# dragonlong/articulated-pose

Hardware: AMD Instinct MI355X
Metric: point-clouds/sec (N=1024, eyeglasses ANCSH infer+pose-fit) (higher is better)
Workload: dtype f32 (network) / f64 (joint LM)

## Files before the change

### articulated-pose_amd/_lib.py

```python
import ctypes
import os
import subprocess

import torch

_HERE = os.path.dirname(os.path.abspath(__file__))
LIB_PATH = os.environ.get("ANCSH_HIP_LIB") or os.path.join(_HERE, "libancsh_hip.so")

_c_int, _c_long, _c_float, _vp = ctypes.c_int, ctypes.c_long, ctypes.c_float, ctypes.c_void_p

SIGNATURES = {
    "ancsh_farthest_point_sample": [_c_int, _c_int, _c_int, _vp, _vp, _vp, _vp],
    "ancsh_farthest_point_sample_gather": [_c_int, _c_int, _c_int, _vp, _vp, _vp, _vp, _vp],
    "ancsh_prob_sample": [_c_int, _c_int, _c_int, _vp, _vp, _vp, _vp, _vp],
    "ancsh_gather_point": [_c_int, _c_int, _c_int, _vp, _vp, _vp, _vp],
    "ancsh_query_ball_point": [_c_int, _c_int, _c_int, _c_float, _c_int, _vp, _vp, _vp, _vp, _vp],
    "ancsh_query_ball_point_multi": [_c_int] + [_vp] * 10,
    "ancsh_group_point": [_c_int, _c_int, _c_int, _c_int, _c_int, _vp, _vp, _vp, _vp],
    "ancsh_group_point_multi": [_c_int] + [_vp] * 9,
    "ancsh_selection_sort": [_c_int, _c_int, _c_int, _c_int, _vp, _vp, _vp, _vp],
    "ancsh_knn_point": [_c_int, _c_int, _c_int, _c_int, _c_int, _vp, _vp, _vp, _vp, _vp],
    "ancsh_group_point_ex": [_c_int, _c_int, _c_int, _c_int, _c_int, _vp, _vp, _vp, _vp, _c_int, _c_int, _vp],
    "ancsh_three_nn": [_c_int, _c_int, _c_int, _vp, _vp, _vp, _vp, _vp],
    "ancsh_three_weights": [_c_int, _vp, _vp, _vp],
    "ancsh_three_nn_weights": [_c_int, _c_int, _c_int, _vp, _vp, _vp, _vp, _vp, _vp],
    "ancsh_three_interpolate": [_c_int, _c_int, _c_int, _c_int, _vp, _vp, _vp, _vp, _vp],
    "ancsh_three_interpolate_ex": [_c_int, _c_int, _c_int, _c_int, _vp, _vp, _vp, _vp, _c_int, _c_int, _vp],
    "ancsh_conv1x1": [_c_long, _c_int, _c_int, _vp, _c_int, _vp, _vp, _vp, _vp, _c_int, _vp, _c_int, _c_int, _vp],
    "ancsh_conv1x1_ex": [_c_long, _c_int, _c_int, _vp, _c_int, _vp, _vp, _vp, _vp, _c_int, _vp, _c_int, _c_int, _vp, _c_int, _vp],
    "ancsh_conv1x1_packed": [_c_long, _c_int, _c_int, _vp, _c_int, _vp, _vp, _vp, _vp, _c_int, _vp, _c_int, _c_int, _vp, _c_int, _vp],
    "ancsh_conv1x1_packed_grouped": [_c_int, _c_long, _c_int, _c_int, _vp, _c_int, _vp, _vp, _vp, _vp, _c_int, _vp, _c_int, _c_int, _vp, _c_int, _vp],
    "ancsh_conv1x1_grouped": [_c_int, _c_long, _c_int, _c_int, _vp, _c_int, _vp, _vp, _vp, _vp, _c_int, _vp, _c_int, _c_int, _vp],
    "ancsh_sa_module_fused_grouped": [_c_int] * 9 + [_vp] * 4 + [_vp, _vp, _vp],
    "ancsh_sa_module_fused_partial_grouped": [_c_int] * 8 + [_vp] * 7,
    "ancsh_fp_interpolate_concat_ex": [_c_int, _c_int, _c_int, _c_int, _vp, _vp, _vp, _vp, _c_int, _vp, _c_int, _c_int, _c_int, _vp],
    "ancsh_sa_pack_weights_bf16x3": [_c_int, _c_int, _vp, _vp, _vp],
    "ancsh_sa_module_fused_bf16x3": [_c_int] * 8 + [_vp] * 4 + [_vp, _vp, _vp],
    "ancsh_sa_module_fused_partial_bf16x3": [_c_int] * 7 + [_vp] * 7,
    "ancsh_sa_module_fused_bf16x3_grouped": [_c_int] * 9 + [_vp] * 4 + [_vp, _vp, _vp],
    "ancsh_sa_module_fused_partial_bf16x3_grouped": [_c_int] * 8 + [_vp] * 7,
    "ancsh_sa_pack_weights_f16x2": [_c_int, _c_int, _vp, _vp, _vp],
    "ancsh_sa_module_fused_f16x2_grouped": [_c_int] * 9 + [_vp] * 4 + [_vp, _vp, _vp],
    "ancsh_sa_module_fused_partial_f16x2_grouped": [_c_int] * 8 + [_vp] * 7,
    "ancsh_mlp_chain_grouped_fp_f16x2": [_c_int] * 5 + [_vp] * 7 + [_vp],
    "ancsh_sa3_chain_grouped_bf16x3": [_c_int] * 7 + [_vp] * 4 + [_vp],
    "ancsh_sa3_chain_grouped_f16x2": [_c_int] * 7 + [_vp] * 4 + [_vp],
    "ancsh_fp1_chain_grouped_bf16x3": [_c_int] * 6 + [_vp] * 4 + [_vp],
    "ancsh_fp1_chain_grouped_f16x2": [_c_int] * 6 + [_vp] * 4 + [_vp],
    "ancsh_fp2_chain_grouped_bf16x3": [_c_int] * 8 + [_vp] * 6 + [_vp],
    "ancsh_fp2_chain_grouped_f16x2": [_c_int] * 8 + [_vp] * 6 + [_vp],
    "ancsh_sa_module_fused_f16x2_grouped_guarded": [_c_int] * 9 + [_vp] * 4 + [_vp, _vp, _vp, _c_int, _vp],
    "ancsh_sa_module_fused_partial_f16x2_grouped_guarded": [_c_int] * 8 + [_vp] * 6 + [_vp, _c_int, _vp],
    "ancsh_mlp_chain_grouped_fp_f16x2_guarded": [_c_int] * 5 + [_vp] * 7 + [_vp, _c_int, _vp],
    "ancsh_sa3_chain_grouped_f16x2_guarded": [_c_int] * 7 + [_vp] * 4 + [_vp, _c_int, _vp],
    "ancsh_fp1_chain_grouped_f16x2_guarded": [_c_int] * 6 + [_vp] * 4 + [_vp, _c_int, _vp],
    "ancsh_fp2_chain_grouped_f16x2_guarded": [_c_int] * 8 + [_vp] * 6 + [_vp, _c_int, _vp],
    "ancsh_iou_3d": [_c_int, _c_int, _vp, _vp, _vp, _vp, _vp],
    "ancsh_joint_params": [_c_int] * 5 + [_vp] * 9 + [_vp],
    "ancsh_part_extents": [_c_int] * 4 + [_vp] * 3 + [_c_int] + [_vp] * 4 + [_vp],
    "ancsh_articulation_rec": [_c_int] * 5 + [_vp] * 10 + [_vp] * 4 + [_vp],
    "ancsh_fp_interpolate_concat": [_c_int, _c_int, _c_int, _c_int, _vp, _vp, _vp, _vp, _c_int, _vp, _c_int, _vp],
    "ancsh_query_ball_group_xyz": [_c_int, _c_int, _c_int, _c_float, _c_int, _vp, _vp, _c_int, _vp, _vp, _vp, _c_int, _vp],
    "ancsh_query_ball_group_xyz_multi": [_c_int] + [_vp] * 13,
    "ancsh_group_max": [_c_long, _c_int, _c_int, _vp, _vp, _vp],
    "ancsh_sa_module_fused": [_c_int] * 8 + [_vp] * 4 + [_vp, _vp, _vp],
    "ancsh_sa_module_fused_partial": [_c_int] * 7 + [_vp] * 7,
    "ancsh_sa_pack_weights": [_c_int, _c_int, _vp, _vp, _vp],
    "ancsh_mlp_chain": [_c_long, _c_int, _vp, _c_int, _c_int, _vp, _vp, _vp],
    "ancsh_mlp_chain_grouped": [_c_int, _c_long, _c_int, _vp, _c_int, _vp, _vp, _vp, _vp, _vp],
    "ancsh_sa3_chain_grouped": [_c_int] * 7 + [_vp] * 4 + [_vp],
    "ancsh_fp_single_source_init": [_c_int] * 5 + [_vp] * 3 + [_vp],
    "ancsh_fp1_chain_grouped": [_c_int] * 6 + [_vp] * 4 + [_vp],
    "ancsh_fp2_chain_grouped": [_c_int] * 8 + [_vp] * 6 + [_vp],
    "ancsh_mlp_chain_grouped_fp": [_c_int] * 5 + [_vp] * 8 + [_vp],
    "ancsh_mlp_chain_grouped_fp_bf16x3": [_c_int] * 5 + [_vp] * 7 + [_vp],
    "ancsh_head_activations": [_c_long, _c_int, _c_int, _vp, _c_int] + [_vp] * 10 + [_vp],
    "ancsh_pose_partition": [_c_int, _c_int, _c_int] + [_vp] * 11 + [_vp],
    "ancsh_pose_poison_records": [_c_int, _c_int, _c_int] + [_vp] * 5 + [_vp],
    "ancsh_pose_joint_direction": [_c_int, _c_int, _c_int, _vp, _vp, _vp, _vp],
    "ancsh_ransac_single": [_c_int, _vp, _vp, _vp, _c_float, _c_int, _vp, ctypes.c_ulonglong, _c_int, _vp, _vp, _vp, _vp, _vp],
    "ancsh_ransac_single_ex": [_c_int, _vp, _vp, _vp, _c_float, _c_int, _vp, ctypes.c_ulonglong, _c_int, _vp, _vp, _vp, _vp, _vp, _c_long, _vp],
    "ancsh_ransac_single_rec": [_c_int, _vp, _vp, _vp, _c_float, _c_int, _vp, ctypes.c_ulonglong, _c_int, _vp, _vp, _vp, _vp, _vp, _c_long,
                                _vp, _c_int, _vp, _c_float, _vp],
    "ancsh_ransac_joint_rec": [_c_int, _vp, _vp, _vp, _vp, _vp, ctypes.c_double, _c_int, _vp, ctypes.c_ulonglong, _c_int]
                              + [_vp] * 7 + [_c_int, _vp, _c_int, _vp, ctypes.c_double, _vp],
    "ancsh_ransac_joint": [_c_int, _vp, _vp, _vp, _vp, _vp, ctypes.c_double, _c_int, _vp, ctypes.c_ulonglong, _c_int]
                          + [_vp] * 7 + [_vp],
    "ancsh_ransac_single_rec_dseed": [_c_int, _vp, _vp, _vp, _c_float, _c_int, _vp, _vp, _c_int, _vp, _vp, _vp, _vp, _vp, _c_long,
                                      _vp, _c_int, _vp, _c_float, _vp],
    "ancsh_ransac_joint_rec_dseed": [_c_int, _vp, _vp, _vp, _vp, _vp, ctypes.c_double, _c_int, _vp, _vp, _c_int]
                                    + [_vp] * 7 + [_c_int, _vp, _c_int, _vp, ctypes.c_double, _vp],
    "ancsh_input_sample_stream": [_c_int, _c_int, _c_int, _vp, _c_long, _vp, _vp, _c_int, _vp, _vp, _vp, _vp, _vp],
    "ancsh_input_sample_stream_keyed": [_c_int, _c_int, _c_int, _vp, _c_long, _vp, _vp, _c_int, _vp, _vp, _vp, _vp, _vp],
    "ancsh_ransac_single_rec_dkey": [_c_int, _vp, _vp, _vp, _c_float, _c_int, _vp, _vp, _c_int, _vp, _vp, _vp, _vp, _vp, _c_long,
                                     _vp, _c_int, _vp, _c_float, _vp],
    "ancsh_ransac_joint_rec_dkey": [_c_int, _vp, _vp, _vp, _vp, _vp, ctypes.c_double, _c_int, _vp, _vp, _c_int]
                                   + [_vp] * 7 + [_c_int, _vp, _c_int, _vp, ctypes.c_double, _vp],
    "ancsh_raw_point_labels": [_c_int] * 5 + [_vp, _c_long] + [_vp] * 8 + [_vp],
    "ancsh_pose_joint_direction_pred": [_c_int, _c_int, _c_int, _c_int, _vp, _vp, _vp, _vp],
    "ancsh_pose_poison_records_pred": [_c_int, _c_int, _c_int] + [_vp] * 4 + [_c_int, _vp, _vp, _vp],
    "ancsh_input_sample_stream_xyz": [_c_int, _c_int, _c_int, _vp, _c_long, _vp, _vp, _vp, _vp, _vp, _vp],
    "ancsh_input_sample_stream_xyz_keyed": [_c_int, _c_int, _c_int, _vp, _c_long, _vp, _vp, _vp, _vp, _vp, _vp],
    "ancsh_ransac_joint_rec_kind": [_c_int, _vp, _vp, _vp, _vp, _vp, ctypes.c_double, _c_int, _vp, ctypes.c_ulonglong, _c_int]
                                   + [_vp] * 7 + [_c_int, _vp, _c_int, _vp, ctypes.c_double, _vp, _vp],
    "ancsh_ransac_joint_rec_dseed_kind": [_c_int, _vp, _vp, _vp, _vp, _vp, ctypes.c_double, _c_int, _vp, _vp, _c_int]
                                         + [_vp] * 7 + [_c_int, _vp, _c_int, _vp, ctypes.c_double, _vp, _vp],
    "ancsh_ransac_joint_rec_dkey_kind": [_c_int, _vp, _vp, _vp, _vp, _vp, ctypes.c_double, _c_int, _vp, _vp, _c_int]
                                        + [_vp] * 7 + [_c_int, _vp, _c_int, _vp, ctypes.c_double, _vp, _vp],
    "ancsh_depth_unproject_stream": [_c_int, _c_int, _vp, _vp, _c_long, _vp, _vp, _vp, _c_long, _vp, _vp, _vp, _vp],
    "ancsh_depth_label_images": [_c_int, _c_int, _vp, _vp, _c_long] + [_vp] * 5 + [_c_long, _vp, _vp, _vp, _c_long, _vp],
    "ancsh_joint_state_rec": [_c_int] * 3 + [_vp, _c_int] + [_vp] * 5 + [_vp],
    "ancsh_fit_quality_rec": [_c_int] * 2 + [_vp] * 4 + [ctypes.c_double] + [_vp] * 3 + [_vp],
    "ancsh_gt_error_rec": [_c_int] * 4 + [_vp, _c_int] + [_vp] * 3 + [_c_int] + [_vp] * 2 + [_vp],
    "ancsh_input_sample": [_c_int, _c_int, _c_int, _vp, _vp, _vp, _vp, _c_int, _c_int, _c_int, _vp, _vp, _vp, _vp, _vp],
    "ancsh_test_losses": [_c_int, _c_int, _c_int, _c_int, _vp, _vp, _vp],
    "ancsh_ransac_joint_ex": [_c_int, _vp, _vp, _vp, _vp, _vp, ctypes.c_double, _c_int, _vp, ctypes.c_ulonglong, _c_int]
                             + [_vp] * 7 + [_c_int, _vp],
    "ancsh_umeyama": [_c_int, _vp, _vp, _vp, _vp, _vp],
    "ancsh_estimate_similarity_transform": [_c_int, _vp, _vp, _vp, _c_int, _vp, ctypes.c_ulonglong, _vp, _vp, _vp],
}

_lib = None


def build(force=False):
    args = ["make", "-s", "-j8", "-C", os.path.join(_HERE, "csrc")]
    if force:
        subprocess.check_call(args + ["clean"])
    subprocess.check_call(args)
    return LIB_PATH


def lib():
    global _lib
    if _lib is None:
        if not os.path.exists(LIB_PATH):
            raise RuntimeError(
                f"{LIB_PATH} is missing: the HIP extension is not built (run __graft_entry__.build()); "
                "there is no CPU fallback for the product path")
        L = ctypes.CDLL(LIB_PATH)
        for name, argtypes in SIGNATURES.items():
            fn = getattr(L, name)
            fn.argtypes = argtypes
            fn.restype = _c_int
        L.ancsh_last_error.restype = ctypes.c_char_p
        L.ancsh_abi_version.restype = _c_int
        L.ancsh_last_ball_query_schedule.restype = _c_int
        L.ancsh_sa_packed_weight_floats.argtypes = [_c_int, _c_int]
        L.ancsh_sa_packed_weight_floats.restype = _c_long
        L.ancsh_sa_packed_weight_bytes_bf16x3.argtypes = [_c_int, _c_int]
        L.ancsh_sa_packed_weight_bytes_bf16x3.restype = _c_long
        L.ancsh_sa_packed_weight_bytes_f16x2.argtypes = [_c_int, _c_int]
        L.ancsh_sa_packed_weight_bytes_f16x2.restype = _c_long
        L.ancsh_ransac_single_quads_floats.argtypes = [_c_long, _c_int]
        L.ancsh_ransac_single_quads_floats.restype = _c_long
        _lib = L
    return _lib


def stream_ptr():
    return torch.cuda.current_stream().cuda_stream


def ptr(t):
    return 0 if t is None else t.data_ptr()


_prof = None
_prof_lead = (0, {})


def profile_start(lead=0, lead_for=None):
    global _prof, _prof_lead
    _prof, _prof_lead = [], (int(lead), dict(lead_for or {}))


def profile_stop():
    global _prof
    rec, _prof = _prof, None
    torch.cuda.synchronize()
    return [(n, a, e0.elapsed_time(e1)) for n, a, e0, e1 in rec]


def call(name, *args):
    L = lib()
    if _prof is not None:
        e0, e1 = torch.cuda.Event(enable_timing=True), torch.cuda.Event(enable_timing=True)
        for _ in range(_prof_lead[1].get(name, _prof_lead[0])):
            getattr(L, name)(*args, stream_ptr())
        e0.record()
        rc = getattr(L, name)(*args, stream_ptr())
        e1.record()
        _prof.append((name, args, e0, e1))
    else:
        rc = getattr(L, name)(*args, stream_ptr())
    if rc != 0:
        msg = L.ancsh_last_error().decode()
        if rc == -1:
            raise ValueError(msg)
        raise RuntimeError(f"{name}: {msg}")


def require_cuda(*tensors):
    for t in tensors:
        if t is not None and not t.is_cuda:
            raise RuntimeError("articulated-pose_amd ops run on the MI355X only: got a CPU tensor "
                               "(no CPU fallback in the product path)")
```

### articulated-pose_amd/csrc/pose.hip

```cpp
#include "common.h"
#include "pose_math.h"

namespace ancsh {
namespace pose {

constexpr int MODEL_A = 13;
constexpr int MODEL_B = 26;

__device__ __forceinline__ unsigned long long splitmix64(unsigned long long x) {
    x += 0x9E3779B97F4A7C15ull;
    x = (x ^ (x >> 30)) * 0xBF58476D1CE4E5B9ull;
    x = (x ^ (x >> 27)) * 0x94D049BB133111EBull;
    return x ^ (x >> 31);
}
__device__ __forceinline__ int device_draw(unsigned long long seed, int prob, int iter, int k, int n) {
    const unsigned long long h = splitmix64(seed ^ splitmix64(((unsigned long long)prob << 40) ^ ((unsigned long long)iter << 8) ^ (unsigned)k));
    return (int)(h % (unsigned long long)n);
}
enum { KEY_VALUE = 0, KEY_DSEED = 1, KEY_DKEY = 2 };
struct DKey {
    const ancsh_stream_key *key;
    int parts;
};
template <int KM> struct KeyArgT { typedef unsigned long long type; };
// ... 112 lines not shown
__device__ __forceinline__ int inlier2_f32(const float R[9], float sc, const float tr[3], f32x2 sx, f32x2 sy, f32x2 sz,
                                           f32x2 tx, f32x2 ty, f32x2 tz, float th_sq) {
#pragma clang fp contract(off)
    const f32x2 rx = __builtin_elementwise_fma((f32x2)R[2], sz, __builtin_elementwise_fma((f32x2)R[1], sy, R[0] * sx));
    const f32x2 ry = __builtin_elementwise_fma((f32x2)R[5], sz, __builtin_elementwise_fma((f32x2)R[4], sy, R[3] * sx));
    const f32x2 rz = __builtin_elementwise_fma((f32x2)R[8], sz, __builtin_elementwise_fma((f32x2)R[7], sy, R[6] * sx));
    const f32x2 ex = (tx - sc * rx) - tr[0], ey = (ty - sc * ry) - tr[1], ez = (tz - sc * rz) - tr[2];
    const f32x2 s = (ex * ex + ey * ey) + ez * ez;
    return (s.x < th_sq ? 1 : 0) + (s.y < th_sq ? 1 : 0);
}

#if defined(__HIP_DEVICE_COMPILE__) && !defined(__gfx950__)
#error "pose.hip: the packed-f32 clamp counting (v_pk_mul_f32 ... clamp, DX10_CLAMP semantics) is written for gfx950 only"
#endif
__device__ __forceinline__ void inlier2_count_f32(const float R[9], float sc, const float tr[3], f32x2 sx, f32x2 sy, f32x2 sz,
                                                  f32x2 tx, f32x2 ty, f32x2 tz, float th_sq, f32x2 &cnt) {
#pragma clang fp contract(off)
    const f32x2 rx = __builtin_elementwise_fma((f32x2)R[2], sz, __builtin_elementwise_fma((f32x2)R[1], sy, R[0] * sx));
    const f32x2 ry = __builtin_elementwise_fma((f32x2)R[5], sz, __builtin_elementwise_fma((f32x2)R[4], sy, R[3] * sx));
    const f32x2 rz = __builtin_elementwise_fma((f32x2)R[8], sz, __builtin_elementwise_fma((f32x2)R[7], sy, R[6] * sx));
    const f32x2 ex = (tx - sc * rx) - tr[0], ey = (ty - sc * ry) - tr[1], ez = (tz - sc * rz) - tr[2];
    const f32x2 s = (ex * ex + ey * ey) + ez * ez;
    const f32x2 nbig = {-0x1p126f, -0x1p126f};
    const f32x2 tbig = {th_sq * 0x1p126f, th_sq * 0x1p126f};
    f32x2 one;
    asm("v_pk_fma_f32 %0, %1, %2, %3 clamp" : "=v"(one) : "v"(s), "v"(nbig), "v"(tbig));
    cnt = cnt + one;
}

__device__ __forceinline__ void load_draw3(const int *draws, unsigned long long seed, int prob, int kbase, int niter, int h, int k0,
                                           int stride, int n, int idx[3]) {
#pragma unroll
    for (int k = 0; k < 3; ++k) {
        int v = draws ? draws[((size_t)prob * niter + h) * stride + k0 + k] : device_draw(seed, prob + kbase, h, k0 + k, n);
        idx[k] = v < 0 ? 0 : (v >= n ? n - 1 : v);
    }
}

#ifndef A_CHUNK_N
#define A_CHUNK_N 2048
#endif
constexpr int A_CHUNK = A_CHUNK_N;

template <int KM>
__global__ __launch_bounds__(256) void ransac_single_score_kernel(const int *__restrict__ off, const float *__restrict__ src,
                                                                  const float *__restrict__ tgt, float th, int niter,
                                                                  const int *__restrict__ draws, KeyArg<KM> seed_arg,
                                                                  int *__restrict__ scores) {
    const unsigned long long seed = kernel_seed<KM>(seed_arg, 0);
    const int kbase = key_problem_base<KM>(seed_arg);
    __shared__ __attribute__((aligned(16))) float pl[6][A_CHUNK];
    const int prob = blockIdx.y, h = blockIdx.x * 256 + threadIdx.x;
    const int r0 = off[prob], n = off[prob + 1] - r0;
    const bool live = h < niter && n > 0;
    float R[9] = {1, 0, 0, 0, 1, 0, 0, 0, 1}, sc = 0.f, tr[3] = {0, 0, 0};
    if (live) {
        int id[3];
        load_draw3(draws, seed, prob, kbase, niter, h, 0, 3, n, id);
        float s3[3][3], t3[3][3];
#pragma unroll
        for (int i = 0; i < 3; ++i)
#pragma unroll
            for (int c = 0; c < 3; ++c) {
                s3[i][c] = src[(size_t)(r0 + id[i]) * 3 + c];
                t3[i][c] = tgt[(size_t)(r0 + id[i]) * 3 + c];
            }
        estimate_single3(s3, t3, R, sc, tr);
    }
    int cnt = 0;
    for (int base = 0; base < n; base += A_CHUNK) {
        const int m = (n - base) < A_CHUNK ? (n - base) : A_CHUNK;
        const int m4 = (m + 3) & ~3;
        __syncthreads();
        for (int e = threadIdx.x; e < m4 * 3; e += 256) {
            const int i = e / 3, c = e - i * 3;
            const bool in = i < m;
            pl[c][i] = in ? src[(size_t)(r0 + base) * 3 + e] : 0.f;
            pl[3 + c][i] = in ? tgt[(size_t)(r0 + base) * 3 + e] : __builtin_inff();
        }
        __syncthreads();
        if (live) {
            const float4 *px = (const float4 *)pl[0], *py = (const float4 *)pl[1], *pz = (const float4 *)pl[2];
            const float4 *pa = (const float4 *)pl[3], *pb = (const float4 *)pl[4], *pc = (const float4 *)pl[5];
            const int nq = m4 >> 2;
            auto score4 = [&](const float4 &x, const float4 &y, const float4 &z, const float4 &a, const float4 &b, const float4 &c) {
                cnt += inlier2_f32(R, sc, tr, f32x2{x.x, x.y}, f32x2{y.x, y.y}, f32x2{z.x, z.y}, f32x2{a.x, a.y}, f32x2{b.x, b.y},
                                   f32x2{c.x, c.y}, th);
                cnt += inlier2_f32(R, sc, tr, f32x2{x.z, x.w}, f32x2{y.z, y.w}, f32x2{z.z, z.w}, f32x2{a.z, a.w}, f32x2{b.z, b.w},
                                   f32x2{c.z, c.w}, th);
            };
            float4 x0 = px[0], y0 = py[0], z0 = pz[0], a0 = pa[0], b0 = pb[0], c0 = pc[0];
            for (int q = 0; q < nq; q += 2) {
                const int q1 = q + 1 < nq ? q + 1 : q, q2 = q + 2 < nq ? q + 2 : q1;
                const float4 x1 = px[q1], y1 = py[q1], z1 = pz[q1], a1 = pa[q1], b1 = pb[q1], c1 = pc[q1];
                __builtin_amdgcn_sched_barrier(0);
                score4(x0, y0, z0, a0, b0, c0);
                __builtin_amdgcn_sched_barrier(0);
                x0 = px[q2]; y0 = py[q2]; z0 = pz[q2]; a0 = pa[q2]; b0 = pb[q2]; c0 = pc[q2];
                __builtin_amdgcn_sched_barrier(0);
                if (q + 1 < nq) score4(x1, y1, z1, a1, b1, c1);
                __builtin_amdgcn_sched_barrier(0);
            }
        }
    }
    if (h < niter) scores[(size_t)prob * niter + h] = cnt;
}

__device__ __forceinline__ int quad_start(int r0, int prob) { return 2 * ((r0 + 7) / 8 + prob); }

__global__ __launch_bounds__(256) void soa_quads_kernel(const int *__restrict__ off, const float *__restrict__ src,
                                                        const float *__restrict__ tgt, float *__restrict__ quads, int cap_quads) {
    const int prob = blockIdx.y, i = blockIdx.x * 256 + threadIdx.x;
    const int r0 = off[prob], n = off[prob + 1] - r0;
    if (i >= ((n + 7) & ~7)) return;
    if (quad_start(r0, prob) + (i >> 2) >= cap_quads) return;
    float *q = quads + ((size_t)quad_start(r0, prob) + (i >> 2)) * 24 + (i & 3);
    const bool in = i < n;
#pragma unroll
    for (int c = 0; c < 3; ++c) {
        q[c * 4] = in ? src[(size_t)(r0 + i) * 3 + c] : 0.f;
        q[12 + c * 4] = in ? tgt[(size_t)(r0 + i) * 3 + c] : __builtin_inff();
    }
}

#ifndef POSE_SCORE_WAVES
#define POSE_SCORE_WAVES 0
#endif
#if POSE_SCORE_WAVES > 0
#define POSE_SCORE_ATTR __attribute__((amdgpu_waves_per_eu(POSE_SCORE_WAVES)))
#else
#define POSE_SCORE_ATTR
#endif
template <int KM>
__global__ __launch_bounds__(256) POSE_SCORE_ATTR void ransac_single_score_sreg_kernel(const int *__restrict__ off, const float *__restrict__ src,
                                                                       const float *__restrict__ tgt, const float *__restrict__ quads,
                                                                       int cap_quads, float th, int niter, const int *__restrict__ draws,
                                                                       KeyArg<KM> seed_arg, int *__restrict__ scores) {
    const unsigned long long seed = kernel_seed<KM>(seed_arg, 0);
    const int kbase = key_problem_base<KM>(seed_arg);
    const int prob = blockIdx.y, h = blockIdx.x * 256 + threadIdx.x;
    const int r0 = off[prob], n = off[prob + 1] - r0;
    float R[9] = {1, 0, 0, 0, 1, 0, 0, 0, 1}, sc = 0.f, tr[3] = {0, 0, 0};
    if (h < niter && n > 0) {
        int id[3];
        load_draw3(draws, seed, prob, kbase, niter, h, 0, 3, n, id);
        float s3[3][3], t3[3][3];
#pragma unroll
        for (int i = 0; i < 3; ++i)
#pragma unroll
            for (int c = 0; c < 3; ++c) {
                s3[i][c] = src[(size_t)(r0 + id[i]) * 3 + c];
                t3[i][c] = tgt[(size_t)(r0 + id[i]) * 3 + c];
            }
        estimate_single3(s3, t3, R, sc, tr);
    }
    typedef float f32x8 __attribute__((ext_vector_type(8)));
    const int q0 = quad_start(r0, prob);
    const f32x8 *Q = reinterpret_cast<const f32x8 *>(quads + (size_t)q0 * 24);
    int nq = ((n + 7) >> 3) * 2;
    nq = min(nq, (cap_quads - q0) & ~1);
    f32x2 cnt2 = {0.f, 0.f};
    auto score4 = [&](const f32x8 &v0, const f32x8 &v1, const f32x8 &v2) {
        inlier2_count_f32(R, sc, tr, f32x2{v0[0], v0[1]}, f32x2{v0[4], v0[5]}, f32x2{v1[0], v1[1]}, f32x2{v1[4], v1[5]},
                          f32x2{v2[0], v2[1]}, f32x2{v2[4], v2[5]}, th, cnt2);
        inlier2_count_f32(R, sc, tr, f32x2{v0[2], v0[3]}, f32x2{v0[6], v0[7]}, f32x2{v1[2], v1[3]}, f32x2{v1[6], v1[7]},
                          f32x2{v2[2], v2[3]}, f32x2{v2[6], v2[7]}, th, cnt2);
    };
    constexpr int LGKM0 = 0xC07F;
    if (nq > 0) {
        f32x8 a0 = Q[0], a1 = Q[1], a2 = Q[2];
        __builtin_amdgcn_s_waitcnt(LGKM0);
        for (int q = 0; q < nq; q += 2) {
            const int q2 = q + 2 < nq ? q + 2 : q;
            const f32x8 b0 = Q[q * 3 + 3], b1 = Q[q * 3 + 4], b2 = Q[q * 3 + 5];
            __builtin_amdgcn_sched_barrier(0);
            score4(a0, a1, a2);
            __builtin_amdgcn_sched_barrier(0);
            __builtin_amdgcn_s_waitcnt(LGKM0);
            a0 = Q[q2 * 3]; a1 = Q[q2 * 3 + 1]; a2 = Q[q2 * 3 + 2];
            __builtin_amdgcn_sched_barrier(0);
            score4(b0, b1, b2);
            __builtin_amdgcn_sched_barrier(0);
            __builtin_amdgcn_s_waitcnt(LGKM0);
        }
    }
    if (h < niter) scores[(size_t)prob * niter + h] = n > 0 ? (int)(cnt2.x + cnt2.y) : 0;
}

template <class T>
__device__ __forceinline__ int block_argmax_first(const T *sc, int niter, T *best_out, void *lds) {
    T bv = (T)-1;
    int bi = 0x7fffffff;
    for (int h = threadIdx.x; h < niter; h += blockDim.x) {
        const T v = sc[h];
        if (v > bv) { bv = v; bi = h; }
    }
#pragma unroll
    for (int o = 32; o > 0; o >>= 1) {
        const T ov = __shfl_xor(bv, o, 64);
        const int oi = __shfl_xor(bi, o, 64);
        if (ov > bv || (ov == bv && oi < bi)) { bv = ov; bi = oi; }
    }
    T *rv = (T *)lds;
    int *ri = (int *)(rv + 8);
    const int lane = threadIdx.x & 63, wave = threadIdx.x >> 6, nw = blockDim.x >> 6;
    __syncthreads();
    if (lane == 0) { rv[wave] = bv; ri[wave] = bi; }
    __syncthreads();
    bv = rv[0]; bi = ri[0];
    for (int w = 1; w < nw; ++w)
        if (rv[w] > bv || (rv[w] == bv && ri[w] < bi)) { bv = rv[w]; bi = ri[w]; }
    __syncthreads();
    *best_out = bv;
    return bi;
}

__device__ __forceinline__ void pair_sums(const float (*cs)[3], const float (*ct)[3], int n, double (&pr)[3]) {
#pragma clang fp contract(off)
    const int lane = threadIdx.x & 63;
    const int wave = __builtin_amdgcn_readfirstlane(threadIdx.x >> 6), nw = blockDim.x >> 6;
    const int seg = (n + nw - 1) / nw;
    const int j0 = wave * seg, j1 = min(n, j0 + seg);
    constexpr int RB = 6;
    for (int ib = lane; ib < n; ib += 64 * RB) {
        float sx[RB], sy[RB], sz[RB], tx[RB], ty[RB], tz[RB], ab[RB], aa[RB], bb[RB];
#pragma unroll
        for (int r = 0; r < RB; ++r) {
            const int i = min(ib + 64 * r, n - 1);
            sx[r] = cs[i][0]; sy[r] = cs[i][1]; sz[r] = cs[i][2];
            tx[r] = ct[i][0]; ty[r] = ct[i][1]; tz[r] = ct[i][2];
            ab[r] = aa[r] = bb[r] = 0.f;
        }
        for (int j = j0; j < j1; ++j) {
            const float cx = cs[j][0], cy = cs[j][1], cz = cs[j][2], dx = ct[j][0], dy = ct[j][1], dz = ct[j][2];
#pragma unroll
            for (int r = 0; r < RB; ++r) {
                const float ux = sx[r] - cx, uy = sy[r] - cy, uz = sz[r] - cz;
                const float vx = tx[r] - dx, vy = ty[r] - dy, vz = tz[r] - dz;
                const float A = __builtin_amdgcn_sqrtf((ux * ux + uy * uy) + uz * uz);
                const float b = __builtin_amdgcn_sqrtf((vx * vx + vy * vy) + vz * vz);
                ab[r] += A * b;
                aa[r] += A * A;
                bb[r] += b * b;
            }
        }
#pragma unroll
        for (int r = 0; r < RB; ++r)
            if (ib + 64 * r < n) { pr[0] += (double)ab[r]; pr[1] += (double)aa[r]; pr[2] += (double)bb[r]; }
    }
}

__device__ __forceinline__ void refit_similarity(const float (*cs)[3], const float (*ct)[3], int n_in, double *red,
                                                 double R[9], double &scale, double tr[3]) {
    double sums[6] = {0, 0, 0, 0, 0, 0};
    for (int i = threadIdx.x; i < n_in; i += 256) {
#pragma unroll
        for (int c = 0; c < 3; ++c) { sums[c] += cs[i][c]; sums[3 + c] += ct[i][c]; }
    }
    block_sum<6>(sums, red, 4);
    double sm[3], tm[3];
#pragma unroll
    for (int c = 0; c < 3; ++c) { sm[c] = sums[c] / n_in; tm[c] = sums[3 + c] / n_in; }
    double M[9] = {0, 0, 0, 0, 0, 0, 0, 0, 0};
    for (int i = threadIdx.x; i < n_in; i += 256)
#pragma unroll
        for (int a = 0; a < 3; ++a)
#pragma unroll
            for (int b = 0; b < 3; ++b) M[a * 3 + b] += (ct[i][a] - tm[a]) * (cs[i][b] - sm[b]);
    block_sum<9>(M, red, 4);
    double q[4];
    horn_quat(M, q);
    quat_to_mat(q, R);
    double pr[3] = {0, 0, 0};
    pair_sums(cs, ct, n_in, pr);
    block_sum<3>(pr, red, 4);
    scale = pr[0] / (pr[1] + 1e-6);
    const double sf = (double)(float)scale;
#pragma unroll
    for (int a = 0; a < 3; ++a) tr[a] = tm[a] - sf * (R[a * 3 + 0] * sm[0] + R[a * 3 + 1] * sm[1] + R[a * 3 + 2] * sm[2]);
}

__device__ __forceinline__ int compact_flagged(bool flag, int i, int n, const float *src, const float *tgt, size_t row0,
                                               float (*cs)[3], float (*ct)[3], int base, int *wcnt) {
    const int lane = threadIdx.x & 63, wave = threadIdx.x >> 6;
    const unsigned long long m = __ballot(flag);
    __syncthreads();
    if (lane == 0) wcnt[wave] = __popcll(m);
    __syncthreads();
    int start = base;
    for (int w = 0; w < wave; ++w) start += wcnt[w];
    const int total = wcnt[0] + wcnt[1] + wcnt[2] + wcnt[3];
    if (flag) {
        const int pos = start + __builtin_amdgcn_mbcnt_hi((unsigned)(m >> 32), __builtin_amdgcn_mbcnt_lo((unsigned)m, 0));
#pragma unroll
        for (int c = 0; c < 3; ++c) {
            cs[pos][c] = src[(row0 + i) * 3 + c];
            ct[pos][c] = tgt[(row0 + i) * 3 + c];
        }
    }
    return base + total;
}

template <int KM>
__global__ __launch_bounds__(256) void ransac_single_finish_kernel(const int *__restrict__ off, const float *__restrict__ src,
                                                                   const float *__restrict__ tgt, float th, int niter,
                                                                   const int *__restrict__ draws, KeyArg<KM> seed_arg,
                                                                   const int *__restrict__ scores, int max_n,
                                                                   double *__restrict__ out_model,
                                                                   unsigned char *__restrict__ out_inliers,
                                                                   int *__restrict__ out_best, FitExtras E) {
    const unsigned long long seed = kernel_seed<KM>(seed_arg, 0);
    const int kbase = key_problem_base<KM>(seed_arg);
    extern __shared__ __attribute__((aligned(16))) unsigned char smem[];
    double *red = (double *)smem;
    int *wcnt = (int *)(red + 64);
    float(*cs)[3] = (float(*)[3])(wcnt + 8);
    float(*ct)[3] = cs + max_n;
    const int prob = blockIdx.x;
    const int r0 = off[prob], n = off[prob + 1] - r0;
    double *om = out_model + (size_t)prob * MODEL_A;
    if (n <= 0 || n > max_n) {
        if (threadIdx.x < MODEL_A) om[threadIdx.x] = NAN;
        if (E.record && threadIdx.x < (E.K == 1 ? 2 * MODEL_A : MODEL_A)) E.record[(size_t)prob * 26 + threadIdx.x] = NAN;
        if (E.tie && threadIdx.x < 2) E.tie[prob * 2 + threadIdx.x] = 0;
        if (threadIdx.x == 0) { out_best[prob * 2] = -1; out_best[prob * 2 + 1] = n <= 0 ? 0 : -2; }
        for (int i = threadIdx.x; i < n; i += 256) out_inliers[r0 + i] = 0;
        return;
    }
    int best_score;
    const int best = block_argmax_first<int>(scores + (size_t)prob * niter, niter, &best_score, red);
    int id[3];
    load_draw3(draws, seed, prob, kbase, niter, best, 0, 3, n, id);
    float s3[3][3], t3[3][3], R[9], sc, tr[3];
#pragma unroll
    for (int i = 0; i < 3; ++i)
#pragma unroll
        for (int c = 0; c < 3; ++c) {
            s3[i][c] = src[(size_t)(r0 + id[i]) * 3 + c];
            t3[i][c] = tgt[(size_t)(r0 + id[i]) * 3 + c];
        }
    estimate_single3(s3, t3, R, sc, tr);
    int n_in = 0, n_border = 0, n_near = 0;
    for (int base = 0; base < n; base += 256) {
        const int i = base + threadIdx.x;
        bool f = false, border = false;
        if (i < n) {
            const float *ps = src + (size_t)(r0 + i) * 3, *pt = tgt + (size_t)(r0 + i) * 3;
            const float rs = residual_sq_f32(R, sc, tr, ps[0], ps[1], ps[2], pt[0], pt[1], pt[2]);
            f = rs < th;
            border = rs >= E.lo_f && rs < E.hi_f;
            out_inliers[r0 + i] = f ? 1 : 0;
        }
        n_border += __popcll(__ballot(border));
        n_in = compact_flagged(f, i, n, src, tgt, (size_t)r0, cs, ct, n_in, wcnt);
    }
    if (E.tie) {
        const bool winner_degenerate = id[0] == id[1] || id[0] == id[2] || id[1] == id[2];
        __shared__ int s_cand[TIE_MAX_CAND];
        const int *sp = scores + (size_t)prob * niter;
        const int lane = threadIdx.x & 63, wave = threadIdx.x >> 6;
        int found = 0;
        for (int h0 = 0; h0 < niter; h0 += 256) {
            const int h = h0 + threadIdx.x;
            bool cand = false;
            if (h < niter && h != best && sp[h] >= best_score - 1) {
                int d3[3];
                load_draw3(draws, seed, prob, kbase, niter, h, 0, 3, n, d3);
                cand = d3[0] == d3[1] || d3[0] == d3[2] || d3[1] == d3[2];
            }
            const unsigned long long m = __ballot(cand);
            __syncthreads();
            if (lane == 0) wcnt[wave] = __popcll(m);
            __syncthreads();
            int start = found;
            for (int w = 0; w < wave; ++w) start += wcnt[w];
            if (cand) {
                const int slot = start + __builtin_amdgcn_mbcnt_hi((unsigned)(m >> 32), __builtin_amdgcn_mbcnt_lo((unsigned)m, 0));
                if (slot < TIE_MAX_CAND) s_cand[slot] = h;
            }
            found += wcnt[0] + wcnt[1] + wcnt[2] + wcnt[3];
        }
        __syncthreads();
        const int ncand = found < TIE_MAX_CAND ? found : TIE_MAX_CAND;
        n_near = found - ncand + (winner_degenerate ? 1 : 0);
        for (int c = 0; c < ncand; ++c) {
            const int h = s_cand[c];
            int d3[3];
            load_draw3(draws, seed, prob, kbase, niter, h, 0, 3, n, d3);
            float hs[3][3], ht[3][3], hR[9], hsc, htr[3];
#pragma unroll
            for (int i = 0; i < 3; ++i)
#pragma unroll
                for (int cc = 0; cc < 3; ++cc) {
                    hs[i][cc] = src[(size_t)(r0 + d3[i]) * 3 + cc];
                    ht[i][cc] = tgt[(size_t)(r0 + d3[i]) * 3 + cc];
                }
            estimate_single3(hs, ht, hR, hsc, htr);
            int differs = 0;
            for (int i = threadIdx.x; i < n; i += 256) {
                const float *ps = src + (size_t)(r0 + i) * 3, *pt = tgt + (size_t)(r0 + i) * 3;
                const bool f = residual_sq_f32(hR, hsc, htr, ps[0], ps[1], ps[2], pt[0], pt[1], pt[2]) < th;
                differs |= (int)(f != (out_inliers[r0 + i] != 0));
            }
            n_near += __syncthreads_or(differs) ? 1 : 0;
        }
        if ((threadIdx.x & 63) == 0) wcnt[4 + (threadIdx.x >> 6)] = n_border;
        __syncthreads();
        if (threadIdx.x == 0) {
            E.tie[prob * 2] = wcnt[4] + wcnt[5] + wcnt[6] + wcnt[7];
            E.tie[prob * 2 + 1] = winner_degenerate ? -n_near : n_near;
        }
    }
    __syncthreads();
    double Rd[9], scale, trd[3];
    if (n_in > 0) {
        refit_similarity(cs, ct, n_in, red, Rd, scale, trd);
    } else {
#pragma unroll
        for (int a = 0; a < 9; ++a) Rd[a] = NAN;
        scale = NAN; trd[0] = trd[1] = trd[2] = NAN;
    }
    if (threadIdx.x == 0) {
#pragma unroll
        for (int a = 0; a < 9; ++a) om[a] = Rd[a];
        om[9] = (double)(float)scale;
#pragma unroll
        for (int a = 0; a < 3; ++a) om[10 + a] = trd[a];
        out_best[prob * 2] = best;
        out_best[prob * 2 + 1] = best_score;
        if (E.record) {
            double *rec = E.record + (size_t)prob * 26;
#pragma unroll
            for (int a = 0; a < MODEL_A; ++a) rec[a] = om[a];
            if (E.K == 1) {
#pragma unroll
                for (int a = 0; a < MODEL_A; ++a) rec[MODEL_A + a] = om[a];
            }
        }
    }
}

struct PartFd {
    Rod b, p[3];
    double rh[3];
    double blk[6];
    double gv[3];
    double ju[3];
    double jd[3][3];

    __device__ __forceinline__ void begin_points(const double r[3]) {
        b = rod_prepare(r[0], r[1], r[2]);
#pragma unroll
        for (int q = 0; q < 3; ++q) {
            const double h = fd_step(r[q]);
            rh[q] = fast_rcp(h);
            p[q] = rod_prepare(r[0] + (q == 0 ? h : 0.0), r[1] + (q == 1 ? h : 0.0), r[2] + (q == 2 ? h : 0.0));
        }
#pragma unroll
        for (int i = 0; i < 6; ++i) blk[i] = 0.0;
        gv[0] = gv[1] = gv[2] = 0.0;
    }
    __device__ __forceinline__ void begin(const double r[3], const double J[3]) {
        begin_points(r);
        rod_apply(b, J[0], J[1], J[2], ju[0], ju[1], ju[2]);
#pragma unroll
        for (int q = 0; q < 3; ++q) {
            double qx, qy, qz;
            rod_apply(p[q], J[0], J[1], J[2], qx, qy, qz);
            jd[0][q] = qx; jd[1][q] = qy; jd[2][q] = qz;
        }
    }
    __device__ __forceinline__ void point(double px, double py, double pz, double yx, double yy, double yz) {
        double ox, oy, oz;
        rod_apply(b, px, py, pz, ox, oy, oz);
        const double f0 = yx - ox, f1 = yy - oy, f2 = yz - oz;
        double a[3][3];
#pragma unroll
        for (int q = 0; q < 3; ++q) {
            double qx, qy, qz;
            rod_apply(p[q], px, py, pz, qx, qy, qz);
            a[0][q] = ((yx - qx) - f0) * rh[q];
            a[1][q] = ((yy - qy) - f1) * rh[q];
            a[2][q] = ((yz - qz) - f2) * rh[q];
        }
#pragma unroll
        for (int q = 0; q < 3; ++q) {
#pragma unroll
            for (int r = 0; r <= q; ++r) blk[q * (q + 1) / 2 + r] += a[0][q] * a[0][r] + a[1][q] * a[1][r] + a[2][q] * a[2][r];
            gv[q] += a[0][q] * f0 + a[1][q] * f1 + a[2][q] * f2;
        }
    }
};

__device__ __forceinline__ void assemble_normal(const PartFd &p0, const double blk0[6], const double g0[3], const PartFd &p1,
                                                const double blk1[6], const double g1[3], double wj, double A[21], double g[6]) {
    double f[3], a[3][6];
#pragma unroll
    for (int c = 0; c < 3; ++c) f[c] = p0.ju[c] - p1.ju[c];
#pragma unroll
    for (int c = 0; c < 3; ++c)
#pragma unroll
        for (int q = 0; q < 3; ++q) {
            a[c][q] = (((p0.jd[c][q] - p1.ju[c]) - f[c])) * p0.rh[q];
            a[c][3 + q] = (((p0.ju[c] - p1.jd[c][q]) - f[c])) * p1.rh[q];
        }
#pragma unroll
    for (int i = 0; i < 6; ++i) {
#pragma unroll
        for (int j = 0; j <= i; ++j) {
            double v = wj * (a[0][i] * a[0][j] + a[1][i] * a[1][j] + a[2][i] * a[2][j]);
            if (i < 3) v += blk0[i * (i + 1) / 2 + j];
            else if (j >= 3) v += blk1[(i - 3) * (i - 2) / 2 + (j - 3)];
            A[i * (i + 1) / 2 + j] = v;
        }
        g[i] = wj * (a[0][i] * f[0] + a[1][i] * f[1] + a[2][i] * f[2]) + (i < 3 ? g0[i] : g1[i - 3]);
    }
}

__device__ __forceinline__ double prismatic_cost(const double x[6]) {
    const double a = x[0] - x[3], b = x[1] - x[4], c = x[2] - x[5];
    return a * a + b * b + c * c;
}
__device__ __forceinline__ void assemble_normal_prismatic(const double x[6], const double blk0[6], const double g0[3],
                                                          const double blk1[6], const double g1[3], double A[21], double g[6]) {
    double f[3], d0[3], d1[3];
#pragma unroll
    for (int c = 0; c < 3; ++c) {
        const double h0 = fd_step(x[c]), h1 = fd_step(x[3 + c]);
        f[c] = x[c] - x[3 + c];
        d0[c] = (((x[c] + h0) - x[3 + c]) - f[c]) * fast_rcp(h0);
        d1[c] = ((x[c] - (x[3 + c] + h1)) - f[c]) * fast_rcp(h1);
    }
#pragma unroll
    for (int i = 0; i < 6; ++i) {
#pragma unroll
        for (int j = 0; j <= i; ++j) {
            double v = 0.0;
            if (i < 3) v = (i == j ? d0[i] * d0[i] : 0.0) + blk0[i * (i + 1) / 2 + j];
            else if (j >= 3) v = (i == j ? d1[i - 3] * d1[i - 3] : 0.0) + blk1[(i - 3) * (i - 2) / 2 + (j - 3)];
            else if (i - 3 == j) v = d1[j] * d0[j];
            A[i * (i + 1) / 2 + j] = v;
        }
        g[i] = i < 3 ? d0[i] * f[i] + g0[i] : d1[i - 3] * f[i - 3] + g1[i - 3];
    }
}

template <bool PRISM>
struct HypProblemT {
    double x0[3][3], y0[3][3], x1[3][3], y1[3][3], J[3], wj;

    __device__ __forceinline__ double cost(const double x[6]) const {
        const Rod r0 = rod_prepare(x[0], x[1], x[2]), r1 = rod_prepare(x[3], x[4], x[5]);
        double s = 0.0, ox, oy, oz;
#pragma unroll
        for (int i = 0; i < 3; ++i) {
            rod_apply(r0, x0[i][0], x0[i][1], x0[i][2], ox, oy, oz);
            const double a = y0[i][0] - ox, b = y0[i][1] - oy, c = y0[i][2] - oz;
            s += a * a + b * b + c * c;
            rod_apply(r1, x1[i][0], x1[i][1], x1[i][2], ox, oy, oz);
            const double d = y1[i][0] - ox, e = y1[i][1] - oy, f = y1[i][2] - oz;
            s += d * d + e * e + f * f;
        }
        if constexpr (PRISM) {
            return s + prismatic_cost(x);
        } else {
            double ux, uy, uz, wx, wy, wz;
            rod_apply(r0, J[0], J[1], J[2], ux, uy, uz);
            rod_apply(r1, J[0], J[1], J[2], wx, wy, wz);
            s += wj * ((ux - wx) * (ux - wx) + (uy - wy) * (uy - wy) + (uz - wz) * (uz - wz));
            return s;
        }
    }
    __device__ __forceinline__ void normal(const double x[6], double A[21], double g[6]) const {
        PartFd p0, p1;
        if constexpr (PRISM) p0.begin_points(x); else p0.begin(x, J);
#pragma unroll
        for (int i = 0; i < 3; ++i) p0.point(x0[i][0], x0[i][1], x0[i][2], y0[i][0], y0[i][1], y0[i][2]);
        if constexpr (PRISM) p1.begin_points(x + 3); else p1.begin(x + 3, J);
#pragma unroll
        for (int i = 0; i < 3; ++i) p1.point(x1[i][0], x1[i][1], x1[i][2], y1[i][0], y1[i][1], y1[i][2]);
        if constexpr (PRISM) assemble_normal_prismatic(x, p0.blk, p0.gv, p1.blk, p1.gv, A, g);
        else assemble_normal(p0, p0.blk, p0.gv, p1, p1.blk, p1.gv, wj, A, g);
    }
};
typedef HypProblemT<false> HypProblem;

__device__ __forceinline__ void scales3(const float s[3][3], const float t[3][3], float &sc, float &sc_inv) {
    double ab = 0.0, aa = 0.0, bb = 0.0;
#pragma unroll
    for (int i = 0; i < 3; ++i)
#pragma unroll
        for (int j = i + 1; j < 3; ++j) {
            double ds = 0.0, dt = 0.0;
#pragma unroll
            for (int c = 0; c < 3; ++c) {
                const double u = (double)s[i][c] - s[j][c], v = (double)t[i][c] - t[j][c];
                ds += u * u;
                dt += v * v;
            }
            ab += 2.0 * sqrt(ds) * sqrt(dt);
            aa += 2.0 * ds;
            bb += 2.0 * dt;
        }
    sc = (float)(ab / (aa + 1e-6));
    sc_inv = (float)(ab / (bb + 1e-6));
}

__device__ __forceinline__ void center_part3(const float s[3][3], const float t[3][3], float sc_inv, double xc[3][3],
                                             double yc[3][3]) {
    float sm[3], tm[3];
#pragma unroll
    for (int c = 0; c < 3; ++c) {
        sm[c] = ((s[0][c] + s[1][c]) + s[2][c]) / 3.0f;
        tm[c] = ((sc_inv * t[0][c] + sc_inv * t[1][c]) + sc_inv * t[2][c]) / 3.0f;
    }
#pragma unroll
    for (int i = 0; i < 3; ++i) {
#pragma unroll
        for (int c = 0; c < 3; ++c) {
            xc[i][c] = (double)(s[i][c] - sm[c]);
            yc[i][c] = (double)(sc_inv * t[i][c] - tm[c]);
        }
    }
}

__device__ __forceinline__ void prep_part3(const float s[3][3], const float t[3][3], float sc_inv, double xc[3][3],
                                           double yc[3][3], double rv[3]) {
    center_part3(s, t, sc_inv, xc, yc);
    double M[9] = {0, 0, 0, 0, 0, 0, 0, 0, 0};
#pragma unroll
    for (int i = 0; i < 3; ++i)
#pragma unroll
        for (int a = 0; a < 3; ++a)
#pragma unroll
            for (int b = 0; b < 3; ++b) M[a * 3 + b] += yc[i][a] * xc[i][b];
    double q[4];
    horn_quat_fast(M, q);
    quat_to_rotvec(q, rv);
}

__device__ __forceinline__ double residual_sq_f64(const double R[9], double sc, const double tr[3], float sx, float sy, float sz,
                                                  float tx, float ty, float tz) {
    const double rx = R[0] * sx + R[1] * sy + R[2] * sz, ry = R[3] * sx + R[4] * sy + R[5] * sz,
                 rz = R[6] * sx + R[7] * sy + R[8] * sz;
    const double ex = ((double)tx - sc * rx) - tr[0], ey = ((double)ty - sc * ry) - tr[1], ez = ((double)tz - sc * rz) - tr[2];
    return ex * ex + ey * ey + ez * ez;
}
__device__ __forceinline__ bool inlier_f64(const double R[9], double sc, const double tr[3], float sx, float sy, float sz,
                                           float tx, float ty, float tz, double th) {
    return residual_sq_f64(R, sc, tr, sx, sy, sz, tx, ty, tz) < th;
}

struct HypSamples {
    float s0[3][3], t0[3][3], s1[3][3], t1[3][3];
};
__device__ __forceinline__ void load_hyp_samples(const float *__restrict__ src, const float *__restrict__ tgt, const int *draws,
                                                 unsigned long long seed, int prob, int kbase, int niter, int h, int a0, int n0, int a1,
                                                 int n1, HypSamples &q) {
    int i0[3], i1[3];
    load_draw3(draws, seed, prob, kbase, niter, h, 0, 6, n0, i0);
    load_draw3(draws, seed, prob, kbase, niter, h, 3, 6, n1, i1);
#pragma unroll
    for (int i = 0; i < 3; ++i)
#pragma unroll
        for (int c = 0; c < 3; ++c) {
            q.s0[i][c] = src[(size_t)(a0 + i0[i]) * 3 + c];
            q.t0[i][c] = tgt[(size_t)(a0 + i0[i]) * 3 + c];
            q.s1[i][c] = src[(size_t)(a1 + i1[i]) * 3 + c];
            q.t1[i][c] = tgt[(size_t)(a1 + i1[i]) * 3 + c];
        }
}

template <int KM>
__global__ __launch_bounds__(64) void ransac_joint_init_kernel(const int *__restrict__ rng0, const int *__restrict__ rng1,
                                                               const float *__restrict__ src, const float *__restrict__ tgt,
                                                               int niter, const int *__restrict__ draws, KeyArg<KM> seed_arg,
                                                               double *__restrict__ scores, double *__restrict__ models) {
    const unsigned long long seed = kernel_seed<KM>(seed_arg, 1);
    const int kbase = key_problem_base<KM>(seed_arg);
    const int prob = blockIdx.y, h = blockIdx.x * 64 + threadIdx.x;
    const int a0 = rng0[prob * 2], n0 = rng0[prob * 2 + 1] - a0;
    const int a1 = rng1[prob * 2], n1 = rng1[prob * 2 + 1] - a1;
    if (h >= niter) return;
    double *mo = models + ((size_t)prob * niter + h) * MODEL_B;
    if (n0 <= 0 || n1 <= 0) {
        scores[(size_t)prob * niter + h] = -1.0;
        for (int i = 0; i < MODEL_B; ++i) mo[i] = NAN;
        return;
    }
    HypSamples q;
    load_hyp_samples(src, tgt, draws, seed, prob, kbase, niter, h, a0, n0, a1, n1, q);
    float sc0, sc0i, sc1, sc1i;
    scales3(q.s0, q.t0, sc0, sc0i);
    scales3(q.s1, q.t1, sc1, sc1i);
    double xc[3][3], yc[3][3], x[6];
    prep_part3(q.s0, q.t0, sc0i, xc, yc, x);
    prep_part3(q.s1, q.t1, sc1i, xc, yc, x + 3);
#pragma unroll
    for (int i = 0; i < 6; ++i) mo[i] = x[i];
    mo[6] = sc0i; mo[7] = sc1i; mo[8] = sc0; mo[9] = sc1;
}

constexpr int HYP_CHUNK = 256;
constexpr int HYP_CHUNK_SMALL = 64;
constexpr long HYP_SMALL_LAUNCH = 8192;
constexpr int HYP_REFILL = 16;

template <int KM, bool PRISM>
__device__ __forceinline__ void ransac_joint_lm_run(const int *__restrict__ rng0, const int *__restrict__ rng1,
                                                    const float *__restrict__ src, const float *__restrict__ tgt,
                                                    const float *__restrict__ joint_dir, int niter,
                                                    const int *__restrict__ draws, KeyArg<KM> seed_arg,
                                                    double *__restrict__ models, int *__restrict__ lm_stat, int chunk) {
    const unsigned long long seed = kernel_seed<KM>(seed_arg, 1);
    const int kbase = key_problem_base<KM>(seed_arg);
    const int prob = blockIdx.y;
    const int a0 = rng0[prob * 2], n0 = rng0[prob * 2 + 1] - a0;
    const int a1 = rng1[prob * 2], n1 = rng1[prob * 2 + 1] - a1;
    if (n0 <= 0 || n1 <= 0) return;
    const int c1 = min(niter, (int)(blockIdx.x + 1) * chunk);
    int next = blockIdx.x * chunk;
    HypProblemT<PRISM> P;
    if constexpr (!PRISM) {
        P.J[0] = joint_dir[prob * 3]; P.J[1] = joint_dir[prob * 3 + 1]; P.J[2] = joint_dir[prob * 3 + 2];
        P.wj = 3.0;
    }
    Lm6 S;
    bool active = false;
    int h = 0;
    for (;;) {
        const unsigned long long idle = __ballot(!active);
        const int n_idle = __popcll(idle);
        if (next < c1 && (n_idle >= HYP_REFILL || n_idle >= c1 - next || n_idle == 64)) {
            if (!active) {
                const int mine = next + __builtin_amdgcn_mbcnt_hi((unsigned)(idle >> 32), __builtin_amdgcn_mbcnt_lo((unsigned)idle, 0));
                if (mine < c1) {
                    h = mine;
                    const double *mo = models + ((size_t)prob * niter + h) * MODEL_B;
                    HypSamples q;
                    load_hyp_samples(src, tgt, draws, seed, prob, kbase, niter, h, a0, n0, a1, n1, q);
                    center_part3(q.s0, q.t0, (float)mo[6], P.x0, P.y0);
                    center_part3(q.s1, q.t1, (float)mo[7], P.x1, P.y1);
#pragma unroll
                    for (int i = 0; i < 6; ++i) S.x[i] = mo[i];
                    lm6_begin(P, S);
                    active = true;
                }
            }
            next += n_idle;
        } else if (n_idle == 64) {
            break;
        }
        if (active && lm6_trip(P, S, 1e-4, 1e-8, 1e-8, 4200)) {
            double *mo = models + ((size_t)prob * niter + h) * MODEL_B;
#pragma unroll
            for (int i = 0; i < 6; ++i) mo[i] = S.x[i];
#ifdef LM_COUNT
            if (lm_stat) { lm_stat[((size_t)prob * niter + h) * 2] = S.info | (S.trips << 4) | (S.nchol << 17); lm_stat[((size_t)prob * niter + h) * 2 + 1] = S.nfev; }
#else
            if (lm_stat) { lm_stat[((size_t)prob * niter + h) * 2] = S.info; lm_stat[((size_t)prob * niter + h) * 2 + 1] = S.nfev; }
#endif
            active = false;
        }
    }
}

template <int KM>
__global__ __launch_bounds__(64) void ransac_joint_lm_kernel(const int *__restrict__ rng0, const int *__restrict__ rng1,
                                                             const float *__restrict__ src, const float *__restrict__ tgt,
                                                             const float *__restrict__ joint_dir, int niter,
                                                             const int *__restrict__ draws, KeyArg<KM> seed_arg,
                                                             double *__restrict__ models, int *__restrict__ lm_stat, int chunk) {
    ransac_joint_lm_run<KM, false>(rng0, rng1, src, tgt, joint_dir, niter, draws, seed_arg, models, lm_stat, chunk);
}

template <int KM>
__global__ __launch_bounds__(64) void ransac_joint_lm_kind_kernel(const int *__restrict__ rng0, const int *__restrict__ rng1,
                                                                  const float *__restrict__ src, const float *__restrict__ tgt,
                                                                  const float *__restrict__ joint_dir, int niter,
                                                                  const int *__restrict__ draws, KeyArg<KM> seed_arg,
                                                                  double *__restrict__ models, int *__restrict__ lm_stat, int chunk,
                                                                  const int *__restrict__ joint_kind) {
    if (joint_kind[blockIdx.y] != 0) ransac_joint_lm_run<KM, true>(rng0, rng1, src, tgt, joint_dir, niter, draws, seed_arg, models, lm_stat, chunk);
    else ransac_joint_lm_run<KM, false>(rng0, rng1, src, tgt, joint_dir, niter, draws, seed_arg, models, lm_stat, chunk);
}

constexpr int COOP_G = 8;
constexpr int COOP_XCH = 112;
constexpr int COOP_HYP_PER_WAVE = 32;

__device__ __forceinline__ void group_lds_fence() {
    __builtin_amdgcn_fence(__ATOMIC_RELEASE, "wavefront");
    __builtin_amdgcn_wave_barrier();
    __builtin_amdgcn_fence(__ATOMIC_ACQUIRE, "wavefront");
}

template <bool PRISM>
struct HypProblemCoopT {
    double x0[3][3], y0[3][3], x1[3][3], y1[3][3], J[3], wj;
    double *xch;
    int role;

    __device__ __forceinline__ double cost(const double x[6]) const {
        const bool joint = role >= 6;
        const bool p1 = role >= 3 && role < 6;
        const int i = joint ? 0 : (p1 ? role - 3 : role);
        double partial;
        if (!joint) {
            const Rod r = p1 ? rod_prepare(x[3], x[4], x[5]) : rod_prepare(x[0], x[1], x[2]);
            const double px = p1 ? (i == 0 ? x1[0][0] : i == 1 ? x1[1][0] : x1[2][0]) : (i == 0 ? x0[0][0] : i == 1 ? x0[1][0] : x0[2][0]);
            const double py = p1 ? (i == 0 ? x1[0][1] : i == 1 ? x1[1][1] : x1[2][1]) : (i == 0 ? x0[0][1] : i == 1 ? x0[1][1] : x0[2][1]);
            const double pz = p1 ? (i == 0 ? x1[0][2] : i == 1 ? x1[1][2] : x1[2][2]) : (i == 0 ? x0[0][2] : i == 1 ? x0[1][2] : x0[2][2]);
            const double tx = p1 ? (i == 0 ? y1[0][0] : i == 1 ? y1[1][0] : y1[2][0]) : (i == 0 ? y0[0][0] : i == 1 ? y0[1][0] : y0[2][0]);
            const double ty = p1 ? (i == 0 ? y1[0][1] : i == 1 ? y1[1][1] : y1[2][1]) : (i == 0 ? y0[0][1] : i == 1 ? y0[1][1] : y0[2][1]);
            const double tz = p1 ? (i == 0 ? y1[0][2] : i == 1 ? y1[1][2] : y1[2][2]) : (i == 0 ? y0[0][2] : i == 1 ? y0[1][2] : y0[2][2]);
            double ox, oy, oz;
            rod_apply(r, px, py, pz, ox, oy, oz);
            const double a = tx - ox, b = ty - oy, c = tz - oz;
            partial = a * a + b * b + c * c;
        } else if constexpr (PRISM) {
            partial = prismatic_cost(x);
        } else {
            const Rod r0 = rod_prepare(x[0], x[1], x[2]), r1 = rod_prepare(x[3], x[4], x[5]);
            double ux, uy, uz, wx, wy, wz;
            rod_apply(r0, J[0], J[1], J[2], ux, uy, uz);
            rod_apply(r1, J[0], J[1], J[2], wx, wy, wz);
            partial = (ux - wx) * (ux - wx) + (uy - wy) * (uy - wy) + (uz - wz) * (uz - wz);
        }
        double *cs = xch + 102;
        if (role < 7) cs[role] = partial;
        group_lds_fence();
        double s = 0.0;
#pragma unroll
        for (int k = 0; k < 3; ++k) { s += cs[k]; s += cs[3 + k]; }
        if constexpr (PRISM) s += cs[6]; else s += wj * cs[6];
        group_lds_fence();
        return s;
    }

    __device__ __forceinline__ void normal(const double x[6], double A[21], double g[6]) const {
        double *col = xch, *jdx = xch + 54, *rhx = xch + 72, *fx = xch + 78, *jux = xch + 96;
        {
            const int cr = role < 6 ? role : role - 6;
            const bool p1 = cr >= 3;
            const int q = p1 ? cr - 3 : cr;
            const double r0 = p1 ? x[3] : x[0], r1 = p1 ? x[4] : x[1], r2 = p1 ? x[5] : x[2];
            const Rod b = rod_prepare(r0, r1, r2);
            const double h = fd_step(q == 0 ? r0 : q == 1 ? r1 : r2);
            const double rh = fast_rcp(h);
            const Rod pr = rod_prepare(r0 + (q == 0 ? h : 0.0), r1 + (q == 1 ? h : 0.0), r2 + (q == 2 ? h : 0.0));
            const bool wr = role < 6;
#pragma unroll
            for (int i = 0; i < 3; ++i) {
                const double px = p1 ? x1[i][0] : x0[i][0], py = p1 ? x1[i][1] : x0[i][1], pz = p1 ? x1[i][2] : x0[i][2];
                const double yx = p1 ? y1[i][0] : y0[i][0], yy = p1 ? y1[i][1] : y0[i][1], yz = p1 ? y1[i][2] : y0[i][2];
                double ox, oy, oz, qx, qy, qz;
                rod_apply(b, px, py, pz, ox, oy, oz);
                const double f0 = yx - ox, f1 = yy - oy, f2 = yz - oz;
                rod_apply(pr, px, py, pz, qx, qy, qz);
                if (wr) {
                    col[cr * 9 + i * 3 + 0] = ((yx - qx) - f0) * rh;
                    col[cr * 9 + i * 3 + 1] = ((yy - qy) - f1) * rh;
                    col[cr * 9 + i * 3 + 2] = ((yz - qz) - f2) * rh;
                    if (q == 0) { fx[(p1 ? 9 : 0) + i * 3] = f0; fx[(p1 ? 9 : 0) + i * 3 + 1] = f1; fx[(p1 ? 9 : 0) + i * 3 + 2] = f2; }
                }
            }
            if constexpr (!PRISM) {
                double ux, uy, uz, vx, vy, vz;
                rod_apply(b, J[0], J[1], J[2], ux, uy, uz);
                rod_apply(pr, J[0], J[1], J[2], vx, vy, vz);
                if (wr) {
                    jdx[cr * 3] = vx; jdx[cr * 3 + 1] = vy; jdx[cr * 3 + 2] = vz;
                    rhx[cr] = rh;
                    if (q == 0) { jux[(p1 ? 3 : 0)] = ux; jux[(p1 ? 3 : 0) + 1] = uy; jux[(p1 ? 3 : 0) + 2] = uz; }
                }
            }
        }
        group_lds_fence();
        double blk[2][6], gv[2][3];
#pragma unroll
        for (int p = 0; p < 2; ++p) {
#pragma unroll
            for (int e = 0; e < 6; ++e) blk[p][e] = 0.0;
            gv[p][0] = gv[p][1] = gv[p][2] = 0.0;
#pragma unroll
            for (int i = 0; i < 3; ++i) {
                double a[3][3];
#pragma unroll
                for (int q = 0; q < 3; ++q)
#pragma unroll
                    for (int c = 0; c < 3; ++c) a[c][q] = col[(p * 3 + q) * 9 + i * 3 + c];
                const double f0 = fx[p * 9 + i * 3], f1 = fx[p * 9 + i * 3 + 1], f2 = fx[p * 9 + i * 3 + 2];
#pragma unroll
                for (int q = 0; q < 3; ++q) {
#pragma unroll
                    for (int r = 0; r <= q; ++r) blk[p][q * (q + 1) / 2 + r] += a[0][q] * a[0][r] + a[1][q] * a[1][r] + a[2][q] * a[2][r];
                    gv[p][q] += a[0][q] * f0 + a[1][q] * f1 + a[2][q] * f2;
                }
            }
        }
        if constexpr (PRISM) {
            assemble_normal_prismatic(x, blk[0], gv[0], blk[1], gv[1], A, g);
        } else {
        double f[3], a[3][6];
#pragma unroll
        for (int c = 0; c < 3; ++c) f[c] = jux[c] - jux[3 + c];
#pragma unroll
        for (int c = 0; c < 3; ++c)
#pragma unroll
            for (int q = 0; q < 3; ++q) {
                a[c][q] = ((jdx[q * 3 + c] - jux[3 + c]) - f[c]) * rhx[q];
                a[c][3 + q] = ((jux[c] - jdx[(3 + q) * 3 + c]) - f[c]) * rhx[3 + q];
            }
#pragma unroll
        for (int i = 0; i < 6; ++i) {
#pragma unroll
            for (int j = 0; j <= i; ++j) {
                double v = wj * (a[0][i] * a[0][j] + a[1][i] * a[1][j] + a[2][i] * a[2][j]);
                if (i < 3) v += blk[0][i * (i + 1) / 2 + j];
                else if (j >= 3) v += blk[1][(i - 3) * (i - 2) / 2 + (j - 3)];
                A[i * (i + 1) / 2 + j] = v;
            }
            g[i] = wj * (a[0][i] * f[0] + a[1][i] * f[1] + a[2][i] * f[2]) + (i < 3 ? gv[0][i] : gv[1][i - 3]);
        }
        }
        group_lds_fence();
    }
};
typedef HypProblemCoopT<false> HypProblemCoop;

template <int KM, bool PRISM>
__device__ __forceinline__ void ransac_joint_lm_coop_run(const int *__restrict__ rng0, const int *__restrict__ rng1,
                                                         const float *__restrict__ src, const float *__restrict__ tgt,
                                                         const float *__restrict__ joint_dir, int niter,
                                                         const int *__restrict__ draws, KeyArg<KM> seed_arg,
                                                         double *__restrict__ models, int *__restrict__ lm_stat,
                                                         double (*xch)[COOP_XCH]) {
    const unsigned long long seed = kernel_seed<KM>(seed_arg, 1);
    const int kbase = key_problem_base<KM>(seed_arg);
    const int prob = blockIdx.y, lane = threadIdx.x;
    const int a0 = rng0[prob * 2], n0 = rng0[prob * 2 + 1] - a0;
    const int a1 = rng1[prob * 2], n1 = rng1[prob * 2 + 1] - a1;
    if (n0 <= 0 || n1 <= 0) return;
    const int c1 = min(niter, (int)(blockIdx.x + 1) * COOP_HYP_PER_WAVE);
    int next = blockIdx.x * COOP_HYP_PER_WAVE;
    const int grp = lane / COOP_G;
    const unsigned long long leaders = 0x0101010101010101ull;
    HypProblemCoopT<PRISM> P;
    if constexpr (!PRISM) {
        P.J[0] = joint_dir[prob * 3]; P.J[1] = joint_dir[prob * 3 + 1]; P.J[2] = joint_dir[prob * 3 + 2];
        P.wj = 3.0;
    }
    P.xch = xch[grp];
    P.role = lane & (COOP_G - 1);
    Lm6 S;
    bool active = false;
    int h = 0;
    for (;;) {
        const unsigned long long idle = __ballot(!active) & leaders;
        const int n_idle = __popcll(idle);
        if (next < c1 && n_idle > 0) {
            if (!active) {
                const int mine = next + __popcll(idle & ((1ull << (grp * COOP_G)) - 1ull));
                if (mine < c1) {
                    h = mine;
                    const double *mo = models + ((size_t)prob * niter + h) * MODEL_B;
                    HypSamples q;
                    load_hyp_samples(src, tgt, draws, seed, prob, kbase, niter, h, a0, n0, a1, n1, q);
                    center_part3(q.s0, q.t0, (float)mo[6], P.x0, P.y0);
                    center_part3(q.s1, q.t1, (float)mo[7], P.x1, P.y1);
#pragma unroll
                    for (int i = 0; i < 6; ++i) S.x[i] = mo[i];
                    lm6_begin(P, S);
                    active = true;
                }
            }
            next += n_idle;
        } else if (n_idle == 64 / COOP_G) {
            break;
        }
        if (active && lm6_trip(P, S, 1e-4, 1e-8, 1e-8, 4200)) {
            if (P.role == 0) {
                double *mo = models + ((size_t)prob * niter + h) * MODEL_B;
#pragma unroll
                for (int i = 0; i < 6; ++i) mo[i] = S.x[i];
                if (lm_stat) { lm_stat[((size_t)prob * niter + h) * 2] = S.info; lm_stat[((size_t)prob * niter + h) * 2 + 1] = S.nfev; }
            }
            active = false;
        }
    }
}

template <int KM>
__global__ __launch_bounds__(64) void ransac_joint_lm_coop_kernel(const int *__restrict__ rng0, const int *__restrict__ rng1,
                                                                  const float *__restrict__ src, const float *__restrict__ tgt,
                                                                  const float *__restrict__ joint_dir, int niter,
                                                                  const int *__restrict__ draws, KeyArg<KM> seed_arg,
                                                                  double *__restrict__ models, int *__restrict__ lm_stat) {
    __shared__ double xch[64 / COOP_G][COOP_XCH];
    ransac_joint_lm_coop_run<KM, false>(rng0, rng1, src, tgt, joint_dir, niter, draws, seed_arg, models, lm_stat, xch);
}

template <int KM>
__global__ __launch_bounds__(64) void ransac_joint_lm_coop_kind_kernel(const int *__restrict__ rng0, const int *__restrict__ rng1,
                                                                       const float *__restrict__ src, const float *__restrict__ tgt,
                                                                       const float *__restrict__ joint_dir, int niter,
                                                                       const int *__restrict__ draws, KeyArg<KM> seed_arg,
                                                                       double *__restrict__ models, int *__restrict__ lm_stat,
                                                                       const int *__restrict__ joint_kind) {
    __shared__ double xch[64 / COOP_G][COOP_XCH];
    if (joint_kind[blockIdx.y] != 0) ransac_joint_lm_coop_run<KM, true>(rng0, rng1, src, tgt, joint_dir, niter, draws, seed_arg, models, lm_stat, xch);
    else ransac_joint_lm_coop_run<KM, false>(rng0, rng1, src, tgt, joint_dir, niter, draws, seed_arg, models, lm_stat, xch);
}

template <int KM>
__global__ __launch_bounds__(64) void ransac_joint_model_kernel(const int *__restrict__ rng0, const int *__restrict__ rng1,
                                                                const float *__restrict__ src, const float *__restrict__ tgt,
                                                                int niter, const int *__restrict__ draws, KeyArg<KM> seed_arg,
                                                                double *__restrict__ models) {
    const unsigned long long seed = kernel_seed<KM>(seed_arg, 1);
    const int kbase = key_problem_base<KM>(seed_arg);
    const int prob = blockIdx.y, h = blockIdx.x * 64 + threadIdx.x;
    const int a0 = rng0[prob * 2], n0 = rng0[prob * 2 + 1] - a0;
    const int a1 = rng1[prob * 2], n1 = rng1[prob * 2 + 1] - a1;
    if (h >= niter || n0 <= 0 || n1 <= 0) return;
    double *mo = models + ((size_t)prob * niter + h) * MODEL_B;
    HypSamples q;
    load_hyp_samples(src, tgt, draws, seed, prob, kbase, niter, h, a0, n0, a1, n1, q);
    double x[6];
#pragma unroll
    for (int i = 0; i < 6; ++i) x[i] = mo[i];
    const float sc0 = (float)mo[8], sc1 = (float)mo[9];
    double R0[9], R1[9], tr0[3], tr1[3];
    rotvec_to_mat(x, R0);
    rotvec_to_mat(x + 3, R1);
#pragma unroll
    for (int a = 0; a < 3; ++a) {
        double u = 0.0, v = 0.0;
#pragma unroll
        for (int i = 0; i < 3; ++i) {
            u += (double)q.t0[i][a] - (double)sc0 * (R0[a * 3] * q.s0[i][0] + R0[a * 3 + 1] * q.s0[i][1] + R0[a * 3 + 2] * q.s0[i][2]);
            v += (double)q.t1[i][a] - (double)sc1 * (R1[a * 3] * q.s1[i][0] + R1[a * 3 + 1] * q.s1[i][1] + R1[a * 3 + 2] * q.s1[i][2]);
        }
        tr0[a] = u / 3.0;
        tr1[a] = v / 3.0;
    }
#pragma unroll
    for (int a = 0; a < 9; ++a) { mo[a] = R0[a]; mo[13 + a] = R1[a]; }
    mo[9] = sc0; mo[22] = sc1;
#pragma unroll
    for (int a = 0; a < 3; ++a) { mo[10 + a] = tr0[a]; mo[23 + a] = tr1[a]; }
}

__global__ __launch_bounds__(256) void ransac_joint_verify_kernel(const int *__restrict__ rng0, const int *__restrict__ rng1,
                                                                 const float *__restrict__ src, const float *__restrict__ tgt,
                                                                 double th, int niter, const double *__restrict__ models,
                                                                 double *__restrict__ scores) {
    const int prob = blockIdx.y, lane = threadIdx.x & 63;
    const int h = blockIdx.x * 4 + (threadIdx.x >> 6);
    if (h >= niter) return;
    const int a0 = rng0[prob * 2], n0 = rng0[prob * 2 + 1] - a0;
    const int a1 = rng1[prob * 2], n1 = rng1[prob * 2 + 1] - a1;
    if (n0 <= 0 || n1 <= 0) return;
    const double *mo = models + ((size_t)prob * niter + h) * MODEL_B;
    double R0[9], R1[9], tr0[3], tr1[3];
#pragma unroll
    for (int a = 0; a < 9; ++a) { R0[a] = mo[a]; R1[a] = mo[13 + a]; }
    const double sc0 = mo[9], sc1 = mo[22];
#pragma unroll
    for (int a = 0; a < 3; ++a) { tr0[a] = mo[10 + a]; tr1[a] = mo[23 + a]; }
    int c0 = 0, c1 = 0;
    for (int i = lane; i < n0; i += 64) {
        const float *ps = src + (size_t)(a0 + i) * 3, *pt = tgt + (size_t)(a0 + i) * 3;
        c0 += inlier_f64(R0, sc0, tr0, ps[0], ps[1], ps[2], pt[0], pt[1], pt[2], th) ? 1 : 0;
    }
    for (int i = lane; i < n1; i += 64) {
        const float *ps = src + (size_t)(a1 + i) * 3, *pt = tgt + (size_t)(a1 + i) * 3;
        c1 += inlier_f64(R1, sc1, tr1, ps[0], ps[1], ps[2], pt[0], pt[1], pt[2], th) ? 1 : 0;
    }
#pragma unroll
    for (int o = 32; o > 0; o >>= 1) { c0 += __shfl_xor(c0, o, 64); c1 += __shfl_xor(c1, o, 64); }
    if (lane == 0) scores[(size_t)prob * niter + h] = ((double)c0 / 3.0 + (double)c1 / 3.0) / 2.0;
}

template <bool PRISM>
struct BlockProblemT {
    const float (*x0)[3];
// ... 474 lines not shown
    }
#pragma unroll
    for (int a = 0; a < 3; ++a) {
#pragma unroll
        for (int b = 0; b < 3; ++b) o[15 + a * 4 + b] = s * R[a * 3 + b];
        o[15 + a * 4 + 3] = T[a];
    }
    o[27] = 0; o[28] = 0; o[29] = 0; o[30] = 1; o[31] = 0;
}


__device__ __forceinline__ void umeyama_small(const double (*s)[3], const double (*t)[3], int n, double T[12]) {
    double sm[3] = {0, 0, 0}, tm[3] = {0, 0, 0};
    for (int i = 0; i < n; ++i)
#pragma unroll
        for (int c = 0; c < 3; ++c) { sm[c] += s[i][c]; tm[c] += t[i][c]; }
#pragma unroll
    for (int c = 0; c < 3; ++c) { sm[c] /= n; tm[c] /= n; }
    double M[9] = {0, 0, 0, 0, 0, 0, 0, 0, 0}, var = 0.0;
    for (int i = 0; i < n; ++i) {
#pragma unroll
        for (int a = 0; a < 3; ++a) {
#pragma unroll
            for (int b = 0; b < 3; ++b) M[a * 3 + b] += (t[i][a] - tm[a]) * (s[i][b] - sm[b]);
            var += (s[i][a] - sm[a]) * (s[i][a] - sm[a]);
        }
    }
#pragma unroll
    for (int a = 0; a < 9; ++a) M[a] /= n;
    var /= n;
    double q[4], R[9];
    horn_quat(M, q);
    quat_to_mat(q, R);
    double tr = 0.0;
#pragma unroll
    for (int a = 0; a < 9; ++a) tr += R[a] * M[a];
    const double sc = tr / var;
#pragma unroll
    for (int a = 0; a < 3; ++a) {
#pragma unroll
        for (int b = 0; b < 3; ++b) T[a * 4 + b] = sc * R[a * 3 + b];
        T[a * 4 + 3] = tm[a] - sc * (R[a * 3] * sm[0] + R[a * 3 + 1] * sm[1] + R[a * 3 + 2] * sm[2]);
    }
}

__global__ __launch_bounds__(128) void ransac_umeyama5_kernel(const int *__restrict__ off, const float *__restrict__ src,
                                                              const float *__restrict__ tgt, int niter,
                                                              const int *__restrict__ draws, unsigned long long seed,
                                                              double *__restrict__ out, int *__restrict__ status) {
    __shared__ double red[64];
    __shared__ double h_res[128], h_ratio[128];
    __shared__ double Tsel[12];
    __shared__ double thr[2];
    __shared__ int sel;
    const int prob = blockIdx.x, r0 = off[prob], n = off[prob + 1] - r0, h = threadIdx.x;
    double *o = out + (size_t)prob * 32;
    if (n <= 0 || niter > 128) {
        if (h < 32) o[h] = NAN;
        if (h == 0) status[prob] = -1;
        return;
    }
    double nm[2] = {0, 0};
    for (int i = h; i < n; i += 128) {
        const float *ps = src + (size_t)(r0 + i) * 3, *pt = tgt + (size_t)(r0 + i) * 3;
        nm[0] += sqrt((double)ps[0] * ps[0] + (double)ps[1] * ps[1] + (double)ps[2] * ps[2]);
        nm[1] += sqrt((double)pt[0] * pt[0] + (double)pt[1] * pt[1] + (double)pt[2] * pt[2]);
    }
    block_sum<2>(nm, red, 2);
    if (h == 0) {
        const double ts = (nm[1] / n) / (nm[0] / n), st = (nm[0] / n) / (nm[1] / n);
        thr[0] = st > ts ? st : ts;
        thr[1] = thr[0] / 100.0;
    }
    __syncthreads();
    const double passT = thr[0], stopT = thr[1];
    double T[12];
    if (h < niter) {
        double s5[5][3], t5[5][3];
#pragma unroll
        for (int k = 0; k < 5; ++k) {
            int v = draws ? draws[((size_t)prob * niter + h) * 5 + k] : device_draw(seed, prob, h, k, n);
            v = v < 0 ? 0 : (v >= n ? n - 1 : v);
#pragma unroll
            for (int c = 0; c < 3; ++c) { s5[k][c] = src[(size_t)(r0 + v) * 3 + c]; t5[k][c] = tgt[(size_t)(r0 + v) * 3 + c]; }
        }
        umeyama_small(s5, t5, 5, T);
        double rs = 0.0;
        int cnt = 0;
        for (int i = 0; i < n; ++i) {
            const float *ps = src + (size_t)(r0 + i) * 3, *pt = tgt + (size_t)(r0 + i) * 3;
            double e2 = 0.0;
#pragma unroll
            for (int a = 0; a < 3; ++a) {
                const double e = (double)pt[a] - (T[a * 4] * ps[0] + T[a * 4 + 1] * ps[1] + T[a * 4 + 2] * ps[2] + T[a * 4 + 3]);
                e2 += e * e;
            }
            rs += e2;
            if (sqrt(e2) < passT && i != 0) ++cnt;
        }
        h_res[h] = sqrt(rs);
        h_ratio[h] = (double)cnt / (double)n;
    }
    __syncthreads();
    if (h == 0) {
        double bestRes = 1e10, bestRatio = 0.0;
        int best = -1;
        for (int i = 0; i < niter; ++i) {
            if (h_ratio[i] > bestRatio) { bestRes = h_res[i]; bestRatio = h_ratio[i]; best = i; }
            if (bestRes < stopT) break;
        }
        sel = best;
        thr[0] = bestRatio;
    }
    __syncthreads();
    const int best = sel;
    const double bestRatio = thr[0];
    if (best >= 0 && h == best)
#pragma unroll
        for (int a = 0; a < 12; ++a) Tsel[a] = T[a];
    __syncthreads();
    if (bestRatio < 0.1) {
        if (h < 32) o[h] = NAN;
        if (h == 0) status[prob] = 1;
        return;
    }
    double sums[7] = {0, 0, 0, 0, 0, 0, 0};
    auto is_in = [&](int i) {
        if (best < 0) return true;
        const float *ps = src + (size_t)(r0 + i) * 3, *pt = tgt + (size_t)(r0 + i) * 3;
        double e2 = 0.0;
#pragma unroll
        for (int a = 0; a < 3; ++a) {
            const double e = (double)pt[a] - (Tsel[a * 4] * ps[0] + Tsel[a * 4 + 1] * ps[1] + Tsel[a * 4 + 2] * ps[2] + Tsel[a * 4 + 3]);
            e2 += e * e;
        }
        return sqrt(e2) < passT;
    };
    for (int i = h; i < n; i += 128)
        if (is_in(i)) {
#pragma unroll
            for (int c = 0; c < 3; ++c) { sums[c] += src[(size_t)(r0 + i) * 3 + c]; sums[3 + c] += tgt[(size_t)(r0 + i) * 3 + c]; }
            sums[6] += 1.0;
        }
    block_sum<7>(sums, red, 2);
    const double m = sums[6];
    double sm[3], tm[3];
#pragma unroll
    for (int c = 0; c < 3; ++c) { sm[c] = sums[c] / m; tm[c] = sums[3 + c] / m; }
    double acc[10] = {0, 0, 0, 0, 0, 0, 0, 0, 0, 0};
    for (int i = h; i < n; i += 128)
        if (is_in(i)) {
            double sc[3], tc[3];
#pragma unroll
            for (int c = 0; c < 3; ++c) { sc[c] = src[(size_t)(r0 + i) * 3 + c] - sm[c]; tc[c] = tgt[(size_t)(r0 + i) * 3 + c] - tm[c]; }
#pragma unroll
            for (int a = 0; a < 3; ++a)
#pragma unroll
                for (int b = 0; b < 3; ++b) acc[a * 3 + b] += tc[a] * sc[b];
            acc[9] += sc[0] * sc[0] + sc[1] * sc[1] + sc[2] * sc[2];
        }
    block_sum<10>(acc, red, 2);
    if (h != 0) return;
    double M[9], q[4], R[9];
#pragma unroll
    for (int a = 0; a < 9; ++a) M[a] = acc[a] / m;
    horn_quat(M, q);
    quat_to_mat(q, R);
    double trace = 0.0;
#pragma unroll
    for (int a = 0; a < 9; ++a) trace += R[a] * M[a];
    const double s = trace / (acc[9] / m);
    o[0] = o[1] = o[2] = s;
#pragma unroll
    for (int a = 0; a < 3; ++a)
#pragma unroll
        for (int b = 0; b < 3; ++b) o[3 + a * 3 + b] = R[b * 3 + a];
#pragma unroll
    for (int a = 0; a < 3; ++a) {
        const double Tv = tm[a] - s * (R[a * 3] * sm[0] + R[a * 3 + 1] * sm[1] + R[a * 3 + 2] * sm[2]);
        o[12 + a] = Tv;
#pragma unroll
        for (int b = 0; b < 3; ++b) o[15 + a * 4 + b] = s * R[a * 3 + b];
        o[15 + a * 4 + 3] = Tv;
    }
    o[27] = 0; o[28] = 0; o[29] = 0; o[30] = 1; o[31] = bestRatio;
    status[prob] = 0;
}

}
}

using namespace ancsh;
using namespace ancsh::pose;

static float sq_threshold_f32(float th) {
    float t = th * th;
    while (sqrtf(t) >= th && t > 0.f) t = nextafterf(t, 0.f);
    while (sqrtf(t) < th) t = nextafterf(t, INFINITY);
    return t;
}
static double sq_threshold_f64(double th) {
    double t = th * th;
    while (sqrt(t) >= th && t > 0.0) t = nextafter(t, 0.0);
    while (sqrt(t) < th) t = nextafter(t, INFINITY);
    return t;
}

extern "C" int ancsh_pose_partition(int b, int n, int K, const float *W, const float *P, const float *nocs, int *labels,
                                    int *part_index, int *off, float *src, float *tgt, int *counts, int *rng0, int *rng1,
                                    void *stream) {
    ANCSH_REQUIRE(b >= 0 && n > 0 && K >= 1 && K <= 16, "pose_partition: bad shape b=%d n=%d K=%d", b, n, K);
    if (b == 0) return ANCSH_OK;
    ANCSH_REQUIRE(W && P && nocs && part_index && off && src && tgt, "pose_partition: null pointer");
    ANCSH_REQUIRE((rng0 == nullptr) == (rng1 == nullptr), "pose_partition: rng0 and rng1 go together");
    hipLaunchKernelGGL(partition_kernel, dim3(b), dim3(256), 0, (hipStream_t)stream, n, K, W, P, nocs, labels, part_index, off,
                       src, tgt, counts, rng0, rng1);
    return check_launch("pose_partition");
}

extern "C" int ancsh_pose_poison_records(int b, int n, int K, const float *P, const float *nocs, const float *W, const float *joint_axis,
                                         double *record, void *stream) {
    ANCSH_REQUIRE(b >= 0 && n > 0 && K >= 1 && K <= 16, "pose_poison_records: bad shape b=%d n=%d K=%d", b, n, K);
    if (b == 0) return ANCSH_OK;
    ANCSH_REQUIRE(P && nocs && W && record, "pose_poison_records: null pointer");
    hipLaunchKernelGGL(poison_records_kernel<false>, dim3(b), dim3(1024), 0, (hipStream_t)stream, n, K, P, nocs, W, joint_axis, record, 0,
                       nullptr);
    return check_launch("pose_poison_records");
}

extern "C" int ancsh_pose_poison_records_pred(int b, int n, int K, const float *P, const float *nocs, const float *W,
                                              const float *joint_axis, int joint_channels, const float *joint_index, double *record,
                                              void *stream) {
    ANCSH_REQUIRE(b >= 0 && n > 0 && K >= 1 && K <= 16, "pose_poison_records_pred: bad shape b=%d n=%d K=%d", b, n, K);
    ANCSH_REQUIRE(joint_channels >= 1 && joint_channels <= 64, "pose_poison_records_pred: joint_channels=%d must be in [1,64]",
                  joint_channels);
    ANCSH_REQUIRE(P && nocs && W && joint_index && record, "pose_poison_records_pred: null pointer");
    if (b == 0) return ANCSH_OK;
    hipLaunchKernelGGL(poison_records_kernel<true>, dim3(b), dim3(1024), 0, (hipStream_t)stream, n, K, P, nocs, W, joint_axis, record,
                       joint_channels, joint_index);
    return check_launch("pose_poison_records_pred");
}

extern "C" int ancsh_pose_joint_direction(int b, int n, int K, const float *joint_axis, const int *joint_cls, float *out,
                                          void *stream) {
    ANCSH_REQUIRE(b >= 0 && n > 0 && K >= 1, "pose_joint_direction: bad shape");
    ANCSH_REQUIRE(n <= 8192, "pose_joint_direction: n %d > 8192", n);
    if (b == 0 || K == 1) return ANCSH_OK;
    ANCSH_REQUIRE(joint_axis && joint_cls && out, "pose_joint_direction: null pointer");
    int npow2 = 1;
    while (npow2 < n) npow2 <<= 1;
    const size_t lds = (size_t)3 * npow2 * sizeof(float);
    if (lds > 48 * 1024) (void)hipFuncSetAttribute((const void *)joint_direction_kernel, hipFuncAttributeMaxDynamicSharedMemorySize, (int)lds);
    hipLaunchKernelGGL(joint_direction_kernel, dim3(b, K - 1), dim3(256), lds, (hipStream_t)stream, n, K, joint_axis, joint_cls, out);
    return check_launch("pose_joint_direction");
}

extern "C" int ancsh_pose_joint_direction_pred(int b, int n, int K, int joint_channels, const float *joint_axis, const float *joint_index,
                                               float *out, void *stream) {
    ANCSH_REQUIRE(b >= 0 && n > 0 && K >= 2 && K <= 16, "pose_joint_direction_pred: bad shape b=%d n=%d K=%d (K >= 2: a joint)", b, n, K);
    ANCSH_REQUIRE(n <= 8192, "pose_joint_direction_pred: n %d > 8192", n);
    ANCSH_REQUIRE(joint_channels >= 1 && joint_channels <= 64, "pose_joint_direction_pred: joint_channels=%d must be in [1,64]",
                  joint_channels);
    ANCSH_REQUIRE(joint_axis && joint_index && out, "pose_joint_direction_pred: null pointer");
    if (b == 0) return ANCSH_OK;
    int npow2 = 1;
    while (npow2 < n) npow2 <<= 1;
    const size_t lds = (size_t)3 * npow2 * sizeof(float);
    if (lds > 48 * 1024)
        (void)hipFuncSetAttribute((const void *)joint_direction_pred_kernel, hipFuncAttributeMaxDynamicSharedMemorySize, (int)lds);
    hipLaunchKernelGGL(joint_direction_pred_kernel, dim3(b, K - 1), dim3(256), lds, (hipStream_t)stream, n, K, joint_channels, joint_axis,
                       joint_index, out);
    return check_launch("pose_joint_direction_pred");
}

static FitExtras no_extras() {
    FitExtras E;
    E.record = nullptr; E.K = 0; E.tie = nullptr;
    E.lo_f = E.hi_f = 0.f; E.lo_d = E.hi_d = 0.0;
    E.draws = nullptr; E.seed = 0;
    return E;
}

static int make_extras(const char *who, int nprob, double *record, int K, int min_K, int *tie, double th, double window, FitExtras &E) {
    E.record = record; E.K = K; E.tie = tie;
    if (record) {
        ANCSH_REQUIRE(K >= min_K && nprob % (K - (min_K - 1)) == 0, "%s: record needs K >= %d and nprob (%d) a multiple of %s (K = %d)", who, min_K, nprob,
                      min_K == 1 ? "K" : "K - 1", K);
    }
    if (tie) {
        ANCSH_REQUIRE(window >= 0.0 && window < th, "%s: tie_window %g must be in [0, inlier_th)", who, window);
        const double lo = (th - window) * (th - window), hi = (th + window) * (th + window);
        E.lo_f = (float)lo; E.hi_f = (float)hi; E.lo_d = lo; E.hi_d = hi;
    }
    return ANCSH_OK;
}

static long single_quads_needed(long rows, int nprob) { return 2 * ((rows + 7) / 8 + nprob) + 2; }

extern "C" long ancsh_ransac_single_quads_floats(long rows, int nprob) {
    if (rows < 0 || nprob < 0) return -1;
    return 24 * single_quads_needed(rows, nprob);
}

template <int KM>
static int ransac_single_impl(int nprob, const int *off, const float *src, const float *tgt, float inlier_th, int niter,
                              const int *draws, KeyArg<KM> seed, int max_n, double *out_model,
                              unsigned char *out_inliers, int *out_best, int *scratch_scores, float *scratch_quads, long rows,
                              FitExtras E, void *stream) {
    ANCSH_REQUIRE(nprob >= 0 && niter > 0 && max_n > 0, "ransac_single: bad sizes nprob=%d niter=%d max_n=%d", nprob, niter, max_n);
    ANCSH_REQUIRE(max_n <= 6144, "ransac_single: max_n %d > 6144 (refit keeps the inliers in LDS)", max_n);
    if (nprob == 0) return ANCSH_OK;
    ANCSH_REQUIRE(off && src && tgt && out_model && out_inliers && out_best && scratch_scores, "ransac_single: null pointer");
    hipStream_t st = (hipStream_t)stream;
    ANCSH_REQUIRE(inlier_th > 0.f, "ransac_single: inlier_th must be positive");
    inlier_th = sq_threshold_f32(inlier_th);
    if (scratch_quads && inlier_th >= 0x1p-100f && inlier_th < 4.0f) {
        ANCSH_REQUIRE(rows >= 0 && rows < (1L << 30), "ransac_single_ex: rows=%ld out of range", rows);
        ANCSH_REQUIRE((((uintptr_t)scratch_quads) & 31) == 0, "ransac_single_ex: scratch_quads must be 32-byte aligned");
        const int cap = (int)single_quads_needed(rows, nprob);
        hipLaunchKernelGGL(soa_quads_kernel, dim3((max_n + 7 + 255) / 256, nprob), dim3(256), 0, st, off, src, tgt, scratch_quads, cap);
        hipLaunchKernelGGL(ransac_single_score_sreg_kernel<KM>, dim3((niter + 255) / 256, nprob), dim3(256), 0, st, off, src, tgt,
                           (const float *)scratch_quads, cap, inlier_th, niter, draws, seed, scratch_scores);
    } else {
        hipLaunchKernelGGL(ransac_single_score_kernel<KM>, dim3((niter + 255) / 256, nprob), dim3(256), 0, st, off, src, tgt, inlier_th,
                           niter, draws, seed, scratch_scores);
    }
    const size_t lds = 64 * sizeof(double) + 8 * sizeof(int) + (size_t)2 * max_n * 3 * sizeof(float);
    if (lds > 48 * 1024) (void)hipFuncSetAttribute((const void *)ransac_single_finish_kernel<KM>, hipFuncAttributeMaxDynamicSharedMemorySize, (int)lds);
    hipLaunchKernelGGL(ransac_single_finish_kernel<KM>, dim3(nprob), dim3(256), lds, st, off, src, tgt, inlier_th, niter, draws, seed,
                       scratch_scores, max_n, out_model, out_inliers, out_best, E);
    return check_launch("ransac_single");
}

extern "C" int ancsh_ransac_single(int nprob, const int *off, const float *src, const float *tgt, float inlier_th, int niter,
                                   const int *draws, unsigned long long seed, int max_n, double *out_model,
                                   unsigned char *out_inliers, int *out_best, int *scratch_scores, void *stream) {
    return ransac_single_impl<KEY_VALUE>(nprob, off, src, tgt, inlier_th, niter, draws, seed, max_n, out_model, out_inliers, out_best,
                                     scratch_scores, nullptr, 0, no_extras(), stream);
}

extern "C" int ancsh_ransac_single_ex(int nprob, const int *off, const float *src, const float *tgt, float inlier_th, int niter,
                                      const int *draws, unsigned long long seed, int max_n, double *out_model,
                                      unsigned char *out_inliers, int *out_best, int *scratch_scores, float *scratch_quads,
                                      long rows, void *stream) {
    ANCSH_REQUIRE(scratch_quads, "ransac_single_ex: scratch_quads is NULL (ancsh_ransac_single is the call without it)");
    return ransac_single_impl<KEY_VALUE>(nprob, off, src, tgt, inlier_th, niter, draws, seed, max_n, out_model, out_inliers, out_best,
                                     scratch_scores, scratch_quads, rows, no_extras(), stream);
}

extern "C" int ancsh_ransac_single_rec(int nprob, const int *off, const float *src, const float *tgt, float inlier_th, int niter,
                                       const int *draws, unsigned long long seed, int max_n, double *out_model,
                                       unsigned char *out_inliers, int *out_best, int *scratch_scores, float *scratch_quads,
                                       long rows, double *record, int K, int *tie_stats, float tie_window, void *stream) {
    FitExtras E = no_extras();
    if (int rc = make_extras("ransac_single_rec", nprob, record, K, 1, tie_stats, (double)inlier_th, (double)tie_window, E)) return rc;
    return ransac_single_impl<KEY_VALUE>(nprob, off, src, tgt, inlier_th, niter, draws, seed, max_n, out_model, out_inliers, out_best,
                                     scratch_scores, scratch_quads, rows, E, stream);
}

template <int KM>
static int ransac_joint_impl(int nprob, const int *rng0, const int *rng1, const float *src, const float *tgt,
                             const float *joint_dir, double inlier_th, int niter, const int *draws,
                             KeyArg<KM> seed, int max_n, double *out_model, unsigned char *out_inliers,
                             int *out_best, double *out_score, double *scratch_scores, double *scratch_models,
                             int *lm_stat, int lm_schedule, FitExtras E, void *stream, const int *joint_kind = nullptr) {
    ANCSH_REQUIRE(lm_schedule >= ANCSH_LM_AUTO && lm_schedule <= ANCSH_LM_LATENCY, "ransac_joint: unknown lm_schedule %d", lm_schedule);
    ANCSH_REQUIRE(nprob >= 0 && niter > 0 && max_n > 0, "ransac_joint: bad sizes");
    ANCSH_REQUIRE(max_n <= 3072, "ransac_joint: max_n %d > 3072 (refit keeps both parts' inliers in LDS)", max_n);
    if (nprob == 0) return ANCSH_OK;
    ANCSH_REQUIRE(rng0 && rng1 && src && tgt && joint_dir && out_model && out_inliers && out_best && out_score &&
                      scratch_scores && scratch_models, "ransac_joint: null pointer");
    hipStream_t st = (hipStream_t)stream;
    ANCSH_REQUIRE(inlier_th > 0.0, "ransac_joint: inlier_th must be positive");
    inlier_th = sq_threshold_f64(inlier_th);
    const dim3 per_hyp((niter + 63) / 64, nprob);
    hipLaunchKernelGGL(ransac_joint_init_kernel<KM>, per_hyp, dim3(64), 0, st, rng0, rng1, src, tgt, niter, draws, seed, scratch_scores,
                       scratch_models);
    if (lm_schedule == ANCSH_LM_LATENCY) {
        const dim3 grid((niter + COOP_HYP_PER_WAVE - 1) / COOP_HYP_PER_WAVE, nprob);
        if (joint_kind)
            hipLaunchKernelGGL(ransac_joint_lm_coop_kind_kernel<KM>, grid, dim3(64), 0, st, rng0, rng1, src, tgt, joint_dir, niter, draws, seed,
                               scratch_models, lm_stat, joint_kind);
        else
            hipLaunchKernelGGL(ransac_joint_lm_coop_kernel<KM>, grid, dim3(64), 0, st,
                               rng0, rng1, src, tgt, joint_dir, niter, draws, seed, scratch_models, lm_stat);
    } else {
        const int chunk = (long)nprob * niter <= HYP_SMALL_LAUNCH ? HYP_CHUNK_SMALL : HYP_CHUNK;
        if (joint_kind)
            hipLaunchKernelGGL(ransac_joint_lm_kind_kernel<KM>, dim3((niter + chunk - 1) / chunk, nprob), dim3(64), 0, st, rng0, rng1, src, tgt,
                               joint_dir, niter, draws, seed, scratch_models, lm_stat, chunk, joint_kind);
        else
            hipLaunchKernelGGL(ransac_joint_lm_kernel<KM>, dim3((niter + chunk - 1) / chunk, nprob), dim3(64), 0, st, rng0, rng1, src, tgt,
                               joint_dir, niter, draws, seed, scratch_models, lm_stat, chunk);
    }
    hipLaunchKernelGGL(ransac_joint_model_kernel<KM>, per_hyp, dim3(64), 0, st, rng0, rng1, src, tgt, niter, draws, seed, scratch_models);
    hipLaunchKernelGGL(ransac_joint_verify_kernel, dim3((niter + 3) / 4, nprob), dim3(256), 0, st, rng0, rng1, src, tgt, inlier_th,
                       niter, scratch_models, scratch_scores);
    const size_t lds = 128 * sizeof(double) + 8 * sizeof(int) + (size_t)4 * max_n * 3 * sizeof(float);
    if (joint_kind) {
        if (lds > 48 * 1024) (void)hipFuncSetAttribute((const void *)ransac_joint_finish_kind_kernel<KM>, hipFuncAttributeMaxDynamicSharedMemorySize, (int)lds);
        hipLaunchKernelGGL(ransac_joint_finish_kind_kernel<KM>, dim3(nprob), dim3(256), lds, st, rng0, rng1, src, tgt, joint_dir, inlier_th,
                           niter, scratch_scores, scratch_models, max_n, out_model, out_inliers, out_best, out_score, E, joint_kind);
        return check_launch("ransac_joint");
    }
    if (lds > 48 * 1024) (void)hipFuncSetAttribute((const void *)ransac_joint_finish_kernel<KM>, hipFuncAttributeMaxDynamicSharedMemorySize, (int)lds);
    hipLaunchKernelGGL(ransac_joint_finish_kernel<KM>, dim3(nprob), dim3(256), lds, st, rng0, rng1, src, tgt, joint_dir, inlier_th,
                       niter, scratch_scores, scratch_models, max_n, out_model, out_inliers, out_best, out_score, E);
    return check_launch("ransac_joint");
}

static int check_joint_kind(const char *who, int nprob, const int *joint_kind) {
    if (!joint_kind || nprob <= 0) return ANCSH_OK;
    hipPointerAttribute_t at;
    if (hipPointerGetAttributes(&at, joint_kind) != hipSuccess) { (void)hipGetLastError(); return ANCSH_OK; }
    if (at.type != hipMemoryTypeHost) return ANCSH_OK;
    for (int p = 0; p < nprob; ++p)
        ANCSH_REQUIRE(joint_kind[p] == 0 || joint_kind[p] == 1, "%s: joint_kind[%d] = %d (0 revolute, 1 prismatic)", who, p, joint_kind[p]);
    return ANCSH_OK;
}

extern "C" int ancsh_ransac_joint(int nprob, const int *rng0, const int *rng1, const float *src, const float *tgt,
                                  const float *joint_dir, double inlier_th, int niter, const int *draws,
                                  unsigned long long seed, int max_n, double *out_model, unsigned char *out_inliers,
                                  int *out_best, double *out_score, double *scratch_scores, double *scratch_models,
                                  int *lm_stat, void *stream) {
    return ransac_joint_impl<KEY_VALUE>(nprob, rng0, rng1, src, tgt, joint_dir, inlier_th, niter, draws, seed, max_n, out_model, out_inliers,
                                    out_best, out_score, scratch_scores, scratch_models, lm_stat, ANCSH_LM_AUTO, no_extras(), stream);
}

extern "C" int ancsh_ransac_joint_ex(int nprob, const int *rng0, const int *rng1, const float *src, const float *tgt,
                                     const float *joint_dir, double inlier_th, int niter, const int *draws,
                                     unsigned long long seed, int max_n, double *out_model, unsigned char *out_inliers,
                                     int *out_best, double *out_score, double *scratch_scores, double *scratch_models,
                                     int *lm_stat, int lm_schedule, void *stream) {
    return ransac_joint_impl<KEY_VALUE>(nprob, rng0, rng1, src, tgt, joint_dir, inlier_th, niter, draws, seed, max_n, out_model, out_inliers,
                                    out_best, out_score, scratch_scores, scratch_models, lm_stat, lm_schedule, no_extras(), stream);
}

extern "C" int ancsh_ransac_joint_rec(int nprob, const int *rng0, const int *rng1, const float *src, const float *tgt,
                                      const float *joint_dir, double inlier_th, int niter, const int *draws,
                                      unsigned long long seed, int max_n, double *out_model, unsigned char *out_inliers,
                                      int *out_best, double *out_score, double *scratch_scores, double *scratch_models,
                                      int *lm_stat, int lm_schedule, double *record, int K, int *tie_stats, double tie_window,
                                      void *stream) {
    FitExtras E = no_extras();
    if (int rc = make_extras("ransac_joint_rec", nprob, record, K, 2, tie_stats, inlier_th, tie_window, E)) return rc;
    E.draws = draws; E.seed = seed;
    return ransac_joint_impl<KEY_VALUE>(nprob, rng0, rng1, src, tgt, joint_dir, inlier_th, niter, draws, seed, max_n, out_model, out_inliers,
                                    out_best, out_score, scratch_scores, scratch_models, lm_stat, lm_schedule, E, stream);
}

extern "C" int ancsh_ransac_single_rec_dseed(int nprob, const int *off, const float *src, const float *tgt, float inlier_th, int niter,
                                             const int *draws, const unsigned long long *seed, int max_n, double *out_model,
                                             unsigned char *out_inliers, int *out_best, int *scratch_scores, float *scratch_quads,
                                             long rows, double *record, int K, int *tie_stats, float tie_window, void *stream) {
    ANCSH_REQUIRE(seed, "ransac_single_rec_dseed: null seed pointer");
    FitExtras E = no_extras();
    if (int rc = make_extras("ransac_single_rec_dseed", nprob, record, K, 1, tie_stats, (double)inlier_th, (double)tie_window, E)) return rc;
    return ransac_single_impl<KEY_DSEED>(nprob, off, src, tgt, inlier_th, niter, draws, (unsigned long long)(uintptr_t)seed, max_n, out_model,
                                    out_inliers, out_best, scratch_scores, scratch_quads, rows, E, stream);
}

extern "C" int ancsh_ransac_joint_rec_dseed(int nprob, const int *rng0, const int *rng1, const float *src, const float *tgt,
                                            const float *joint_dir, double inlier_th, int niter, const int *draws,
                                            const unsigned long long *seed, int max_n, double *out_model, unsigned char *out_inliers,
                                            int *out_best, double *out_score, double *scratch_scores, double *scratch_models,
                                            int *lm_stat, int lm_schedule, double *record, int K, int *tie_stats, double tie_window,
                                            void *stream) {
    ANCSH_REQUIRE(seed, "ransac_joint_rec_dseed: null seed pointer");
    FitExtras E = no_extras();
    if (int rc = make_extras("ransac_joint_rec_dseed", nprob, record, K, 2, tie_stats, inlier_th, tie_window, E)) return rc;
    E.draws = draws; E.seed = (unsigned long long)(uintptr_t)seed;
    return ransac_joint_impl<KEY_DSEED>(nprob, rng0, rng1, src, tgt, joint_dir, inlier_th, niter, draws, E.seed, max_n, out_model,
                                   out_inliers, out_best, out_score, scratch_scores, scratch_models, lm_stat, lm_schedule, E, stream);
}

extern "C" int ancsh_ransac_single_rec_dkey(int nprob, const int *off, const float *src, const float *tgt, float inlier_th, int niter,
                                            const int *draws, const ancsh_stream_key *key, int max_n, double *out_model,
                                            unsigned char *out_inliers, int *out_best, int *scratch_scores, float *scratch_quads,
                                            long rows, double *record, int K, int *tie_stats, float tie_window, void *stream) {
    ANCSH_REQUIRE(key, "ransac_single_rec_dkey: null key pointer");
    ANCSH_REQUIRE(K >= 1 && nprob >= 0 && nprob % K == 0 && nprob < (1 << 20),
                  "ransac_single_rec_dkey: nprob (%d) must be a multiple of K (%d) below 2^20", nprob, K);
    FitExtras E = no_extras();
    if (int rc = make_extras("ransac_single_rec_dkey", nprob, record, K, 1, tie_stats, (double)inlier_th, (double)tie_window, E)) return rc;
    return ransac_single_impl<KEY_DKEY>(nprob, off, src, tgt, inlier_th, niter, draws, DKey{key, K}, max_n, out_model, out_inliers,
                                        out_best, scratch_scores, scratch_quads, rows, E, stream);
}

extern "C" int ancsh_ransac_joint_rec_dkey(int nprob, const int *rng0, const int *rng1, const float *src, const float *tgt,
                                           const float *joint_dir, double inlier_th, int niter, const int *draws,
                                           const ancsh_stream_key *key, int max_n, double *out_model, unsigned char *out_inliers,
                                           int *out_best, double *out_score, double *scratch_scores, double *scratch_models,
                                           int *lm_stat, int lm_schedule, double *record, int K, int *tie_stats, double tie_window,
                                           void *stream) {
    ANCSH_REQUIRE(key, "ransac_joint_rec_dkey: null key pointer");
    ANCSH_REQUIRE(K >= 2 && nprob >= 0 && nprob % (K - 1) == 0 && nprob < (1 << 20),
                  "ransac_joint_rec_dkey: nprob (%d) must be a multiple of K - 1 (K = %d >= 2) below 2^20", nprob, K);
    FitExtras E = no_extras();
    if (int rc = make_extras("ransac_joint_rec_dkey", nprob, record, K, 2, tie_stats, inlier_th, tie_window, E)) return rc;
    E.draws = draws; E.seed = (unsigned long long)(uintptr_t)key;
    return ransac_joint_impl<KEY_DKEY>(nprob, rng0, rng1, src, tgt, joint_dir, inlier_th, niter, draws, DKey{key, K - 1}, max_n,
                                       out_model, out_inliers, out_best, out_score, scratch_scores, scratch_models, lm_stat, lm_schedule,
                                       E, stream);
}

extern "C" int ancsh_ransac_joint_rec_kind(int nprob, const int *rng0, const int *rng1, const float *src, const float *tgt,
                                           const float *joint_dir, double inlier_th, int niter, const int *draws,
                                           unsigned long long seed, int max_n, double *out_model, unsigned char *out_inliers,
                                           int *out_best, double *out_score, double *scratch_scores, double *scratch_models,
                                           int *lm_stat, int lm_schedule, double *record, int K, int *tie_stats, double tie_window,
                                           const int *joint_kind, void *stream) {
    if (int rc = check_joint_kind("ransac_joint_rec_kind", nprob, joint_kind)) return rc;
    FitExtras E = no_extras();
    if (int rc = make_extras("ransac_joint_rec_kind", nprob, record, K, 2, tie_stats, inlier_th, tie_window, E)) return rc;
    E.draws = draws; E.seed = seed;
    return ransac_joint_impl<KEY_VALUE>(nprob, rng0, rng1, src, tgt, joint_dir, inlier_th, niter, draws, seed, max_n, out_model, out_inliers,
                                        out_best, out_score, scratch_scores, scratch_models, lm_stat, lm_schedule, E, stream, joint_kind);
}

extern "C" int ancsh_ransac_joint_rec_dseed_kind(int nprob, const int *rng0, const int *rng1, const float *src, const float *tgt,
                                                 const float *joint_dir, double inlier_th, int niter, const int *draws,
                                                 const unsigned long long *seed, int max_n, double *out_model,
                                                 unsigned char *out_inliers, int *out_best, double *out_score, double *scratch_scores,
                                                 double *scratch_models, int *lm_stat, int lm_schedule, double *record, int K,
                                                 int *tie_stats, double tie_window, const int *joint_kind, void *stream) {
    ANCSH_REQUIRE(seed, "ransac_joint_rec_dseed_kind: null seed pointer");
    if (int rc = check_joint_kind("ransac_joint_rec_dseed_kind", nprob, joint_kind)) return rc;
    FitExtras E = no_extras();
    if (int rc = make_extras("ransac_joint_rec_dseed_kind", nprob, record, K, 2, tie_stats, inlier_th, tie_window, E)) return rc;
    E.draws = draws; E.seed = (unsigned long long)(uintptr_t)seed;
    return ransac_joint_impl<KEY_DSEED>(nprob, rng0, rng1, src, tgt, joint_dir, inlier_th, niter, draws, E.seed, max_n, out_model,
                                        out_inliers, out_best, out_score, scratch_scores, scratch_models, lm_stat, lm_schedule, E, stream,
                                        joint_kind);
}

extern "C" int ancsh_ransac_joint_rec_dkey_kind(int nprob, const int *rng0, const int *rng1, const float *src, const float *tgt,
                                                const float *joint_dir, double inlier_th, int niter, const int *draws,
                                                const ancsh_stream_key *key, int max_n, double *out_model, unsigned char *out_inliers,
                                                int *out_best, double *out_score, double *scratch_scores, double *scratch_models,
                                                int *lm_stat, int lm_schedule, double *record, int K, int *tie_stats,
                                                double tie_window, const int *joint_kind, void *stream) {
    ANCSH_REQUIRE(key, "ransac_joint_rec_dkey_kind: null key pointer");
    ANCSH_REQUIRE(K >= 2 && nprob >= 0 && nprob % (K - 1) == 0 && nprob < (1 << 20),
                  "ransac_joint_rec_dkey_kind: nprob (%d) must be a multiple of K - 1 (K = %d >= 2) below 2^20", nprob, K);
    if (int rc = check_joint_kind("ransac_joint_rec_dkey_kind", nprob, joint_kind)) return rc;
    FitExtras E = no_extras();
    if (int rc = make_extras("ransac_joint_rec_dkey_kind", nprob, record, K, 2, tie_stats, inlier_th, tie_window, E)) return rc;
    E.draws = draws; E.seed = (unsigned long long)(uintptr_t)key;
    return ransac_joint_impl<KEY_DKEY>(nprob, rng0, rng1, src, tgt, joint_dir, inlier_th, niter, draws, DKey{key, K - 1}, max_n,
                                       out_model, out_inliers, out_best, out_score, scratch_scores, scratch_models, lm_stat, lm_schedule,
                                       E, stream, joint_kind);
}

extern "C" int ancsh_umeyama(int nprob, const int *off, const float *src, const float *tgt, double *out, void *stream) {
    ANCSH_REQUIRE(nprob >= 0, "umeyama: negative nprob");
    if (nprob == 0) return ANCSH_OK;
    ANCSH_REQUIRE(off && src && tgt && out, "umeyama: null pointer");
    hipLaunchKernelGGL(umeyama_kernel, dim3(nprob), dim3(256), 0, (hipStream_t)stream, off, src, tgt, out);
    return check_launch("umeyama");
}

extern "C" int ancsh_estimate_similarity_transform(int nprob, const int *off, const float *src, const float *tgt, int niter,
                                                   const int *draws, unsigned long long seed, double *out, int *status,
                                                   void *stream) {
    ANCSH_REQUIRE(nprob >= 0 && niter > 0 && niter <= 128, "estimate_similarity_transform: niter %d outside 1..128", niter);
    if (nprob == 0) return ANCSH_OK;
    ANCSH_REQUIRE(off && src && tgt && out && status, "estimate_similarity_transform: null pointer");
    hipLaunchKernelGGL(ransac_umeyama5_kernel, dim3(nprob), dim3(128), 0, (hipStream_t)stream, off, src, tgt, niter, draws, seed,
                       out, status);
    return check_launch("estimate_similarity_transform");
}
```

### articulated-pose_amd/pose/parallel_ancsh_pose.py

```python
import os
import pickle

import numpy as np
import torch

from .. import _lib
from .d3_utils import rot_diff_degree


def _i32(t, dev):
    if torch.is_tensor(t):
        return t.to(dev, torch.int32).contiguous()
    return torch.from_numpy(np.ascontiguousarray(t, np.int32)).to(dev)


def _f32(t, dev):
    if torch.is_tensor(t):
        return t.to(dev, torch.float32).contiguous()
    return torch.from_numpy(np.ascontiguousarray(t, np.float32)).to(dev)


TIE_WINDOW = 32 * 2.0 ** -27


def ransac_single_batch(off, src, tgt, inlier_th, niter, draws=None, seed=0, max_n=None, scalar_points=True, record=None, K=0,
                        tie_window=None, seed_dev=None, key_dev=None):
    dev = src.device
    nprob = off.numel() - 1
    rows = src.shape[0]
    max_n = int(max_n or rows)
    model = torch.empty((nprob, 13), dtype=torch.float64, device=dev)
    inl = torch.empty((rows,), dtype=torch.uint8, device=dev)
    best = torch.empty((nprob, 2), dtype=torch.int32, device=dev)
    scores = torch.empty((nprob * niter,), dtype=torch.int32, device=dev)
    d = None if draws is None else _i32(draws, dev)
    if d is not None and d.numel() != nprob * niter * 3:
        raise ValueError("draws must have shape (nprob, niter, 3)")
    quads, tie = None, None
    if scalar_points:
        quads = torch.empty((_lib.lib().ancsh_ransac_single_quads_floats(rows, nprob),), dtype=torch.float32, device=dev)
    if key_dev is not None or seed_dev is not None:
        tie = torch.empty((nprob, 2), dtype=torch.int32, device=dev) if tie_window is not None else None
        _lib.call("ancsh_ransac_single_rec_dkey" if key_dev is not None else "ancsh_ransac_single_rec_dseed", nprob, _lib.ptr(off),
                  _lib.ptr(src), _lib.ptr(tgt), float(inlier_th), int(niter), _lib.ptr(d), _lib.ptr(key_dev if key_dev is not None else seed_dev),
                  max_n, _lib.ptr(model), _lib.ptr(inl), _lib.ptr(best), _lib.ptr(scores), _lib.ptr(quads),
                  rows, _lib.ptr(record), int(K), _lib.ptr(tie), float(tie_window or 0.0))
    elif record is not None or tie_window is not None:
        tie = torch.empty((nprob, 2), dtype=torch.int32, device=dev) if tie_window is not None else None
        _lib.call("ancsh_ransac_single_rec", nprob, _lib.ptr(off), _lib.ptr(src), _lib.ptr(tgt), float(inlier_th), int(niter),
                  _lib.ptr(d), int(seed), max_n, _lib.ptr(model), _lib.ptr(inl), _lib.ptr(best), _lib.ptr(scores), _lib.ptr(quads), rows,
                  _lib.ptr(record), int(K), _lib.ptr(tie), float(tie_window or 0.0))
    elif scalar_points:
        _lib.call("ancsh_ransac_single_ex", nprob, _lib.ptr(off), _lib.ptr(src), _lib.ptr(tgt), float(inlier_th), int(niter),
                  _lib.ptr(d), int(seed), max_n, _lib.ptr(model), _lib.ptr(inl), _lib.ptr(best), _lib.ptr(scores), _lib.ptr(quads), rows)
    else:
        _lib.call("ancsh_ransac_single", nprob, _lib.ptr(off), _lib.ptr(src), _lib.ptr(tgt), float(inlier_th), int(niter),
                  _lib.ptr(d), int(seed), max_n, _lib.ptr(model), _lib.ptr(inl), _lib.ptr(best), _lib.ptr(scores))
    return dict(model=model, inliers=inl, best=best, scores=scores.view(nprob, niter), tie=tie, _keep=(d, scores, quads))


LM_SCHEDULES = {"auto": 0, "throughput": 1, "latency": 2}
JOINT_KINDS = {"revolute": 0, "prismatic": 1}


def check_joint_types(joint_types, num_parts):
    if joint_types is None:
        return None
    nj = max(int(num_parts) - 1, 0)
    if isinstance(joint_types, str):
        if joint_types not in JOINT_KINDS:
            raise ValueError("joint_types must be one of %s, got %r" % (tuple(JOINT_KINDS), joint_types))
        return (JOINT_KINDS[joint_types],) * nj
    if not isinstance(joint_types, (list, tuple)):
        raise ValueError("joint_types must be None, one of %s, or a sequence of %d of them (one per joint), got %r"
                         % (tuple(JOINT_KINDS), nj, joint_types))
    if len(joint_types) != nj:
        raise ValueError("joint_types must name the %d joints of a %d-part object, got %d entries: %r"
                         % (nj, num_parts, len(joint_types), list(joint_types)))
    for j, t in enumerate(joint_types):
        if not isinstance(t, str) or t not in JOINT_KINDS:
            raise ValueError("joint_types[%d] (joint %d) must be one of %s, got %r" % (j, j + 1, tuple(JOINT_KINDS), t))
    return tuple(JOINT_KINDS[t] for t in joint_types)


def joint_kind_tensor(kinds, B, device):
    if kinds is None:
        return None
    return torch.tensor(list(kinds) * int(B), dtype=torch.int32).to(device)


def ransac_joint_batch(rng0, rng1, src, tgt, joint_dir, inlier_th, niter, draws=None, seed=0, max_n=None, want_lm_stat=False,
                       lm_schedule="auto", record=None, K=0, tie_window=None, seed_dev=None, key_dev=None, joint_kind=None):
    dev = src.device
    nprob = rng0.shape[0]
    max_n = int(max_n or src.shape[0])
    model = torch.empty((nprob, 26), dtype=torch.float64, device=dev)
    inl = torch.empty((nprob, 2, max_n), dtype=torch.uint8, device=dev)
    best = torch.empty((nprob,), dtype=torch.int32, device=dev)
    score = torch.empty((nprob,), dtype=torch.float64, device=dev)
    sc = torch.empty((nprob * niter,), dtype=torch.float64, device=dev)
    mo = torch.empty((nprob * niter, 26), dtype=torch.float64, device=dev)
    stat = torch.empty((nprob, niter, 2), dtype=torch.int32, device=dev) if want_lm_stat else None
    d = None if draws is None else _i32(draws, dev)
    if d is not None and d.numel() != nprob * niter * 6:
        raise ValueError("draws must have shape (nprob, niter, 6)")
    tie = None
    if joint_kind is not None:
        if joint_kind.dtype != torch.int32 or joint_kind.numel() != nprob or not joint_kind.is_contiguous():
            raise ValueError("joint_kind must be a contiguous int32 tensor of %d entries (one per problem)" % nprob)
        tie = torch.empty((nprob, 2), dtype=torch.int32, device=dev) if tie_window is not None else None
        name, key = (("ancsh_ransac_joint_rec_dkey_kind", _lib.ptr(key_dev)) if key_dev is not None else
                     ("ancsh_ransac_joint_rec_dseed_kind", _lib.ptr(seed_dev)) if seed_dev is not None else
                     ("ancsh_ransac_joint_rec_kind", int(seed)))
        _lib.call(name, nprob, _lib.ptr(rng0), _lib.ptr(rng1), _lib.ptr(src), _lib.ptr(tgt), _lib.ptr(joint_dir), float(inlier_th),
                  int(niter), _lib.ptr(d), key, max_n, _lib.ptr(model), _lib.ptr(inl), _lib.ptr(best), _lib.ptr(score), _lib.ptr(sc),
                  _lib.ptr(mo), _lib.ptr(stat), LM_SCHEDULES[lm_schedule], _lib.ptr(record), int(K), _lib.ptr(tie),
                  float(tie_window or 0.0), _lib.ptr(joint_kind))
    elif key_dev is not None or seed_dev is not None:
        tie = torch.empty((nprob, 2), dtype=torch.int32, device=dev) if tie_window is not None else None
        _lib.call("ancsh_ransac_joint_rec_dkey" if key_dev is not None else "ancsh_ransac_joint_rec_dseed", nprob, _lib.ptr(rng0),
                  _lib.ptr(rng1), _lib.ptr(src), _lib.ptr(tgt), _lib.ptr(joint_dir), float(inlier_th), int(niter), _lib.ptr(d),
                  _lib.ptr(key_dev if key_dev is not None else seed_dev), max_n, _lib.ptr(model), _lib.ptr(inl), _lib.ptr(best),
                  _lib.ptr(score), _lib.ptr(sc), _lib.ptr(mo), _lib.ptr(stat), LM_SCHEDULES[lm_schedule], _lib.ptr(record), int(K),
                  _lib.ptr(tie), float(tie_window or 0.0))
    elif record is not None or tie_window is not None:
        tie = torch.empty((nprob, 2), dtype=torch.int32, device=dev) if tie_window is not None else None
        _lib.call("ancsh_ransac_joint_rec", nprob, _lib.ptr(rng0), _lib.ptr(rng1), _lib.ptr(src), _lib.ptr(tgt), _lib.ptr(joint_dir),
                  float(inlier_th), int(niter), _lib.ptr(d), int(seed), max_n, _lib.ptr(model), _lib.ptr(inl), _lib.ptr(best),
                  _lib.ptr(score), _lib.ptr(sc), _lib.ptr(mo), _lib.ptr(stat), LM_SCHEDULES[lm_schedule], _lib.ptr(record), int(K),
                  _lib.ptr(tie), float(tie_window or 0.0))
    else:
        _lib.call("ancsh_ransac_joint_ex", nprob, _lib.ptr(rng0), _lib.ptr(rng1), _lib.ptr(src), _lib.ptr(tgt), _lib.ptr(joint_dir),
                  float(inlier_th), int(niter), _lib.ptr(d), int(seed), max_n, _lib.ptr(model), _lib.ptr(inl), _lib.ptr(best),
                  _lib.ptr(score), _lib.ptr(sc), _lib.ptr(mo), _lib.ptr(stat), LM_SCHEDULES[lm_schedule])
    return dict(model=model, inliers=inl, best=best, score=score, lm_stat=stat, hyp_models=mo, hyp_scores=sc, tie=tie, _keep=(d, joint_kind))


def draws_from_seed(seed, counts, niter_a, niter_b):
    rs = np.random.RandomState(seed)
    K = len(counts)
    da = np.zeros((K, niter_a, 3), np.int32)
    for j in range(K):
        for i in range(niter_a):
            da[j, i] = rs.randint(counts[j], size=3)
    db = np.zeros((max(K - 1, 0), niter_b, 6), np.int32)
    for j in range(1, K):
        for i in range(niter_b):
            db[j - 1, i, :3] = rs.randint(counts[0], size=3)
            db[j - 1, i, 3:] = rs.randint(counts[j], size=3)
    return da, db


class PoseSolver(object):

    def __init__(self, num_parts, inlier_th=0.1, niter_a=10000, niter_b=200, device="cuda:0", want_lm_stat=False,
                 max_part_points=None, lm_schedule="auto", tie_window=TIE_WINDOW, joint_types=None):
        kinds = check_joint_types(joint_types, num_parts)
        self.joint_kinds = kinds if kinds is not None and any(kinds) else None
        self._kind_dev = {}
        self.K, self.th, self.niter_a, self.niter_b = num_parts, inlier_th, niter_a, niter_b
        self.tie_window = tie_window
        self.device = torch.device(device)
        self.max_part_points = max_part_points
        if lm_schedule not in LM_SCHEDULES:
            raise ValueError("lm_schedule must be one of %s" % sorted(LM_SCHEDULES))
        self.lm_schedule = lm_schedule
        self.want_lm_stat = want_lm_stat

    def prepare(self, B):
        if self.joint_kinds is None or self.K < 2:
            return None
        if B not in self._kind_dev:
            self._kind_dev[B] = joint_kind_tensor(self.joint_kinds, B, self.device)
        return self._kind_dev[B]

    def solve(self, P, nocs_pred, mask_pred, joint_axis_per_point, joint_cls=None, draws_a=None, draws_b=None, seed=0, seed_dev=None,
              key_dev=None, joint_index=None, fit_quality=False, ground_truth=None):
        _one_association(joint_cls, joint_index)
        if fit_quality:
            from .quality import check_fit_quality
            check_fit_quality(True, self.th)
        out = self._partition(P, nocs_pred, mask_pred)
        self._stage_b_fits(out, joint_axis_per_point, joint_cls, draws_b, seed, seed_dev, key_dev, joint_index)
        out = self._poison(self._stage_a_fits(out, draws_a, seed, seed_dev, key_dev))
        if fit_quality:
            from .quality import fit_quality_batch
            out["record_wide"] = fit_quality_batch(out, self.th)
        if ground_truth is not None:
            from .gt_errors import gt_error_batch
            P32, nocs32, mask32 = out["_inputs"]
            out["record_gt"] = gt_error_batch(P32, nocs32, mask32, out["record_wide"] if fit_quality else out["record"], ground_truth)
        return out

    def solve_stage_a(self, P, nocs_pred, mask_pred, draws_a=None, seed=0):
        out = self._partition(P, nocs_pred, mask_pred)
        if self.K > 1:
            out["record"][:, :, 13:] = float("nan")
        return self._poison(self._stage_a_fits(out, draws_a, seed))

    def _poison(self, out):
        B, N = out["_shape"]
        P, nocs, W = out["_inputs"]
        axis = out.get("_axis")
        index = out.get("_index")
        if index is not None:
            _lib.call("ancsh_pose_poison_records_pred", B, N, self.K, _lib.ptr(P), _lib.ptr(nocs), _lib.ptr(W), _lib.ptr(axis),
                      int(index.shape[2]), _lib.ptr(index), _lib.ptr(out["record"]))
        else:
            _lib.call("ancsh_pose_poison_records", B, N, self.K, _lib.ptr(P), _lib.ptr(nocs), _lib.ptr(W), _lib.ptr(axis),
                      _lib.ptr(out["record"]))
        return out

    def _partition(self, P, nocs_pred, mask_pred):
        dev, K = self.device, self.K
        P, nocs, W = _f32(P, dev), _f32(nocs_pred, dev), _f32(mask_pred, dev)
        B, N, _ = P.shape
        if nocs.shape != (B, N, 3 * K) or W.shape != (B, N, K):
            raise ValueError("nocs_pred must be (B,N,3K) and mask_pred (B,N,K)")
        max_n = min(N, self.max_part_points or N)
        labels = torch.empty((B, N), dtype=torch.int32, device=dev)
        pidx = torch.empty((B, N), dtype=torch.int32, device=dev)
        off = torch.empty((B * K + 1,), dtype=torch.int32, device=dev)
        src = torch.empty((B * N, 3), dtype=torch.float32, device=dev)
        tgt = torch.empty((B * N, 3), dtype=torch.float32, device=dev)
        counts = torch.empty((B, K), dtype=torch.int32, device=dev)
        rng0 = torch.empty((B * max(K - 1, 1), 2), dtype=torch.int32, device=dev) if K > 1 else None
        rng1 = torch.empty((B * max(K - 1, 1), 2), dtype=torch.int32, device=dev) if K > 1 else None
        _lib.call("ancsh_pose_partition", B, N, K, _lib.ptr(W), _lib.ptr(P), _lib.ptr(nocs), _lib.ptr(labels), _lib.ptr(pidx),
                  _lib.ptr(off), _lib.ptr(src), _lib.ptr(tgt), _lib.ptr(counts), _lib.ptr(rng0), _lib.ptr(rng1))
        record = torch.empty((B, K, 26), dtype=torch.float64, device=dev)
        return dict(labels=labels, part_index=pidx, off=off, counts=counts, record=record, _src=src, _tgt=tgt, _max_n=max_n, _shape=(B, N),
                    _rng=(rng0, rng1), _inputs=(P, nocs, W))

    def _stage_a_fits(self, out, draws_a=None, seed=0, seed_dev=None, key_dev=None):
        dev, K = self.device, self.K
        B, N = out["_shape"]
        a = ransac_single_batch(out["off"], out["_src"], out["_tgt"], self.th, self.niter_a,
                                None if draws_a is None else _i32(draws_a, dev).reshape(B * K, self.niter_a, 3), seed, out["_max_n"],
                                record=out["record"], K=K, tie_window=self.tie_window, seed_dev=seed_dev, key_dev=key_dev)
        out.update(baseline=out["record"][:, :, :13], best_a=a["best"].view(B, K, 2), inliers_a=a["inliers"].view(B, N))
        if a["tie"] is not None:
            out["tie_a"] = a["tie"].view(B, K, 2)
        if K == 1:
            out["nonlinear"] = out["record"][:, :, 13:]
        return out

    def solve_stage_b(self, out, joint_axis_per_point, joint_cls=None, draws_b=None, seed=0, seed_dev=None, key_dev=None,
                      joint_index=None):
        _one_association(joint_cls, joint_index)
        return self._poison(self._stage_b_fits(out, joint_axis_per_point, joint_cls, draws_b, seed, seed_dev, key_dev, joint_index))

    def _stage_b_fits(self, out, joint_axis_per_point, joint_cls, draws_b=None, seed=0, seed_dev=None, key_dev=None, joint_index=None):
        dev, K = self.device, self.K
        B, N = out["_shape"]
        src, tgt, max_n = out["_src"], out["_tgt"], out["_max_n"]
        rng0, rng1 = out["_rng"]
        if K > 1:
            axis = _f32(joint_axis_per_point, dev)
            out["_axis"] = axis
            jdir = torch.empty((B, K - 1, 3), dtype=torch.float32, device=dev)
            if joint_index is not None:
                index = _f32(joint_index, dev)
                if index.dim() != 3 or tuple(index.shape[:2]) != (B, N):
                    raise ValueError("joint_index must be (B, N, C) for %d clouds of %d points, got %s" % (B, N, tuple(index.shape)))
                out["_index"] = index
                _lib.call("ancsh_pose_joint_direction_pred", B, N, K, int(index.shape[2]), _lib.ptr(axis), _lib.ptr(index), _lib.ptr(jdir))
            else:
                jcls = _i32(joint_cls, dev)
                _lib.call("ancsh_pose_joint_direction", B, N, K, _lib.ptr(axis), _lib.ptr(jcls), _lib.ptr(jdir))
            b = ransac_joint_batch(rng0, rng1, src, tgt, jdir.view(-1, 3), self.th, self.niter_b,
                                   None if draws_b is None else _i32(draws_b, dev).reshape(B * (K - 1), self.niter_b, 6),
                                   seed + 1, max_n, want_lm_stat=self.want_lm_stat, lm_schedule=self.lm_schedule,
                                   record=out["record"], K=K, tie_window=self.tie_window, seed_dev=seed_dev, key_dev=key_dev,
                                   joint_kind=self.prepare(B))
            if self.want_lm_stat:
                out["lm_stat"] = b["lm_stat"].view(B, K - 1, self.niter_b, 2)
            out["nonlinear"] = out["record"][:, :, 13:]
            if b["tie"] is not None:
                out["tie_b"] = b["tie"].view(B, K - 1, 2)
            out["best_b"] = b["best"].view(B, K - 1)
            out["score_b"] = b["score"].view(B, K - 1)
            out["joint_direction"] = jdir
            out["inliers_b"] = b["inliers"].view(B, K - 1, 2, max_n)
        else:
            out["nonlinear"] = out["record"][:, :, 13:]
        return out


def _one_association(joint_cls, joint_index):
    if (joint_cls is None) == (joint_index is None):
        raise ValueError("give exactly one of joint_cls (a label per point) and joint_index (the index_per_point head), got %s"
                         % ("both" if joint_cls is not None else "neither"))


def _model_to_rst(m):
    return m[:9].reshape(3, 3), m[9], m[10:13]


def records_from_solution(sol, rts_list=None):
    base = sol["baseline"].cpu().numpy()
    nonl = sol["nonlinear"].cpu().numpy()
    B, K, _ = base.shape
    recs = []
    for b in range(B):
        scale_dict = {'gt': [], 'baseline': [], 'nonlinear': []}
        r_dict = {'gt': [], 'baseline': [], 'nonlinear': []}
        t_dict = {'gt': [], 'baseline': [], 'nonlinear': []}
        xyz_err = {'baseline': [], 'nonlinear': []}
        rpy_err = {'baseline': [], 'nonlinear': []}
        scale_err = {'baseline': [], 'nonlinear': []}
        for j in range(K):
            for kind, arr in (('baseline', base), ('nonlinear', nonl)):
                R, s, t = _model_to_rst(arr[b, j])
                scale_dict[kind].append(s)
                r_dict[kind].append(R)
                t_dict[kind].append(t)
                if rts_list is not None:
                    rt_gt, s_gt = rts_list[b]['rt']['gt'][j], rts_list[b]['scale']['gt'][j]
                    rpy_err[kind].append(rot_diff_degree(R, rt_gt[:3, :3]))
                    xyz_err[kind].append(np.linalg.norm(t - rt_gt[:3, 3]))
                    scale_err[kind].append(np.linalg.norm(s - s_gt[0]))
            if rts_list is not None:
                scale_dict['gt'].append(rts_list[b]['scale']['gt'][j][0])
                r_dict['gt'].append(rts_list[b]['rt']['gt'][j][:3, :3])
                t_dict['gt'].append(rts_list[b]['rt']['gt'][j][:3, 3])
        recs.append({'scale': scale_dict, 'rotation': r_dict, 'translation': t_dict, 'xyz_err': xyz_err,
                     'rpy_err': rpy_err, 'scale_err': scale_err})
    return recs


JOINT_SOURCES = ("gt", "predicted")


def solver_ransac_nonlinear(s_ind, e_ind, test_exp, baseline_exp, choose_threshold, num_parts, test_group, problem_ins,
                            rts_all, file_name, base_path=None, batch_size=32, seed=0, device="cuda:0", joint_source="gt",
                            joint_types=None):
    if joint_source not in JOINT_SOURCES:
        raise ValueError("joint_source must be one of %s, got %r" % (JOINT_SOURCES, joint_source))
    check_joint_types(joint_types, num_parts)
    from .. import prediction_io
    base_path = base_path or os.environ.get("ANCSH_BASE_PATH", ".")
    solver = PoseSolver(num_parts, choose_threshold, device=device, joint_types=joint_types)
    names = [test_group[i].split('.')[0] for i in range(s_ind, e_ind) if test_group[i].split('_')[0] not in problem_ins]
    all_rts = {}
    for c0 in range(0, len(names), batch_size):
        chunk = names[c0:c0 + batch_size]
        f = [prediction_io.load_record(os.path.join(base_path, 'results/test_pred', str(test_exp)), n) for n in chunk]
        fb = [prediction_io.load_record(os.path.join(base_path, 'results/test_pred', str(baseline_exp)), n) for n in chunk]
        sol = solver.solve(np.stack([r['P'][:, :3] for r in f]), np.stack([r['nocs_per_point'] for r in fb]),
                           np.stack([r['instance_per_point'] for r in fb]), np.stack([r['joint_axis_per_point'] for r in f]),
                           **({"joint_index": np.stack([r['index_per_point'] for r in f])} if joint_source == "predicted" else
                              {"joint_cls": np.stack([r['joint_cls_gt'] for r in f])}), seed=seed + c0)
        gts = [rts_all[n] for n in chunk] if rts_all is not None else None
        for n, rec in zip(chunk, records_from_solution(sol, gts)):
            all_rts[n] = rec
    with open(file_name, 'wb') as fh:
        pickle.dump(all_rts, fh)
    return all_rts
```

### include/ancsh_hip.h

```cpp
#ifndef ANCSH_HIP_H
#define ANCSH_HIP_H

#ifdef __cplusplus
extern "C" {
#endif

#define ANCSH_OK 0
#define ANCSH_EINVAL (-1)
#define ANCSH_EHIP (-2)

#define ANCSH_ACT_NONE 0
#define ANCSH_ACT_RELU 1
#define ANCSH_MAX_GROUPS 4
#define ANCSH_ACT_RAW 2

int ancsh_abi_version(void);
const char *ancsh_last_error(void);


int ancsh_farthest_point_sample(int b, int n, int m, const float *inp, float *temp, int *out, void *stream);

int ancsh_farthest_point_sample_gather(int b, int n, int m, const float *inp, float *temp, int *out_idx, float *out_xyz,
                                       void *stream);

int ancsh_prob_sample(int b, int n, int m, const float *inp_p, const float *inp_r, float *temp, int *out, void *stream);

int ancsh_gather_point(int b, int n, int m, const float *inp, const int *idx, float *out, void *stream);

int ancsh_query_ball_point(int b, int n, int m, float radius, int nsample, const float *xyz1, const float *xyz2,
                           int *idx, int *pts_cnt, void *stream);

int ancsh_query_ball_point_multi(int nprob, const int *b, const int *n, const int *m, const float *radius, const int *nsample,
                                 const float *const *xyz1, const float *const *xyz2, int *const *idx, int *const *pts_cnt,
                                 void *stream);

int ancsh_query_ball_group_xyz(int b, int n, int m, float radius, int nsample, const float *xyz1, const float *xyz2, int center,
                               int *idx, int *pts_cnt, float *grouped_xyz, int out_ld, void *stream);
int ancsh_query_ball_group_xyz_multi(int nprob, const int *b, const int *n, const int *m, const float *radius, const int *nsample,
                                     const float *const *xyz1, const float *const *xyz2, const int *center, int *const *idx,
                                     int *const *pts_cnt, float *const *grouped_xyz, const int *out_ld, void *stream);

int ancsh_group_point(int b, int n, int c, int m, int nsample, const float *points, const int *idx, float *out,
                      void *stream);

int ancsh_group_point_multi(int nprob, const int *b, const int *n, const int *c, const int *m, const int *nsample,
                            const float *const *points, const int *const *idx, float *const *out, void *stream);

int ancsh_selection_sort(int b, int n, int m, int k, const float *dist, int *outi, float *out, void *stream);

int ancsh_knn_point(int b, int n, int m, int c, int k, const float *xyz1, const float *xyz2, float *val, int *idx, void *stream);

int ancsh_group_point_ex(int b, int n, int c, int m, int nsample, const float *points, const int *idx,
                         const float *center, float *out, int out_ld, int out_off, void *stream);

int ancsh_three_nn(int b, int n, int m, const float *xyz1, const float *xyz2, float *dist, int *idx, void *stream);

int ancsh_three_weights(int rows, const float *dist, float *weight, void *stream);

int ancsh_three_nn_weights(int b, int n, int m, const float *xyz1, const float *xyz2, float *dist, int *idx, float *weight,
                           void *stream);

int ancsh_three_interpolate(int b, int m, int c, int n, const float *points, const int *idx, const float *weight,
                            float *out, void *stream);

int ancsh_three_interpolate_ex(int b, int m, int c, int n, const float *points, const int *idx,
                               const float *weight, float *out, int out_ld, int out_off, void *stream);

int ancsh_fp_interpolate_concat(int b, int m, int c2, int n, const float *points2, const int *idx, const float *weight,
                                const float *points1, int c1, float *out, int out_ld, void *stream);

int ancsh_fp_interpolate_concat_ex(int b, int m, int c2, int n, const float *points2, const int *idx, const float *weight,
                                   const float *points1, int c1, float *out, int out_ld, int geo_batch, int points1_batch,
                                   void *stream);


int ancsh_conv1x1(long rows, int cin, int cout, const float *x, int ldx, const float *w, const float *bias,
                  const float *scale, const float *shift, int act, float *y, int ldy, int pool, void *stream);

int ancsh_conv1x1_ex(long rows, int cin, int cout, const float *x, int ldx, const float *w, const float *bias,
                     const float *scale, const float *shift, int act, float *y, int ldy, int pool, const float *acc_init,
                     int init_rows, void *stream);

int ancsh_conv1x1_packed(long rows, int cin, int cout, const float *x, int ldx, const float *w_packed, const float *bias,
                         const float *scale, const float *shift, int act, float *y, int ldy, int pool,
                         const float *acc_init, int init_rows, void *stream);

int ancsh_conv1x1_packed_grouped(int ngroups, long rows, int cin, int cout, const float *x, int ldx,
                                 const float *const *w_packed, const float *const *bias, const float *const *scale,
                                 const float *const *shift, int act, float *y, int ldy, int pool, const float *acc_init,
                                 int init_rows, void *stream);
int ancsh_conv1x1_grouped(int ngroups, long rows, int cin, int cout, const float *x, int ldx, const float *const *w,
                          const float *const *bias, const float *const *scale, const float *const *shift, int act, float *y,
                          int ldy, int pool, void *stream);

int ancsh_sa_module_fused(int b, int n, int m, int nsample, int cfeat, int c1, int c2, int c3, const float *xyz,
                          const float *feats, const float *new_xyz, const int *idx, const float *const *params, float *out,
                          void *stream);
int ancsh_sa_module_fused_partial(int b, int n, int m, int nsample, int c1, int c2, int c3, const float *xyz,
                                  const float *partial, const float *new_xyz, const int *idx, const float *const *params,
                                  float *out, void *stream);

int ancsh_sa_module_fused_grouped(int ngroups, int b, int n, int m, int nsample, int cfeat, int c1, int c2, int c3,
                                  const float *xyz, const float *feats, const float *new_xyz, const int *idx,
                                  const float *const *params, float *out, void *stream);
int ancsh_sa_module_fused_partial_grouped(int ngroups, int b, int n, int m, int nsample, int c1, int c2, int c3,
                                          const float *xyz, const float *partial, const float *new_xyz, const int *idx,
                                          const float *const *params, float *out, void *stream);

long ancsh_sa_packed_weight_bytes_bf16x3(int k, int n);
int ancsh_sa_pack_weights_bf16x3(int k, int n, const float *w, void *packed, void *stream);
int ancsh_sa_module_fused_bf16x3(int b, int n, int m, int nsample, int cfeat, int c1, int c2, int c3, const float *xyz,
                                 const float *feats, const float *new_xyz, const int *idx, const float *const *params, float *out,
                                 void *stream);
int ancsh_sa_module_fused_partial_bf16x3(int b, int n, int m, int nsample, int c1, int c2, int c3, const float *xyz,
                                         const float *partial, const float *new_xyz, const int *idx, const float *const *params,
                                         float *out, void *stream);
int ancsh_sa_module_fused_bf16x3_grouped(int ngroups, int b, int n, int m, int nsample, int cfeat, int c1, int c2, int c3,
                                         const float *xyz, const float *feats, const float *new_xyz, const int *idx,
                                         const float *const *params, float *out, void *stream);
int ancsh_sa_module_fused_partial_bf16x3_grouped(int ngroups, int b, int n, int m, int nsample, int c1, int c2, int c3,
                                                 const float *xyz, const float *partial, const float *new_xyz, const int *idx,
                                                 const float *const *params, float *out, void *stream);
long ancsh_sa_packed_weight_bytes_f16x2(int k, int n);
int ancsh_sa_pack_weights_f16x2(int k, int n, const float *w, void *packed, void *stream);
int ancsh_sa_module_fused_f16x2_grouped(int ngroups, int b, int n, int m, int nsample, int cfeat, int c1, int c2, int c3,
                                        const float *xyz, const float *feats, const float *new_xyz, const int *idx,
                                        const float *const *params, float *out, void *stream);
int ancsh_sa_module_fused_partial_f16x2_grouped(int ngroups, int b, int n, int m, int nsample, int c1, int c2, int c3,
                                                const float *xyz, const float *partial, const float *new_xyz, const int *idx,
                                                const float *const *params, float *out, void *stream);
int ancsh_sa_module_fused_f16x2_grouped_guarded(int ngroups, int b, int n, int m, int nsample, int cfeat, int c1, int c2, int c3,
                                                const float *xyz, const float *feats, const float *new_xyz, const int *idx,
                                                const float *const *params, float *out, unsigned *range_flags, int flag_bit0, void *stream);
int ancsh_sa_module_fused_partial_f16x2_grouped_guarded(int ngroups, int b, int n, int m, int nsample, int c1, int c2, int c3,
                                                        const float *xyz, const float *partial, const float *new_xyz, const int *idx,
                                                        const float *const *params, float *out, unsigned *range_flags, int flag_bit0,
                                                        void *stream);

long ancsh_sa_packed_weight_floats(int k, int n);
int ancsh_sa_pack_weights(int k, int n, const float *w, float *packed, void *stream);

int ancsh_mlp_chain(long rows, int cin, const float *x, int ldx, int nops, const int *ops, const void *const *ptrs,
                    void *stream);

int ancsh_mlp_chain_grouped(int ngroups, long rows, int cin, const float *x, int ldx, const int *nops, const int *const *ops,
                            const void *const *const *ptrs, float *scratch, void *stream);

int ancsh_sa3_chain_grouped(int ngroups, int b, int npts, int cfeat, int c1, int c2, int c3, const float *xyz, const float *feats,
                            const float *const *params, float *out, void *stream);
int ancsh_fp_single_source_init(int ngroups, int b, int cin, int cout, int nparts, const float *x, const float *const *w, float *y,
                                void *stream);
int ancsh_fp1_chain_grouped(int ngroups, int b, int npts, int cskip, int c1, int c2, const float *skip, const float *init,
                            const float *const *params, float *out, void *stream);
int ancsh_fp2_chain_grouped(int ngroups, int b, int m, int n, int c2, int c1, int n1, int n2, const float *points2, const int *idx,
                            const float *weight, const float *points1, const float *const *params, float *out, void *stream);

int ancsh_last_ball_query_schedule(void);

int ancsh_mlp_chain_grouped_fp(int ngroups, int b, int n, int m, int c2, const float *points2, const int *idx, const float *weight,
                               const float *xyz, const int *nops, const int *const *ops, const void *const *const *ptrs, float *scratch,
                               void *stream);

int ancsh_mlp_chain_grouped_fp_bf16x3(int ngroups, int b, int n, int m, int c2, const float *points2, const int *idx, const float *weight,
                                      const float *xyz, const int *nops, const int *const *ops, const void *const *const *ptrs,
                                      void *stream);
int ancsh_mlp_chain_grouped_fp_f16x2(int ngroups, int b, int n, int m, int c2, const float *points2, const int *idx, const float *weight,
                                     const float *xyz, const int *nops, const int *const *ops, const void *const *const *ptrs,
                                     void *stream);
int ancsh_mlp_chain_grouped_fp_f16x2_guarded(int ngroups, int b, int n, int m, int c2, const float *points2, const int *idx, const float *weight,
                                             const float *xyz, const int *nops, const int *const *ops, const void *const *const *ptrs,
                                             unsigned *range_flags, int flag_bit0, void *stream);

int ancsh_sa3_chain_grouped_bf16x3(int ngroups, int b, int npts, int cfeat, int c1, int c2, int c3, const float *xyz, const float *feats,
                                   const float *const *params, float *out, void *stream);
int ancsh_sa3_chain_grouped_f16x2(int ngroups, int b, int npts, int cfeat, int c1, int c2, int c3, const float *xyz, const float *feats,
                                  const float *const *params, float *out, void *stream);
int ancsh_fp1_chain_grouped_bf16x3(int ngroups, int b, int npts, int cskip, int c1, int c2, const float *skip, const float *init,
                                   const float *const *params, float *out, void *stream);
int ancsh_fp1_chain_grouped_f16x2(int ngroups, int b, int npts, int cskip, int c1, int c2, const float *skip, const float *init,
                                  const float *const *params, float *out, void *stream);
int ancsh_fp2_chain_grouped_bf16x3(int ngroups, int b, int m, int n, int c2, int c1, int n1, int n2, const float *points2, const int *idx,
                                   const float *weight, const float *points1, const float *const *params, float *out, void *stream);
int ancsh_fp2_chain_grouped_f16x2(int ngroups, int b, int m, int n, int c2, int c1, int n1, int n2, const float *points2, const int *idx,
                                  const float *weight, const float *points1, const float *const *params, float *out, void *stream);
int ancsh_sa3_chain_grouped_f16x2_guarded(int ngroups, int b, int npts, int cfeat, int c1, int c2, int c3, const float *xyz, const float *feats,
                                          const float *const *params, float *out, unsigned *range_flags, int flag_bit0, void *stream);
int ancsh_fp1_chain_grouped_f16x2_guarded(int ngroups, int b, int npts, int cskip, int c1, int c2, const float *skip, const float *init,
                                          const float *const *params, float *out, unsigned *range_flags, int flag_bit0, void *stream);
int ancsh_fp2_chain_grouped_f16x2_guarded(int ngroups, int b, int m, int n, int c2, int c1, int n1, int n2, const float *points2, const int *idx,
                                          const float *weight, const float *points1, const float *const *params, float *out,
                                          unsigned *range_flags, int flag_bit0, void *stream);

int ancsh_group_max(long groups, int nsample, int c, const float *x, float *y, void *stream);

int ancsh_head_activations(long rows, int K, int mixed_pred, const float *logits, int ld, float *W, float *nocs,
                           float *confi, float *heatmap, float *unitvec, float *axis, float *joint_cls,
                           float *gocs, float *scale, float *trans, void *stream);


int ancsh_pose_partition(int b, int n, int K, const float *W, const float *P, const float *nocs, int *labels,
                         int *part_index, int *off, float *src, float *tgt, int *counts, int *rng0, int *rng1, void *stream);

int ancsh_pose_poison_records(int b, int n, int K, const float *P, const float *nocs, const float *W, const float *joint_axis,
                              double *record, void *stream);

int ancsh_pose_poison_records_pred(int b, int n, int K, const float *P, const float *nocs, const float *W, const float *joint_axis,
                                   int joint_channels, const float *joint_index, double *record, void *stream);

int ancsh_pose_joint_direction(int b, int n, int K, const float *joint_axis, const int *joint_cls, float *out,
                               void *stream);

int ancsh_pose_joint_direction_pred(int b, int n, int K, int joint_channels, const float *joint_axis, const float *joint_index,
                                    float *out, void *stream);

int ancsh_ransac_single(int nprob, const int *off, const float *src, const float *tgt, float inlier_th, int niter,
                        const int *draws, unsigned long long seed, int max_n, double *out_model,
                        unsigned char *out_inliers, int *out_best, int *scratch_scores, void *stream);

long ancsh_ransac_single_quads_floats(long rows, int nprob);
int ancsh_ransac_single_ex(int nprob, const int *off, const float *src, const float *tgt, float inlier_th, int niter,
                           const int *draws, unsigned long long seed, int max_n, double *out_model,
                           unsigned char *out_inliers, int *out_best, int *scratch_scores, float *scratch_quads, long rows,
                           void *stream);

int ancsh_ransac_single_rec(int nprob, const int *off, const float *src, const float *tgt, float inlier_th, int niter,
                            const int *draws, unsigned long long seed, int max_n, double *out_model, unsigned char *out_inliers,
                            int *out_best, int *scratch_scores, float *scratch_quads, long rows, double *record, int K,
                            int *tie_stats, float tie_window, void *stream);

int ancsh_ransac_joint(int nprob, const int *rng0, const int *rng1, const float *src, const float *tgt,
                       const float *joint_dir, double inlier_th, int niter, const int *draws,
                       unsigned long long seed, int max_n, double *out_model, unsigned char *out_inliers,
                       int *out_best, double *out_score, double *scratch_scores, double *scratch_models,
                       int *lm_stat, void *stream);

#define ANCSH_LM_AUTO 0
#define ANCSH_LM_THROUGHPUT 1
#define ANCSH_LM_LATENCY 2
int ancsh_ransac_joint_ex(int nprob, const int *rng0, const int *rng1, const float *src, const float *tgt,
                          const float *joint_dir, double inlier_th, int niter, const int *draws,
                          unsigned long long seed, int max_n, double *out_model, unsigned char *out_inliers,
                          int *out_best, double *out_score, double *scratch_scores, double *scratch_models,
                          int *lm_stat, int lm_schedule, void *stream);

int ancsh_ransac_joint_rec(int nprob, const int *rng0, const int *rng1, const float *src, const float *tgt,
                           const float *joint_dir, double inlier_th, int niter, const int *draws, unsigned long long seed,
                           int max_n, double *out_model, unsigned char *out_inliers, int *out_best, double *out_score,
                           double *scratch_scores, double *scratch_models, int *lm_stat, int lm_schedule, double *record, int K,
                           int *tie_stats, double tie_window, void *stream);

int ancsh_ransac_single_rec_dseed(int nprob, const int *off, const float *src, const float *tgt, float inlier_th, int niter,
                                  const int *draws, const unsigned long long *seed, int max_n, double *out_model,
                                  unsigned char *out_inliers, int *out_best, int *scratch_scores, float *scratch_quads, long rows,
                                  double *record, int K, int *tie_stats, float tie_window, void *stream);
int ancsh_ransac_joint_rec_dseed(int nprob, const int *rng0, const int *rng1, const float *src, const float *tgt,
                                 const float *joint_dir, double inlier_th, int niter, const int *draws, const unsigned long long *seed,
                                 int max_n, double *out_model, unsigned char *out_inliers, int *out_best, double *out_score,
                                 double *scratch_scores, double *scratch_models, int *lm_stat, int lm_schedule, double *record, int K,
                                 int *tie_stats, double tie_window, void *stream);

typedef struct {
    unsigned long long seed;
    int cloud_base;
    int reserved;
} ancsh_stream_key;

int ancsh_ransac_single_rec_dkey(int nprob, const int *off, const float *src, const float *tgt, float inlier_th, int niter,
                                 const int *draws, const ancsh_stream_key *key, int max_n, double *out_model,
                                 unsigned char *out_inliers, int *out_best, int *scratch_scores, float *scratch_quads, long rows,
                                 double *record, int K, int *tie_stats, float tie_window, void *stream);
int ancsh_ransac_joint_rec_dkey(int nprob, const int *rng0, const int *rng1, const float *src, const float *tgt,
                                const float *joint_dir, double inlier_th, int niter, const int *draws, const ancsh_stream_key *key,
                                int max_n, double *out_model, unsigned char *out_inliers, int *out_best, double *out_score,
                                double *scratch_scores, double *scratch_models, int *lm_stat, int lm_schedule, double *record, int K,
                                int *tie_stats, double tie_window, void *stream);

#define ANCSH_JOINT_REVOLUTE 0
#define ANCSH_JOINT_PRISMATIC 1
int ancsh_ransac_joint_rec_kind(int nprob, const int *rng0, const int *rng1, const float *src, const float *tgt,
                                const float *joint_dir, double inlier_th, int niter, const int *draws, unsigned long long seed,
                                int max_n, double *out_model, unsigned char *out_inliers, int *out_best, double *out_score,
                                double *scratch_scores, double *scratch_models, int *lm_stat, int lm_schedule, double *record, int K,
                                int *tie_stats, double tie_window, const int *joint_kind, void *stream);
int ancsh_ransac_joint_rec_dseed_kind(int nprob, const int *rng0, const int *rng1, const float *src, const float *tgt,
                                      const float *joint_dir, double inlier_th, int niter, const int *draws,
                                      const unsigned long long *seed, int max_n, double *out_model, unsigned char *out_inliers,
                                      int *out_best, double *out_score, double *scratch_scores, double *scratch_models, int *lm_stat,
                                      int lm_schedule, double *record, int K, int *tie_stats, double tie_window, const int *joint_kind,
                                      void *stream);
int ancsh_ransac_joint_rec_dkey_kind(int nprob, const int *rng0, const int *rng1, const float *src, const float *tgt,
                                     const float *joint_dir, double inlier_th, int niter, const int *draws, const ancsh_stream_key *key,
                                     int max_n, double *out_model, unsigned char *out_inliers, int *out_best, double *out_score,
                                     double *scratch_scores, double *scratch_models, int *lm_stat, int lm_schedule, double *record, int K,
                                     int *tie_stats, double tie_window, const int *joint_kind, void *stream);

int ancsh_umeyama(int nprob, const int *off, const float *src, const float *tgt, double *out, void *stream);

int ancsh_estimate_similarity_transform(int nprob, const int *off, const float *src, const float *tgt, int niter,
                                        const int *draws, unsigned long long seed, double *out, int *status, void *stream);

int ancsh_iou_3d(int npairs, int nres, const double *bbox1, const double *bbox2, double *iou, long *counts, void *stream);

int ancsh_joint_params(int b, int n, int K, int gocs_channels, int axis_mean, const float *gocs, const float *nocs,
                       const float *mask, const float *heatmap, const float *unitvec, const float *joint_axis,
                       const int *joint_cls, double *st, double *joint, void *stream);

int ancsh_part_extents(int b, int n, int K, int nocs_channels, const float *nocs, const float *mask, const float *P, int ldp,
                       const double *pose0, float *scale_pred, double *dynam, int *count, void *stream);

#define ANCSH_ARTICULATION_MAX_N 4096
int ancsh_articulation_rec(int b, int n, int K, int gocs_channels, int joint_channels, const float *gocs, const float *nocs,
                           const float *mask, const float *heatmap, const float *unitvec, const float *joint_axis,
                           const float *joint_index, const float *npcs_nocs, const float *npcs_mask, const double *record,
                           double *art, double *joint_nocs, double *st0, float *extent, void *stream);

int ancsh_joint_state_rec(int b, int n, int K, const float *P, int ldp, const float *npcs_nocs, const float *npcs_mask,
                          const double *record, const double *art, double *wide, void *stream);

#define ANCSH_FIT_QUALITY_MAX_N 8192
int ancsh_fit_quality_rec(int b, int K, const int *off, const float *src, const float *tgt, const double *record, double inlier_th,
                          const int *best_a, const double *score_b, double *wide, void *stream);

int ancsh_gt_error_rec(int b, int n, int K, int nres, const float *P, int ldp, const float *npcs_nocs, const float *npcs_mask,
                       const double *record, int ld, const double *gt, double *wide, void *stream);


int ancsh_input_sample(int nclouds, int num_points, int nchan, const float *rows, const int *offsets, const int *perm,
                       const float *norm_factor, int cls_col, int jcls_col, int n_parts, float *P, float *chan_out,
                       float *mask_array, float *joint_cls_mask, void *stream);

int ancsh_input_sample_stream(int nclouds, int num_points, int nchan, const float *rows, long capacity, const int *offsets,
                              const float *norm_factor, int jcls_col, const unsigned long long *seed, float *P, int *joint_cls,
                              int *perm_out, void *stream);

int ancsh_input_sample_stream_keyed(int nclouds, int num_points, int nchan, const float *rows, long capacity, const int *offsets,
                                    const float *norm_factor, int jcls_col, const ancsh_stream_key *key, float *P, int *joint_cls,
                                    int *perm_out, void *stream);

int ancsh_input_sample_stream_xyz(int nclouds, int num_points, int nchan, const float *rows, long capacity, const int *offsets,
                                  const float *norm_factor, const unsigned long long *seed, float *P, int *perm_out, void *stream);
int ancsh_input_sample_stream_xyz_keyed(int nclouds, int num_points, int nchan, const float *rows, long capacity, const int *offsets,
                                        const float *norm_factor, const ancsh_stream_key *key, float *P, int *perm_out, void *stream);

#define ANCSH_DEPTH_U16 0
#define ANCSH_DEPTH_F32 1
#define ANCSH_DEPTH_MAX_CHUNKS 64
int ancsh_depth_unproject_stream(int nclouds, int depth_type, const void *depth, const unsigned char *mask, long pixel_capacity,
                                 const int *geom, const float *cam, float *rows, long capacity, int *offsets, int *counts, int *scratch,
                                 void *stream);

#define ANCSH_LABEL_NAN_BITS 0x7fc00000u
int ancsh_depth_label_images(int nclouds, int depth_type, const void *depth, const unsigned char *mask, long pixel_capacity,
                             const int *geom, const int *offsets, const int *scratch, const int *labels, const float *values,
                             long capacity, const int *dest, int *img_labels, float *img_values, long image_capacity, void *stream);

int ancsh_raw_point_labels(int nclouds, int num_points, int K, int gocs_channels, int nchan, const float *rows, long capacity,
                           const int *offsets, const float *norm_factor, const float *P, const float *W, const float *nocs,
                           const float *gocs, int *labels, float *values, void *stream);


int ancsh_test_losses(int b, int n, int K, int type_l, const void *const *ptrs, float *out, void *stream);

#ifdef __cplusplus
}
#endif
#endif
```

Before: 17720.

## Fuse joint LM refinement and single-part RANSAC finish into one pose-fit launch

Adds a combined pose_fit_rec entry point that launches the joint-RANSAC LM hypothesis kernel and the single-part RANSAC finish kernel as one grid. Leading blocks run four LM chunks each, one per wave; trailing blocks each run a single-part finish problem. The goal is to cut kernel launches and let the two independent stages fill the GPU together instead of running back to back. The risk is higher LDS and register use from mixing heterogeneous block work in one kernel. The Python path is rerouted to use the fused call.

```diff
diff --git a/articulated-pose_amd/_lib.py b/articulated-pose_amd/_lib.py
--- a/articulated-pose_amd/_lib.py
+++ b/articulated-pose_amd/_lib.py
@@ -112,6 +112,11 @@
     "ancsh_joint_state_rec": [_c_int] * 3 + [_vp, _c_int] + [_vp] * 5 + [_vp],
     "ancsh_fit_quality_rec": [_c_int] * 2 + [_vp] * 4 + [ctypes.c_double] + [_vp] * 3 + [_vp],
     "ancsh_gt_error_rec": [_c_int] * 4 + [_vp, _c_int] + [_vp] * 3 + [_c_int] + [_vp] * 2 + [_vp],
+    **{"ancsh_pose_fit_rec" + sfx: [_c_int, _vp, _vp, _vp, _c_float, _c_int, _vp, key, _c_int, _vp, _vp, _vp, _vp, _vp, _c_long, _vp, _c_float,
+                                    _c_int, _vp, _vp, _vp, ctypes.c_double, _c_int, _vp, key] + [_vp] * 7 + [_c_int, _vp, ctypes.c_double,
+                                    _vp, _c_int] + kind + [_vp]
+       for sfx, key, kind in (("", ctypes.c_ulonglong, []), ("_dseed", _vp, []), ("_dkey", _vp, []),
+                              ("_kind", ctypes.c_ulonglong, [_vp]), ("_dseed_kind", _vp, [_vp]), ("_dkey_kind", _vp, [_vp]))},
     "ancsh_input_sample": [_c_int, _c_int, _c_int, _vp, _vp, _vp, _vp, _c_int, _c_int, _c_int, _vp, _vp, _vp, _vp, _vp],
     "ancsh_test_losses": [_c_int, _c_int, _c_int, _c_int, _vp, _vp, _vp],
     "ancsh_ransac_joint_ex": [_c_int, _vp, _vp, _vp, _vp, _vp, ctypes.c_double, _c_int, _vp, ctypes.c_ulonglong, _c_int]
diff --git a/articulated-pose_amd/csrc/pose.hip b/articulated-pose_amd/csrc/pose.hip
--- a/articulated-pose_amd/csrc/pose.hip
+++ b/articulated-pose_amd/csrc/pose.hip
@@ -438,21 +438,18 @@
 }
 
 template <int KM>
-__global__ __launch_bounds__(256) void ransac_single_finish_kernel(const int *__restrict__ off, const float *__restrict__ src,
-                                                                   const float *__restrict__ tgt, float th, int niter,
-                                                                   const int *__restrict__ draws, KeyArg<KM> seed_arg,
-                                                                   const int *__restrict__ scores, int max_n,
-                                                                   double *__restrict__ out_model,
-                                                                   unsigned char *__restrict__ out_inliers,
-                                                                   int *__restrict__ out_best, FitExtras E) {
+__device__ __forceinline__ void ransac_single_finish_run(int prob, unsigned char *smem, const int *__restrict__ off,
+                                                         const float *__restrict__ src, const float *__restrict__ tgt, float th, int niter,
+                                                         const int *__restrict__ draws, KeyArg<KM> seed_arg,
+                                                         const int *__restrict__ scores, int max_n, double *__restrict__ out_model,
+                                                         unsigned char *__restrict__ out_inliers, int *__restrict__ out_best,
+                                                         const FitExtras &E) {
     const unsigned long long seed = kernel_seed<KM>(seed_arg, 0);
     const int kbase = key_problem_base<KM>(seed_arg);
-    extern __shared__ __attribute__((aligned(16))) unsigned char smem[];
     double *red = (double *)smem;
     int *wcnt = (int *)(red + 64);
     float(*cs)[3] = (float(*)[3])(wcnt + 8);
     float(*ct)[3] = cs + max_n;
-    const int prob = blockIdx.x;
     const int r0 = off[prob], n = off[prob + 1] - r0;
     double *om = out_model + (size_t)prob * MODEL_A;
     if (n <= 0 || n > max_n) {
@@ -576,6 +573,18 @@
     }
 }
 
+template <int KM>
+__global__ __launch_bounds__(256) void ransac_single_finish_kernel(const int *__restrict__ off, const float *__restrict__ src,
+                                                                   const float *__restrict__ tgt, float th, int niter,
+                                                                   const int *__restrict__ draws, KeyArg<KM> seed_arg,
+                                                                   const int *__restrict__ scores, int max_n,
+                                                                   double *__restrict__ out_model,
+                                                                   unsigned char *__restrict__ out_inliers,
+                                                                   int *__restrict__ out_best, FitExtras E) {
+    extern __shared__ __attribute__((aligned(16))) unsigned char smem[];
+    ransac_single_finish_run<KM>(blockIdx.x, smem, off, src, tgt, th, niter, draws, seed_arg, scores, max_n, out_model, out_inliers, out_best, E);
+}
+
 struct PartFd {
     Rod b, p[3];
     double rh[3];
@@ -847,15 +856,15 @@
                                                     const float *__restrict__ src, const float *__restrict__ tgt,
                                                     const float *__restrict__ joint_dir, int niter,
                                                     const int *__restrict__ draws, KeyArg<KM> seed_arg,
-                                                    double *__restrict__ models, int *__restrict__ lm_stat, int chunk) {
+                                                    double *__restrict__ models, int *__restrict__ lm_stat, int chunk, int prob,
+                                                    int chunk_idx) {
     const unsigned long long seed = kernel_seed<KM>(seed_arg, 1);
     const int kbase = key_problem_base<KM>(seed_arg);
-    const int prob = blockIdx.y;
     const int a0 = rng0[prob * 2], n0 = rng0[prob * 2 + 1] - a0;
     const int a1 = rng1[prob * 2], n1 = rng1[prob * 2 + 1] - a1;
     if (n0 <= 0 || n1 <= 0) return;
-    const int c1 = min(niter, (int)(blockIdx.x + 1) * chunk);
-    int next = blockIdx.x * chunk;
+    const int c1 = min(niter, (chunk_idx + 1) * chunk);
+    int next = chunk_idx * chunk;
     HypProblemT<PRISM> P;
     if constexpr (!PRISM) {
         P.J[0] = joint_dir[prob * 3]; P.J[1] = joint_dir[prob * 3 + 1]; P.J[2] = joint_dir[prob * 3 + 2];
@@ -907,7 +916,7 @@
                                                              const float *__restrict__ joint_dir, int niter,
                                                              const int *__restrict__ draws, KeyArg<KM> seed_arg,
                                                              double *__restrict__ models, int *__restrict__ lm_stat, int chunk) {
-    ransac_joint_lm_run<KM, false>(rng0, rng1, src, tgt, joint_dir, niter, draws, seed_arg, models, lm_stat, chunk);
+    ransac_joint_lm_run<KM, false>(rng0, rng1, src, tgt, joint_dir, niter, draws, seed_arg, models, lm_stat, chunk, blockIdx.y, blockIdx.x);
 }
 
 template <int KM>
@@ -917,8 +926,64 @@
                                                                   const int *__restrict__ draws, KeyArg<KM> seed_arg,
                                                                   double *__restrict__ models, int *__restrict__ lm_stat, int chunk,
                                                                   const int *__restrict__ joint_kind) {
-    if (joint_kind[blockIdx.y] != 0) ransac_joint_lm_run<KM, true>(rng0, rng1, src, tgt, joint_dir, niter, draws, seed_arg, models, lm_stat, chunk);
-    else ransac_joint_lm_run<KM, false>(rng0, rng1, src, tgt, joint_dir, niter, draws, seed_arg, models, lm_stat, chunk);
+    if (joint_kind[blockIdx.y] != 0) ransac_joint_lm_run<KM, true>(rng0, rng1, src, tgt, joint_dir, niter, draws, seed_arg, models, lm_stat, chunk, blockIdx.y, blockIdx.x);
+    else ransac_joint_lm_run<KM, false>(rng0, rng1, src, tgt, joint_dir, niter, draws, seed_arg, models, lm_stat, chunk, blockIdx.y, blockIdx.x);
+}
+
+struct LmArgs {
+    const int *rng0, *rng1;
+    const float *joint_dir;
+    int niter;
+    const int *draws;
+    double *models;
+    int *lm_stat;
+    int chunk, chunks_per_prob, n_chunks, n_lm;
+};
+struct FinishAArgs {
+    const int *off;
+    float th;
+    int niter;
+    const int *draws, *scores;
+    int max_n;
+    double *out_model;
+    unsigned char *out_inliers;
+    int *out_best;
+};
+
+template <int KM, bool KIND>
+__device__ __forceinline__ void pose_lm_finish_a_run(unsigned char *smem, const float *__restrict__ src, const float *__restrict__ tgt,
+                                                     const LmArgs &L, KeyArg<KM> seed_b, const int *__restrict__ joint_kind,
+                                                     const FinishAArgs &A, KeyArg<KM> seed_a, const FitExtras &EA) {
+    if ((int)blockIdx.x >= L.n_lm) {
+        ransac_single_finish_run<KM>((int)blockIdx.x - L.n_lm, smem, A.off, src, tgt, A.th, A.niter, A.draws, seed_a, A.scores, A.max_n,
+                                     A.out_model, A.out_inliers, A.out_best, EA);
+        return;
+    }
+    const int chunk_id = (int)blockIdx.x * 4 + __builtin_amdgcn_readfirstlane((int)(threadIdx.x >> 6));
+    if (chunk_id >= L.n_chunks) return;
+    const int prob = chunk_id / L.chunks_per_prob, chunk_idx = chunk_id - prob * L.chunks_per_prob;
+    if constexpr (KIND) {
+        if (joint_kind[prob] != 0) {
+            ransac_joint_lm_run<KM, true>(L.rng0, L.rng1, src, tgt, L.joint_dir, L.niter, L.draws, seed_b, L.models, L.lm_stat, L.chunk, prob, chunk_idx);
+            return;
+        }
+    }
+    ransac_joint_lm_run<KM, false>(L.rng0, L.rng1, src, tgt, L.joint_dir, L.niter, L.draws, seed_b, L.models, L.lm_stat, L.chunk, prob, chunk_idx);
+}
+
+template <int KM>
+__global__ __launch_bounds__(256) void pose_lm_finish_a_kernel(const float *__restrict__ src, const float *__restrict__ tgt, LmArgs L,
+                                                               KeyArg<KM> seed_b, FinishAArgs A, KeyArg<KM> seed_a, FitExtras EA) {
+    extern __shared__ __attribute__((aligned(16))) unsigned char smem[];
+    pose_lm_finish_a_run<KM, false>(smem, src, tgt, L, seed_b, nullptr, A, seed_a, EA);
+}
+
+template <int KM>
+__global__ __launch_bounds__(256) void pose_lm_finish_a_kind_kernel(const float *__restrict__ src, const float *__restrict__ tgt, LmArgs L,
+                                                                    KeyArg<KM> seed_b, const int *__restrict__ joint_kind, FinishAArgs A,
+                                                                    KeyArg<KM> seed_a, FitExtras EA) {
+    extern __shared__ __attribute__((aligned(16))) unsigned char smem[];
+    pose_lm_finish_a_run<KM, true>(smem, src, tgt, L, seed_b, joint_kind, A, seed_a, EA);
 }
 
 constexpr int COOP_G = 8;
@@ -1999,30 +2064,51 @@
     return 24 * single_quads_needed(rows, nprob);
 }
 
+static int ransac_single_check(int nprob, const int *off, const float *src, const float *tgt, float inlier_th, int niter, int max_n,
+                               double *out_model, unsigned char *out_inliers, int *out_best, int *scratch_scores, float *scratch_quads,
+                               long rows) {
+    ANCSH_REQUIRE(nprob >= 0 && niter > 0 && max_n > 0, "ransac_single: bad sizes nprob=%d niter=%d max_n=%d", nprob, niter, max_n);
+    ANCSH_REQUIRE(max_n <= 6144, "ransac_single: max_n %d > 6144 (refit keeps the inliers in LDS)", max_n);
+    if (nprob == 0) return ANCSH_OK;
+    ANCSH_REQUIRE(off && src && tgt && out_model && out_inliers && out_best && scratch_scores, "ransac_single: null pointer");
+    ANCSH_REQUIRE(inlier_th > 0.f, "ransac_single: inlier_th must be positive");
+    const float th_sq = sq_threshold_f32(inlier_th);
+    if (scratch_quads && th_sq >= 0x1p-100f && th_sq < 4.0f) {
+        ANCSH_REQUIRE(rows >= 0 && rows < (1L << 30), "ransac_single_ex: rows=%ld out of range", rows);
+        ANCSH_REQUIRE((((uintptr_t)scratch_quads) & 31) == 0, "ransac_single_ex: scratch_quads must be 32-byte aligned");
+    }
+    return ANCSH_OK;
+}
+
+template <int KM>
+static void ransac_single_launch_score(int nprob, const int *off, const float *src, const float *tgt, float th_sq, int niter,
+                                       const int *draws, KeyArg<KM> seed, int max_n, int *scratch_scores, float *scratch_quads, long rows,
+                                       hipStream_t st) {
+    if (scratch_quads && th_sq >= 0x1p-100f && th_sq < 4.0f) {
+        const int cap = (int)single_quads_needed(rows, nprob);
+        hipLaunchKernelGGL(soa_quads_kernel, dim3((max_n + 7 + 255) / 256, nprob), dim3(256), 0, st, off, src, tgt, scratch_quads, cap);
+        hipLaunchKernelGGL(ransac_single_score_sreg_kernel<KM>, dim3((niter + 255) / 256, nprob), dim3(256), 0, st, off, src, tgt,
+                           (const float *)scratch_quads, cap, th_sq, niter, draws, seed, scratch_scores);
+    } else {
+        hipLaunchKernelGGL(ransac_single_score_kernel<KM>, dim3((niter + 255) / 256, nprob), dim3(256), 0, st, off, src, tgt, th_sq,
+                           niter, draws, seed, scratch_scores);
+    }
+}
+
+static size_t single_finish_lds(int max_n) { return 64 * sizeof(double) + 8 * sizeof(int) + (size_t)2 * max_n * 3 * sizeof(float); }
+
 template <int KM>
 static int ransac_single_impl(int nprob, const int *off, const float *src, const float *tgt, float inlier_th, int niter,
                               const int *draws, KeyArg<KM> seed, int max_n, double *out_model,
                               unsigned char *out_inliers, int *out_best, int *scratch_scores, float *scratch_quads, long rows,
                               FitExtras E, void *stream) {
-    ANCSH_REQUIRE(nprob >= 0 && niter > 0 && max_n > 0, "ransac_single: bad sizes nprob=%d niter=%d max_n=%d", nprob, niter, max_n);
-    ANCSH_REQUIRE(max_n <= 6144, "ransac_single: max_n %d > 6144 (refit keeps the inliers in LDS)", max_n);
+    if (int rc = ransac_single_check(nprob, off, src, tgt, inlier_th, niter, max_n, out_model, out_inliers, out_best, scratch_scores,
+                                     scratch_quads, rows)) return rc;
     if (nprob == 0) return ANCSH_OK;
-    ANCSH_REQUIRE(off && src && tgt && out_model && out_inliers && out_best && scratch_scores, "ransac_single: null pointer");
     hipStream_t st = (hipStream_t)stream;
-    ANCSH_REQUIRE(inlier_th > 0.f, "ransac_single: inlier_th must be positive");
     inlier_th = sq_threshold_f32(inlier_th);
-    if (scratch_quads && inlier_th >= 0x1p-100f && inlier_th < 4.0f) {
-        ANCSH_REQUIRE(rows >= 0 && rows < (1L << 30), "ransac_single_ex: rows=%ld out of range", rows);
-        ANCSH_REQUIRE((((uintptr_t)scratch_quads) & 31) == 0, "ransac_single_ex: scratch_quads must be 32-byte aligned");
-        const int cap = (int)single_quads_needed(rows, nprob);
-        hipLaunchKernelGGL(soa_quads_kernel, dim3((max_n + 7 + 255) / 256, nprob), dim3(256), 0, st, off, src, tgt, scratch_quads, cap);
-        hipLaunchKernelGGL(ransac_single_score_sreg_kernel<KM>, dim3((niter + 255) / 256, nprob), dim3(256), 0, st, off, src, tgt,
-                           (const float *)scratch_quads, cap, inlier_th, niter, draws, seed, scratch_scores);
-    } else {
-        hipLaunchKernelGGL(ransac_single_score_kernel<KM>, dim3((niter + 255) / 256, nprob), dim3(256), 0, st, off, src, tgt, inlier_th,
-                           niter, draws, seed, scratch_scores);
-    }
-    const size_t lds = 64 * sizeof(double) + 8 * sizeof(int) + (size_t)2 * max_n * 3 * sizeof(float);
+    ransac_single_launch_score<KM>(nprob, off, src, tgt, inlier_th, niter, draws, seed, max_n, scratch_scores, scratch_quads, rows, st);
+    const size_t lds = single_finish_lds(max_n);
     if (lds > 48 * 1024) (void)hipFuncSetAttribute((const void *)ransac_single_finish_kernel<KM>, hipFuncAttributeMaxDynamicSharedMemorySize, (int)lds);
     hipLaunchKernelGGL(ransac_single_finish_kernel<KM>, dim3(nprob), dim3(256), lds, st, off, src, tgt, inlier_th, niter, draws, seed,
                        scratch_scores, max_n, out_model, out_inliers, out_best, E);
@@ -2055,20 +2141,53 @@
                                      scratch_scores, scratch_quads, rows, E, stream);
 }
 
+static int ransac_joint_check(int nprob, const int *rng0, const int *rng1, const float *src, const float *tgt, const float *joint_dir,
+                              double inlier_th, int niter, int max_n, double *out_model, unsigned char *out_inliers, int *out_best,
+                              double *out_score, double *scratch_scores, double *scratch_models, int lm_schedule) {
+    ANCSH_REQUIRE(lm_schedule >= ANCSH_LM_AUTO && lm_schedule <= ANCSH_LM_LATENCY, "ransac_joint: unknown lm_schedule %d", lm_schedule);
+    ANCSH_REQUIRE(nprob >= 0 && niter > 0 && max_n > 0, "ransac_joint: bad sizes");
+    ANCSH_REQUIRE(max_n <= 3072, "ransac_joint: max_n %d > 3072 (refit keeps both parts' inliers in LDS)", max_n);
+    if (nprob == 0) return ANCSH_OK;
+    ANCSH_REQUIRE(rng0 && rng1 && src && tgt && joint_dir && out_model && out_inliers && out_best && out_score &&
+                      scratch_scores && scratch_models, "ransac_joint: null pointer");
+    ANCSH_REQUIRE(inlier_th > 0.0, "ransac_joint: inlier_th must be positive");
+    return ANCSH_OK;
+}
+
+static int lm_chunk(int nprob, int niter) { return (long)nprob * niter <= HYP_SMALL_LAUNCH ? HYP_CHUNK_SMALL : HYP_CHUNK; }
+
+template <int KM>
+static void ransac_joint_launch_tail(int nprob, const int *rng0, const int *rng1, const float *src, const float *tgt,
+                                     const float *joint_dir, double th_sq, int niter, const int *draws, KeyArg<KM> seed, int max_n,
+                                     double *out_model, unsigned char *out_inliers, int *out_best, double *out_score,
+                                     double *scratch_scores, double *scratch_models, const FitExtras &E, hipStream_t st,
+                                     const int *joint_kind) {
+    hipLaunchKernelGGL(ransac_joint_model_kernel<KM>, dim3((niter + 63) / 64, nprob), dim3(64), 0, st, rng0, rng1, src, tgt, niter, draws, seed,
+                       scratch_models);
+    hipLaunchKernelGGL(ransac_joint_verify_kernel, dim3((niter + 3) / 4, nprob), dim3(256), 0, st, rng0, rng1, src, tgt, th_sq,
+                       niter, scratch_models, scratch_scores);
+    const size_t lds = 128 * sizeof(double) + 8 * sizeof(int) + (size_t)4 * max_n * 3 * sizeof(float);
+    if (joint_kind) {
+        if (lds > 48 * 1024) (void)hipFuncSetAttribute((const void *)ransac_joint_finish_kind_kernel<KM>, hipFuncAttributeMaxDynamicSharedMemorySize, (int)lds);
+        hipLaunchKernelGGL(ransac_joint_finish_kind_kernel<KM>, dim3(nprob), dim3(256), lds, st, rng0, rng1, src, tgt, joint_dir, th_sq,
+                           niter, scratch_scores, scratch_models, max_n, out_model, out_inliers, out_best, out_score, E, joint_kind);
+        return;
+    }
+    if (lds > 48 * 1024) (void)hipFuncSetAttribute((const void *)ransac_joint_finish_kernel<KM>, hipFuncAttributeMaxDynamicSharedMemorySize, (int)lds);
+    hipLaunchKernelGGL(ransac_joint_finish_kernel<KM>, dim3(nprob), dim3(256), lds, st, rng0, rng1, src, tgt, joint_dir, th_sq,
+                       niter, scratch_scores, scratch_models, max_n, out_model, out_inliers, out_best, out_score, E);
+}
+
 template <int KM>
 static int ransac_joint_impl(int nprob, const int *rng0, const int *rng1, const float *src, const float *tgt,
                              const float *joint_dir, double inlier_th, int niter, const int *draws,
                              KeyArg<KM> seed, int max_n, double *out_model, unsigned char *out_inliers,
                              int *out_best, double *out_score, double *scratch_scores, double *scratch_models,
                              int *lm_stat, int lm_schedule, FitExtras E, void *stream, const int *joint_kind = nullptr) {
-    ANCSH_REQUIRE(lm_schedule >= ANCSH_LM_AUTO && lm_schedule <= ANCSH_LM_LATENCY, "ransac_joint: unknown lm_schedule %d", lm_schedule);
-    ANCSH_REQUIRE(nprob >= 0 && niter > 0 && max_n > 0, "ransac_joint: bad sizes");
-    ANCSH_REQUIRE(max_n <= 3072, "ransac_joint: max_n %d > 3072 (refit keeps both parts' inliers in LDS)", max_n);
+    if (int rc = ransac_joint_check(nprob, rng0, rng1, src, tgt, joint_dir, inlier_th, niter, max_n, out_model, out_inliers, out_best,
+                                    out_score, scratch_scores, scratch_models, lm_schedule)) return rc;
     if (nprob == 0) return ANCSH_OK;
-    ANCSH_REQUIRE(rng0 && rng1 && src && tgt && joint_dir && out_model && out_inliers && out_best && out_score &&
-                      scratch_scores && scratch_models, "ransac_joint: null pointer");
     hipStream_t st = (hipStream_t)stream;
-    ANCSH_REQUIRE(inlier_th > 0.0, "ransac_joint: inlier_th must be positive");
     inlier_th = sq_threshold_f64(inlier_th);
     const dim3 per_hyp((niter + 63) / 64, nprob);
     hipLaunchKernelGGL(ransac_joint_init_kernel<KM>, per_hyp, dim3(64), 0, st, rng0, rng1, src, tgt, niter, draws, seed, scratch_scores,
@@ -2082,7 +2201,7 @@
             hipLaunchKernelGGL(ransac_joint_lm_coop_kernel<KM>, grid, dim3(64), 0, st,
                                rng0, rng1, src, tgt, joint_dir, niter, draws, seed, scratch_models, lm_stat);
     } else {
-        const int chunk = (long)nprob * niter <= HYP_SMALL_LAUNCH ? HYP_CHUNK_SMALL : HYP_CHUNK;
+        const int chunk = lm_chunk(nprob, niter);
         if (joint_kind)
             hipLaunchKernelGGL(ransac_joint_lm_kind_kernel<KM>, dim3((niter + chunk - 1) / chunk, nprob), dim3(64), 0, st, rng0, rng1, src, tgt,
                                joint_dir, niter, draws, seed, scratch_models, lm_stat, chunk, joint_kind);
@@ -2090,19 +2209,8 @@
             hipLaunchKernelGGL(ransac_joint_lm_kernel<KM>, dim3((niter + chunk - 1) / chunk, nprob), dim3(64), 0, st, rng0, rng1, src, tgt,
                                joint_dir, niter, draws, seed, scratch_models, lm_stat, chunk);
     }
-    hipLaunchKernelGGL(ransac_joint_model_kernel<KM>, per_hyp, dim3(64), 0, st, rng0, rng1, src, tgt, niter, draws, seed, scratch_models);
-    hipLaunchKernelGGL(ransac_joint_verify_kernel, dim3((niter + 3) / 4, nprob), dim3(256), 0, st, rng0, rng1, src, tgt, inlier_th,
-                       niter, scratch_models, scratch_scores);
-    const size_t lds = 128 * sizeof(double) + 8 * sizeof(int) + (size_t)4 * max_n * 3 * sizeof(float);
-    if (joint_kind) {
-        if (lds > 48 * 1024) (void)hipFuncSetAttribute((const void *)ransac_joint_finish_kind_kernel<KM>, hipFuncAttributeMaxDynamicSharedMemorySize, (int)lds);
-        hipLaunchKernelGGL(ransac_joint_finish_kind_kernel<KM>, dim3(nprob), dim3(256), lds, st, rng0, rng1, src, tgt, joint_dir, inlier_th,
-                           niter, scratch_scores, scratch_models, max_n, out_model, out_inliers, out_best, out_score, E, joint_kind);
-        return check_launch("ransac_joint");
-    }
-    if (lds > 48 * 1024) (void)hipFuncSetAttribute((const void *)ransac_joint_finish_kernel<KM>, hipFuncAttributeMaxDynamicSharedMemorySize, (int)lds);
-    hipLaunchKernelGGL(ransac_joint_finish_kernel<KM>, dim3(nprob), dim3(256), lds, st, rng0, rng1, src, tgt, joint_dir, inlier_th,
-                       niter, scratch_scores, scratch_models, max_n, out_model, out_inliers, out_best, out_score, E);
+    ransac_joint_launch_tail<KM>(nprob, rng0, rng1, src, tgt, joint_dir, inlier_th, niter, draws, seed, max_n, out_model, out_inliers, out_best,
+                                 out_score, scratch_scores, scratch_models, E, st, joint_kind);
     return check_launch("ransac_joint");
 }
 
@@ -2250,6 +2358,139 @@
                                        E, stream, joint_kind);
 }
 
+template <int KM>
+static int pose_fit_impl(int nprob_a, const int *off, const float *src, const float *tgt, float inlier_th_a, int niter_a,
+                         const int *draws_a, KeyArg<KM> seed_a, int max_n, double *out_model_a, unsigned char *out_inliers_a,
+                         int *out_best_a, int *scratch_scores_a, float *scratch_quads, long rows, const FitExtras &EA, int nprob_b,
+                         const int *rng0, const int *rng1, const float *joint_dir, double inlier_th_b, int niter_b, const int *draws_b,
+                         KeyArg<KM> seed_b, double *out_model_b, unsigned char *out_inliers_b, int *out_best_b, double *out_score_b,
+                         double *scratch_scores_b, double *scratch_models_b, int *lm_stat, int lm_schedule, const FitExtras &EB,
+                         const int *joint_kind, void *stream) {
+    if (int rc = ransac_single_check(nprob_a, off, src, tgt, inlier_th_a, niter_a, max_n, out_model_a, out_inliers_a, out_best_a,
+                                     scratch_scores_a, scratch_quads, rows)) return rc;
+    if (int rc = ransac_joint_check(nprob_b, rng0, rng1, src, tgt, joint_dir, inlier_th_b, niter_b, max_n, out_model_b, out_inliers_b,
+                                    out_best_b, out_score_b, scratch_scores_b, scratch_models_b, lm_schedule)) return rc;
+    if (nprob_a == 0 && nprob_b == 0) return ANCSH_OK;
+    if (nprob_a == 0 || nprob_b == 0 || lm_schedule == ANCSH_LM_LATENCY) {
+        if (int rc = ransac_joint_impl<KM>(nprob_b, rng0, rng1, src, tgt, joint_dir, inlier_th_b, niter_b, draws_b, seed_b, max_n, out_model_b,
+                                           out_inliers_b, out_best_b, out_score_b, scratch_scores_b, scratch_models_b, lm_stat, lm_schedule, EB,
+                                           stream, joint_kind)) return rc;
+        return ransac_single_impl<KM>(nprob_a, off, src, tgt, inlier_th_a, niter_a, draws_a, seed_a, max_n, out_model_a, out_inliers_a,
+                                      out_best_a, scratch_scores_a, scratch_quads, rows, EA, stream);
+    }
+    LmArgs L;
+    L.chunk = lm_chunk(nprob_b, niter_b);
+    L.chunks_per_prob = (niter_b + L.chunk - 1) / L.chunk;
+    const long n_chunks = (long)L.chunks_per_prob * nprob_b;
+    ANCSH_REQUIRE((n_chunks + 3) / 4 + nprob_a < (1L << 31), "pose_fit: %ld LM chunks + %d parts exceed one grid", n_chunks, nprob_a);
+    hipStream_t st = (hipStream_t)stream;
+    const float th_a = sq_threshold_f32(inlier_th_a);
+    const double th_b = sq_threshold_f64(inlier_th_b);
+    ransac_single_launch_score<KM>(nprob_a, off, src, tgt, th_a, niter_a, draws_a, seed_a, max_n, scratch_scores_a, scratch_quads, rows, st);
+    hipLaunchKernelGGL(ransac_joint_init_kernel<KM>, dim3((niter_b + 63) / 64, nprob_b), dim3(64), 0, st, rng0, rng1, src, tgt, niter_b, draws_b,
+                       seed_b, scratch_scores_b, scratch_models_b);
+    L.rng0 = rng0; L.rng1 = rng1; L.joint_dir = joint_dir; L.niter = niter_b; L.draws = draws_b; L.models = scratch_models_b; L.lm_stat = lm_stat;
+    L.n_chunks = (int)n_chunks;
+    L.n_lm = (int)((n_chunks + 3) / 4);
+    FinishAArgs A;
+    A.off = off; A.th = th_a; A.niter = niter_a; A.draws = draws_a; A.scores = scratch_scores_a; A.max_n = max_n;
+    A.out_model = out_model_a; A.out_inliers = out_inliers_a; A.out_best = out_best_a;
+    const size_t lds = single_finish_lds(max_n);
+    const dim3 grid(L.n_lm + nprob_a);
+    if (joint_kind) {
+        if (lds > 48 * 1024) (void)hipFuncSetAttribute((const void *)pose_lm_finish_a_kind_kernel<KM>, hipFuncAttributeMaxDynamicSharedMemorySize, (int)lds);
+        hipLaunchKernelGGL(pose_lm_finish_a_kind_kernel<KM>, grid, dim3(256), lds, st, src, tgt, L, seed_b, joint_kind, A, seed_a, EA);
+    } else {
+        if (lds > 48 * 1024) (void)hipFuncSetAttribute((const void *)pose_lm_finish_a_kernel<KM>, hipFuncAttributeMaxDynamicSharedMemorySize, (int)lds);
+        hipLaunchKernelGGL(pose_lm_finish_a_kernel<KM>, grid, dim3(256), lds, st, src, tgt, L, seed_b, A, seed_a, EA);
+    }
+    ransac_joint_launch_tail<KM>(nprob_b, rng0, rng1, src, tgt, joint_dir, th_b, niter_b, draws_b, seed_b, max_n, out_model_b, out_inliers_b,
+                                 out_best_b, out_score_b, scratch_scores_b, scratch_models_b, EB, st, joint_kind);
+    return check_launch("pose_fit");
+}
+
+static int pose_fit_extras(const char *who, int nprob_a, int nprob_b, double *record, int K, int *tie_a, float inlier_th_a, float tie_window_a,
+                           int *tie_b, double inlier_th_b, double tie_window_b, const int *draws_b, unsigned long long seed_b, FitExtras &EA,
+                           FitExtras &EB) {
+    EA = no_extras(); EB = no_extras();
+    if (nprob_a != 0)
+        if (int rc = make_extras(who, nprob_a, record, K, 1, tie_a, (double)inlier_th_a, (double)tie_window_a, EA)) return rc;
+    if (nprob_b != 0)
+        if (int rc = make_extras(who, nprob_b, record, K, 2, tie_b, inlier_th_b, tie_window_b, EB)) return rc;
+    EB.draws = draws_b; EB.seed = seed_b;
+    return ANCSH_OK;
+}
+
+#define POSE_FIT_PARAMS(KEY_T)                                                                                                             \
+    int nprob_a, const int *off, const float *src, const float *tgt, float inlier_th_a, int niter_a, const int *draws_a, KEY_T key_a,     \
+        int max_n, double *out_model_a, unsigned char *out_inliers_a, int *out_best_a, int *scratch_scores_a, float *scratch_quads,        \
+        long rows, int *tie_stats_a, float tie_window_a, int nprob_b, const int *rng0, const int *rng1, const float *joint_dir,            \
+        double inlier_th_b, int niter_b, const int *draws_b, KEY_T key_b, double *out_model_b, unsigned char *out_inliers_b,               \
+        int *out_best_b, double *out_score_b, double *scratch_scores_b, double *scratch_models_b, int *lm_stat, int lm_schedule,           \
+        int *tie_stats_b, double tie_window_b, double *record, int K
+#define POSE_FIT_CALL(KM, KA, KB, KIND)                                                                                                    \
+    pose_fit_impl<KM>(nprob_a, off, src, tgt, inlier_th_a, niter_a, draws_a, KA, max_n, out_model_a, out_inliers_a, out_best_a,            \
+                      scratch_scores_a, scratch_quads, rows, EA, nprob_b, rng0, rng1, joint_dir, inlier_th_b, niter_b, draws_b, KB,        \
+                      out_model_b, out_inliers_b, out_best_b, out_score_b, scratch_scores_b, scratch_models_b, lm_stat, lm_schedule, EB,   \
+                      KIND, stream)
+
+static int pose_fit_rec(const char *who, POSE_FIT_PARAMS(unsigned long long), const int *joint_kind, void *stream) {
+    if (int rc = check_joint_kind(who, nprob_b, joint_kind)) return rc;
+    FitExtras EA, EB;
+    if (int rc = pose_fit_extras(who, nprob_a, nprob_b, record, K, tie_stats_a, inlier_th_a, tie_window_a, tie_stats_b, inlier_th_b, tie_window_b,
+                                 draws_b, key_b, EA, EB)) return rc;
+    return POSE_FIT_CALL(KEY_VALUE, key_a, key_b, joint_kind);
+}
+
+static int pose_fit_rec_dseed(const char *who, POSE_FIT_PARAMS(const unsigned long long *), const int *joint_kind, void *stream) {
+    ANCSH_REQUIRE((key_a || nprob_a <= 0) && (key_b || nprob_b <= 0), "%s: null seed pointer", who);
+    if (int rc = check_joint_kind(who, nprob_b, joint_kind)) return rc;
+    FitExtras EA, EB;
+    if (int rc = pose_fit_extras(who, nprob_a, nprob_b, record, K, tie_stats_a, inlier_th_a, tie_window_a, tie_stats_b, inlier_th_b, tie_window_b,
+                                 draws_b, (unsigned long long)(uintptr_t)key_b, EA, EB)) return rc;
+    return POSE_FIT_CALL(KEY_DSEED, (unsigned long long)(uintptr_t)key_a, (unsigned long long)(uintptr_t)key_b, joint_kind);
+}
+
+static int pose_fit_rec_dkey(const char *who, POSE_FIT_PARAMS(const ancsh_stream_key *), const int *joint_kind, void *stream) {
+    ANCSH_REQUIRE((key_a || nprob_a <= 0) && (key_b || nprob_b <= 0), "%s: null key pointer", who);
+    ANCSH_REQUIRE(K >= 1 && nprob_a >= 0 && nprob_a % K == 0 && nprob_a < (1 << 20), "%s: nprob_a (%d) must be a multiple of K (%d) below 2^20", who,
+                  nprob_a, K);
+    ANCSH_REQUIRE(nprob_b == 0 || (K >= 2 && nprob_b > 0 && nprob_b % (K - 1) == 0 && nprob_b < (1 << 20)),
+                  "%s: nprob_b (%d) must be a multiple of K - 1 (K = %d >= 2) below 2^20", who, nprob_b, K);
+    if (int rc = check_joint_kind(who, nprob_b, joint_kind)) return rc;
+    FitExtras EA, EB;
+    if (int rc = pose_fit_extras(who, nprob_a, nprob_b, record, K, tie_stats_a, inlier_th_a, tie_window_a, tie_stats_b, inlier_th_b, tie_window_b,
+                                 draws_b, (unsigned long long)(uintptr_t)key_b, EA, EB)) return rc;
+    return POSE_FIT_CALL(KEY_DKEY, (DKey{key_a, K}), (DKey{key_b, K - 1}), joint_kind);
+}
+
+#define POSE_FIT_ARGS                                                                                                                      \
+    nprob_a, off, src, tgt, inlier_th_a, niter_a, draws_a, key_a, max_n, out_model_a, out_inliers_a, out_best_a, scratch_scores_a,          \
+        scratch_quads, rows, tie_stats_a, tie_window_a, nprob_b, rng0, rng1, joint_dir, inlier_th_b, niter_b, draws_b, key_b, out_model_b,  \
+        out_inliers_b, out_best_b, out_score_b, scratch_scores_b, scratch_models_b, lm_stat, lm_schedule, tie_stats_b, tie_window_b, record, K
+
+extern "C" int ancsh_pose_fit_rec(POSE_FIT_PARAMS(unsigned long long), void *stream) {
+    return pose_fit_rec("pose_fit_rec", POSE_FIT_ARGS, nullptr, stream);
+}
+extern "C" int ancsh_pose_fit_rec_dseed(POSE_FIT_PARAMS(const unsigned long long *), void *stream) {
+    return pose_fit_rec_dseed("pose_fit_rec_dseed", POSE_FIT_ARGS, nullptr, stream);
+}
+extern "C" int ancsh_pose_fit_rec_dkey(POSE_FIT_PARAMS(const ancsh_stream_key *), void *stream) {
+    return pose_fit_rec_dkey("pose_fit_rec_dkey", POSE_FIT_ARGS, nullptr, stream);
+}
+extern "C" int ancsh_pose_fit_rec_kind(POSE_FIT_PARAMS(unsigned long long), const int *joint_kind, void *stream) {
+    return pose_fit_rec("pose_fit_rec_kind", POSE_FIT_ARGS, joint_kind, stream);
+}
+extern "C" int ancsh_pose_fit_rec_dseed_kind(POSE_FIT_PARAMS(const unsigned long long *), const int *joint_kind, void *stream) {
+    return pose_fit_rec_dseed("pose_fit_rec_dseed_kind", POSE_FIT_ARGS, joint_kind, stream);
+}
+extern "C" int ancsh_pose_fit_rec_dkey_kind(POSE_FIT_PARAMS(const ancsh_stream_key *), const int *joint_kind, void *stream) {
+    return pose_fit_rec_dkey("pose_fit_rec_dkey_kind", POSE_FIT_ARGS, joint_kind, stream);
+}
+#undef POSE_FIT_PARAMS
+#undef POSE_FIT_CALL
+#undef POSE_FIT_ARGS
+
 extern "C" int ancsh_umeyama(int nprob, const int *off, const float *src, const float *tgt, double *out, void *stream) {
     ANCSH_REQUIRE(nprob >= 0, "umeyama: negative nprob");
     if (nprob == 0) return ANCSH_OK;
diff --git a/articulated-pose_amd/pose/parallel_ancsh_pose.py b/articulated-pose_amd/pose/parallel_ancsh_pose.py
--- a/articulated-pose_amd/pose/parallel_ancsh_pose.py
+++ b/articulated-pose_amd/pose/parallel_ancsh_pose.py
@@ -136,6 +136,45 @@
     return dict(model=model, inliers=inl, best=best, score=score, lm_stat=stat, hyp_models=mo, hyp_scores=sc, tie=tie, _keep=(d, joint_kind))
 
 
+def pose_fit_batch(off, rng0, rng1, src, tgt, joint_dir, inlier_th, niter_a, niter_b, draws_a=None, draws_b=None, seed=0, max_n=None,
+                   want_lm_stat=False, lm_schedule="auto", record=None, K=0, tie_window=None, seed_dev=None, key_dev=None, joint_kind=None):
+    dev = src.device
+    npa, npb = off.numel() - 1, rng0.shape[0]
+    rows = src.shape[0]
+    max_n = int(max_n or rows)
+    E = lambda shape, dt: torch.empty(shape, dtype=dt, device=dev)
+    model_a, inl_a, best_a, scores_a = E((npa, 13), torch.float64), E((rows,), torch.uint8), E((npa, 2), torch.int32), E((npa * niter_a,), torch.int32)
+    quads = E((_lib.lib().ancsh_ransac_single_quads_floats(rows, npa),), torch.float32)
+    model_b, inl_b, best_b, score_b = E((npb, 26), torch.float64), E((npb, 2, max_n), torch.uint8), E((npb,), torch.int32), E((npb,), torch.float64)
+    sc_b, mo_b = E((npb * niter_b,), torch.float64), E((npb * niter_b, 26), torch.float64)
+    stat = E((npb, niter_b, 2), torch.int32) if want_lm_stat else None
+    tie_a = E((npa, 2), torch.int32) if tie_window is not None else None
+    tie_b = E((npb, 2), torch.int32) if tie_window is not None else None
+    da = None if draws_a is None else _i32(draws_a, dev)
+    db = None if draws_b is None else _i32(draws_b, dev)
+    if da is not None and da.numel() != npa * niter_a * 3:
+        raise ValueError("draws_a must have shape (nprob_a, niter_a, 3)")
+    if db is not None and db.numel() != npb * niter_b * 6:
+        raise ValueError("draws_b must have shape (nprob_b, niter_b, 6)")
+    if joint_kind is not None and (joint_kind.dtype != torch.int32 or joint_kind.numel() != npb or not joint_kind.is_contiguous()):
+        raise ValueError("joint_kind must be a contiguous int32 tensor of %d entries (one per problem)" % npb)
+    if key_dev is not None:
+        name, key_a, key_b = "ancsh_pose_fit_rec_dkey", _lib.ptr(key_dev), _lib.ptr(key_dev)
+    elif seed_dev is not None:
+        name, key_a, key_b = "ancsh_pose_fit_rec_dseed", _lib.ptr(seed_dev), _lib.ptr(seed_dev)
+    else:
+        name, key_a, key_b = "ancsh_pose_fit_rec", int(seed), int(seed) + 1
+    _lib.call(name + ("_kind" if joint_kind is not None else ""),
+              npa, _lib.ptr(off), _lib.ptr(src), _lib.ptr(tgt), float(inlier_th), int(niter_a), _lib.ptr(da), key_a, max_n, _lib.ptr(model_a),
+              _lib.ptr(inl_a), _lib.ptr(best_a), _lib.ptr(scores_a), _lib.ptr(quads), rows, _lib.ptr(tie_a), float(tie_window or 0.0),
+              npb, _lib.ptr(rng0), _lib.ptr(rng1), _lib.ptr(joint_dir), float(inlier_th), int(niter_b), _lib.ptr(db), key_b, _lib.ptr(model_b),
+              _lib.ptr(inl_b), _lib.ptr(best_b), _lib.ptr(score_b), _lib.ptr(sc_b), _lib.ptr(mo_b), _lib.ptr(stat), LM_SCHEDULES[lm_schedule],
+              _lib.ptr(tie_b), float(tie_window or 0.0), _lib.ptr(record), int(K), *([_lib.ptr(joint_kind)] if joint_kind is not None else []))
+    return (dict(model=model_a, inliers=inl_a, best=best_a, scores=scores_a.view(npa, niter_a), tie=tie_a, _keep=(da, scores_a, quads)),
+            dict(model=model_b, inliers=inl_b, best=best_b, score=score_b, lm_stat=stat, hyp_models=mo_b, hyp_scores=sc_b, tie=tie_b,
+                 _keep=(db, joint_kind)))
+
+
 def draws_from_seed(seed, counts, niter_a, niter_b):
     rs = np.random.RandomState(seed)
     K = len(counts)
@@ -153,6 +192,8 @@
 
 class PoseSolver(object):
 
+    fused_launch = True
+
     def __init__(self, num_parts, inlier_th=0.1, niter_a=10000, niter_b=200, device="cuda:0", want_lm_stat=False,
                  max_part_points=None, lm_schedule="auto", tie_window=TIE_WINDOW, joint_types=None):
         kinds = check_joint_types(joint_types, num_parts)
@@ -181,8 +222,12 @@
             from .quality import check_fit_quality
             check_fit_quality(True, self.th)
         out = self._partition(P, nocs_pred, mask_pred)
-        self._stage_b_fits(out, joint_axis_per_point, joint_cls, draws_b, seed, seed_dev, key_dev, joint_index)
-        out = self._poison(self._stage_a_fits(out, draws_a, seed, seed_dev, key_dev))
+        if self.fused_launch and self.K > 1 and self.lm_schedule != "latency":
+            self._fused_fits(out, joint_axis_per_point, joint_cls, draws_a, draws_b, seed, seed_dev, key_dev, joint_index)
+        else:
+            self._stage_b_fits(out, joint_axis_per_point, joint_cls, draws_b, seed, seed_dev, key_dev, joint_index)
+            self._stage_a_fits(out, draws_a, seed, seed_dev, key_dev)
+        out = self._poison(out)
         if fit_quality:
             from .quality import fit_quality_batch
             out["record_wide"] = fit_quality_batch(out, self.th)
@@ -238,6 +283,11 @@
         a = ransac_single_batch(out["off"], out["_src"], out["_tgt"], self.th, self.niter_a,
                                 None if draws_a is None else _i32(draws_a, dev).reshape(B * K, self.niter_a, 3), seed, out["_max_n"],
                                 record=out["record"], K=K, tie_window=self.tie_window, seed_dev=seed_dev, key_dev=key_dev)
+        return self._publish_a(out, a)
+
+    def _publish_a(self, out, a):
+        K = self.K
+        B, N = out["_shape"]
         out.update(baseline=out["record"][:, :, :13], best_a=a["best"].view(B, K, 2), inliers_a=a["inliers"].view(B, N))
         if a["tie"] is not None:
             out["tie_a"] = a["tie"].view(B, K, 2)
@@ -256,34 +306,60 @@
         src, tgt, max_n = out["_src"], out["_tgt"], out["_max_n"]
         rng0, rng1 = out["_rng"]
         if K > 1:
-            axis = _f32(joint_axis_per_point, dev)
-            out["_axis"] = axis
-            jdir = torch.empty((B, K - 1, 3), dtype=torch.float32, device=dev)
-            if joint_index is not None:
-                index = _f32(joint_index, dev)
-                if index.dim() != 3 or tuple(index.shape[:2]) != (B, N):
-                    raise ValueError("joint_index must be (B, N, C) for %d clouds of %d points, got %s" % (B, N, tuple(index.shape)))
-                out["_index"] = index
-                _lib.call("ancsh_pose_joint_direction_pred", B, N, K, int(index.shape[2]), _lib.ptr(axis), _lib.ptr(index), _lib.ptr(jdir))
-            else:
-                jcls = _i32(joint_cls, dev)
-                _lib.call("ancsh_pose_joint_direction", B, N, K, _lib.ptr(axis), _lib.ptr(jcls), _lib.ptr(jdir))
+            jdir = self._joint_directions(out, joint_axis_per_point, joint_cls, joint_index)
             b = ransac_joint_batch(rng0, rng1, src, tgt, jdir.view(-1, 3), self.th, self.niter_b,
                                    None if draws_b is None else _i32(draws_b, dev).reshape(B * (K - 1), self.niter_b, 6),
                                    seed + 1, max_n, want_lm_stat=self.want_lm_stat, lm_schedule=self.lm_schedule,
                                    record=out["record"], K=K, tie_window=self.tie_window, seed_dev=seed_dev, key_dev=key_dev,
                                    joint_kind=self.prepare(B))
-            if self.want_lm_stat:
-                out["lm_stat"] = b["lm_stat"].view(B, K - 1, self.niter_b, 2)
-            out["nonlinear"] = out["record"][:, :, 13:]
-            if b["tie"] is not None:
-                out["tie_b"] = b["tie"].view(B, K - 1, 2)
-            out["best_b"] = b["best"].view(B, K - 1)
-            out["score_b"] = b["score"].view(B, K - 1)
-            out["joint_direction"] = jdir
-            out["inliers_b"] = b["inliers"].view(B, K - 1, 2, max_n)
+            self._publish_b(out, b, jdir)
         else:
             out["nonlinear"] = out["record"][:, :, 13:]
+        return out
+
+    def _joint_directions(self, out, joint_axis_per_point, joint_cls, joint_index):
+        dev, K = self.device, self.K
+        B, N = out["_shape"]
+        axis = _f32(joint_axis_per_point, dev)
+        out["_axis"] = axis
+        jdir = torch.empty((B, K - 1, 3), dtype=torch.float32, device=dev)
+        if joint_index is not None:
+            index = _f32(joint_index, dev)
+            if index.dim() != 3 or tuple(index.shape[:2]) != (B, N):
+                raise ValueError("joint_index must be (B, N, C) for %d clouds of %d points, got %s" % (B, N, tuple(index.shape)))
+            out["_index"] = index
+            _lib.call("ancsh_pose_joint_direction_pred", B, N, K, int(index.shape[2]), _lib.ptr(axis), _lib.ptr(index), _lib.ptr(jdir))
+        else:
+            jcls = _i32(joint_cls, dev)
+            _lib.call("ancsh_pose_joint_direction", B, N, K, _lib.ptr(axis), _lib.ptr(jcls), _lib.ptr(jdir))
+        return jdir
+
+    def _fused_fits(self, out, joint_axis_per_point, joint_cls, draws_a=None, draws_b=None, seed=0, seed_dev=None, key_dev=None,
+                    joint_index=None):
+        dev, K = self.device, self.K
+        B, N = out["_shape"]
+        rng0, rng1 = out["_rng"]
+        jdir = self._joint_directions(out, joint_axis_per_point, joint_cls, joint_index)
+        a, b = pose_fit_batch(out["off"], rng0, rng1, out["_src"], out["_tgt"], jdir.view(-1, 3), self.th, self.niter_a, self.niter_b,
+                              None if draws_a is None else _i32(draws_a, dev).reshape(B * K, self.niter_a, 3),
+                              None if draws_b is None else _i32(draws_b, dev).reshape(B * (K - 1), self.niter_b, 6),
+                              seed, out["_max_n"], want_lm_stat=self.want_lm_stat, lm_schedule=self.lm_schedule, record=out["record"], K=K,
+                              tie_window=self.tie_window, seed_dev=seed_dev, key_dev=key_dev, joint_kind=self.prepare(B))
+        self._publish_b(out, b, jdir)
+        return self._publish_a(out, a)
+
+    def _publish_b(self, out, b, jdir):
+        K, max_n = self.K, out["_max_n"]
+        B, N = out["_shape"]
+        if self.want_lm_stat:
+            out["lm_stat"] = b["lm_stat"].view(B, K - 1, self.niter_b, 2)
+        out["nonlinear"] = out["record"][:, :, 13:]
+        if b["tie"] is not None:
+            out["tie_b"] = b["tie"].view(B, K - 1, 2)
+        out["best_b"] = b["best"].view(B, K - 1)
+        out["score_b"] = b["score"].view(B, K - 1)
+        out["joint_direction"] = jdir
+        out["inliers_b"] = b["inliers"].view(B, K - 1, 2, max_n)
         return out
 
 
diff --git a/include/ancsh_hip.h b/include/ancsh_hip.h
--- a/include/ancsh_hip.h
+++ b/include/ancsh_hip.h
@@ -294,6 +294,49 @@
                                      double *scratch_scores, double *scratch_models, int *lm_stat, int lm_schedule, double *record, int K,
                                      int *tie_stats, double tie_window, const int *joint_kind, void *stream);
 
+int ancsh_pose_fit_rec(int nprob_a, const int *off, const float *src, const float *tgt, float inlier_th_a, int niter_a,
+        const int *draws_a, unsigned long long key_a, int max_n, double *out_model_a, unsigned char *out_inliers_a, int *out_best_a,
+        int *scratch_scores_a, float *scratch_quads, long rows, int *tie_stats_a, float tie_window_a, int nprob_b, const int *rng0,
+        const int *rng1, const float *joint_dir, double inlier_th_b, int niter_b, const int *draws_b, unsigned long long key_b,
+        double *out_model_b, unsigned char *out_inliers_b, int *out_best_b, double *out_score_b, double *scratch_scores_b,
+        double *scratch_models_b, int *lm_stat, int lm_schedule, int *tie_stats_b, double tie_window_b, double *record, int K,
+        void *stream);
+int ancsh_pose_fit_rec_dseed(int nprob_a, const int *off, const float *src, const float *tgt, float inlier_th_a, int niter_a,
+        const int *draws_a, const unsigned long long * key_a, int max_n, double *out_model_a, unsigned char *out_inliers_a, int *out_best_a,
+        int *scratch_scores_a, float *scratch_quads, long rows, int *tie_stats_a, float tie_window_a, int nprob_b, const int *rng0,
+        const int *rng1, const float *joint_dir, double inlier_th_b, int niter_b, const int *draws_b, const unsigned long long * key_b,
+        double *out_model_b, unsigned char *out_inliers_b, int *out_best_b, double *out_score_b, double *scratch_scores_b,
+        double *scratch_models_b, int *lm_stat, int lm_schedule, int *tie_stats_b, double tie_window_b, double *record, int K,
+        void *stream);
+int ancsh_pose_fit_rec_dkey(int nprob_a, const int *off, const float *src, const float *tgt, float inlier_th_a, int niter_a,
+        const int *draws_a, const ancsh_stream_key * key_a, int max_n, double *out_model_a, unsigned char *out_inliers_a, int *out_best_a,
+        int *scratch_scores_a, float *scratch_quads, long rows, int *tie_stats_a, float tie_window_a, int nprob_b, const int *rng0,
+        const int *rng1, const float *joint_dir, double inlier_th_b, int niter_b, const int *draws_b, const ancsh_stream_key * key_b,
+        double *out_model_b, unsigned char *out_inliers_b, int *out_best_b, double *out_score_b, double *scratch_scores_b,
+        double *scratch_models_b, int *lm_stat, int lm_schedule, int *tie_stats_b, double tie_window_b, double *record, int K,
+        void *stream);
+int ancsh_pose_fit_rec_kind(int nprob_a, const int *off, const float *src, const float *tgt, float inlier_th_a, int niter_a,
+        const int *draws_a, unsigned long long key_a, int max_n, double *out_model_a, unsigned char *out_inliers_a, int *out_best_a,
+        int *scratch_scores_a, float *scratch_quads, long rows, int *tie_stats_a, float tie_window_a, int nprob_b, const int *rng0,
+        const int *rng1, const float *joint_dir, double inlier_th_b, int niter_b, const int *draws_b, unsigned long long key_b,
+        double *out_model_b, unsigned char *out_inliers_b, int *out_best_b, double *out_score_b, double *scratch_scores_b,
+        double *scratch_models_b, int *lm_stat, int lm_schedule, int *tie_stats_b, double tie_window_b, double *record, int K,
+        const int *joint_kind, void *stream);
+int ancsh_pose_fit_rec_dseed_kind(int nprob_a, const int *off, const float *src, const float *tgt, float inlier_th_a, int niter_a,
+        const int *draws_a, const unsigned long long * key_a, int max_n, double *out_model_a, unsigned char *out_inliers_a, int *out_best_a,
+        int *scratch_scores_a, float *scratch_quads, long rows, int *tie_stats_a, float tie_window_a, int nprob_b, const int *rng0,
+        const int *rng1, const float *joint_dir, double inlier_th_b, int niter_b, const int *draws_b, const unsigned long long * key_b,
+        double *out_model_b, unsigned char *out_inliers_b, int *out_best_b, double *out_score_b, double *scratch_scores_b,
+        double *scratch_models_b, int *lm_stat, int lm_schedule, int *tie_stats_b, double tie_window_b, double *record, int K,
+        const int *joint_kind, void *stream);
+int ancsh_pose_fit_rec_dkey_kind(int nprob_a, const int *off, const float *src, const float *tgt, float inlier_th_a, int niter_a,
+        const int *draws_a, const ancsh_stream_key * key_a, int max_n, double *out_model_a, unsigned char *out_inliers_a, int *out_best_a,
+        int *scratch_scores_a, float *scratch_quads, long rows, int *tie_stats_a, float tie_window_a, int nprob_b, const int *rng0,
+        const int *rng1, const float *joint_dir, double inlier_th_b, int niter_b, const int *draws_b, const ancsh_stream_key * key_b,
+        double *out_model_b, unsigned char *out_inliers_b, int *out_best_b, double *out_score_b, double *scratch_scores_b,
+        double *scratch_models_b, int *lm_stat, int lm_schedule, int *tie_stats_b, double tie_window_b, double *record, int K,
+        const int *joint_kind, void *stream);
+
 int ancsh_umeyama(int nprob, const int *off, const float *src, const float *tgt, double *out, void *stream);
 
 int ancsh_estimate_similarity_transform(int nprob, const int *off, const float *src, const float *tgt, int niter,
```

Result: faster. 18320 (median of 6 runs) (+3.4%).
